# facebookresearch/PartDistillation

Measured on AMD Instinct MI355X. Metric: images/sec training step, R50 Mask2Former 1024² bs=2/GPU, 1/2/4/8 MI355X, higher is better.
Workload: dtype bf16

## Files before the change

### include/pd_rowwise.h

```cpp
#ifndef PD_ROWWISE_H
#define PD_ROWWISE_H

#include <stdint.h>

#ifdef __cplusplus
extern "C" {
#endif

int pd_add_layernorm_fwd(const void *x, int x_dtype, const float *res, const float *gamma, const float *beta, float eps,
                         float *z, float *y, void *y_c, const float *pos, int pos_div, void *ypos_c, int c_dtype,
                         float *mean, float *rstd, int rows, int C, void *stream);

int pd_add_layernorm_bwd(const float *dy, const float *dy2, const void *dy_c, const void *dypos_c, int c_dtype,
                         const float *z, const float *mean, const float *rstd, const float *gamma, float *dz, void *dz_c,
                         int dzc_dtype, float *dgamma, float *dbeta, float *dbias, float *dpos_acc, int pos_div,
                         int rows, int C, void *stream);

int pd_add_layernorm_fwd_amax(const void *x, int x_dtype, const float *res, const float *gamma, const float *beta, float eps,
                              float *z, float *y, void *y_c, const float *pos, int pos_div, void *ypos_c, int c_dtype,
                              float *mean, float *rstd, float *y_amax, float *ypos_amax, int rows, int C, void *stream);
int pd_add_layernorm_bwd_amax(const float *dy, const float *dy2, const void *dy_c, const void *dypos_c, int c_dtype,
                              const float *z, const float *mean, const float *rstd, const float *gamma, float *dz, void *dz_c,
                              int dzc_dtype, float *dgamma, float *dbeta, float *dbias, float *dpos_acc, int pos_div,
                              float *dz_amax, int rows, int C, void *stream);

int pd_colsum_acc(const void *x, int dtype, int rows, int N, float *acc, void *stream);

int pd_relu_bwd_colsum(void *dh, const void *h, int dtype, int rows, int N, float *acc, void *stream);

int pd_mem_prep_fwd(const float *tok, int64_t tok_batch_stride, const float *level_embed, const float *pos, void *mem_c,
                    void *mempos_c, int c_dtype, int B, int HW, int C, void *stream);

int pd_mem_prep_bwd(const void *dmem_c, const void *dmempos_c, int c_dtype, float *dtok, int64_t dtok_batch_stride, int B,
                    int HW, int C, void *stream);

int pd_attn_mask_u8(const void *logits, int dtype, int rows, int n, uint8_t *mask, void *stream);

int pd_matcher_point_terms(const void *x, int dtype, int rows, int n, float *x_f32, float *sigmoid_x, float *softplus_sum,
                           float *sigmoid_sum, void *stream);

int pd_msda_prep_fwd(const float *offs, const float *logits, const float *ref, const int64_t *spatial_shapes, float *loc,
                     float *attn, int64_t tokens, int M, int L, int P, int ld_offs, int ld_logits, void *stream);

int pd_msda_prep_bwd(const float *gloc, const float *gattn, const float *attn, const int64_t *spatial_shapes, float *d_offs,
                     float *d_logits, int64_t tokens, int M, int L, int P, int ld_offs, int ld_logits, void *stream);
int pd_msda_prep_bwd_amax(const float *gloc, const float *gattn, const float *attn, const int64_t *spatial_shapes, float *d_offs, float *d_logits,
                          float *row_amax, int64_t tokens, int M, int L, int P, int ld_offs, int ld_logits, void *stream);

int pd_point_sample_nhwc_f32(const float *in, const float *coords, float *out, int B, int H, int W, int C, int P, void *stream);
int pd_point_sample_nhwc_f32_bf16(const float *in, const float *coords, void *out, int B, int H, int W, int C, int P, void *stream);

int pd_point_sample_planar_f32(const float *in, const float *coords, float *out, int N, int C, int H, int W, int P, void *stream);
int pd_point_sample_planar_bwd_f32(const float *grad_out, const float *coords, float *grad_in, int N, int C, int H, int W, int P, void *stream);
int pd_point_sample_planar_bwd_needs_zero(int C, int H, int W);
int pd_point_sample_planar_bwd_needs_zero_n(int N, int C, int H, int W);

int pd_upsample_add_nhwc_f32(const float *lo, int64_t lo_batch_stride, const float *cur, float *y, int B, int h, int w, int H, int W, int C, void *stream);
int pd_upsample_add_amax_nhwc_f32(const float *lo, int64_t lo_batch_stride, const float *cur, float *y, float *amax, int B, int h, int w, int H, int W, int C,
                                  void *stream);
int pd_upsample2x_bwd_nhwc_f32(const float *dy, float *dlo, int B, int h, int w, int C, void *stream);

#define PD_RESIZE_MAX 4
int pd_resize_bilinear_nhwc_f32(const float *x, int B, int H, int W, int C, const int *heights, const int *widths, void *const *outs, int count,
                                int out_dtype, void *stream);


int pd_add_rows_amax_f32(const float *a, const float *b, float *q, float *a_copy, float *a_amax, float *q_amax, int rows, int cols, void *stream);

int pd_sum3_sum2_f32(const float *a, const float *b, const float *c, const float *d, float *out1, float *out2, int64_t n, void *stream);

int pd_skinny_linear_fwd(const void *x_bf16, const void *w, const void *b, int wb_dtype, float *y, int R, int C, int K, void *stream);
int64_t pd_skinny_linear_partial_floats(int R, int C, int K);
int pd_skinny_linear_bwd(const void *x_bf16, const void *w, int w_dtype, const float *dy, const void *dx_in_bf16, void *dx_out, int dx_dtype,
                         float *partial, void *dw, void *db, int b_dtype, int R, int C, int K, void *stream);

#define PD_TRANSPOSE_MAX 8
typedef struct {
  const void *src;
  void *dst;
  int64_t src_batch_stride, src_row_stride;
  int32_t batch, rows, cols, reserved;
} PdTransposeProblem;
int pd_transpose_batched_f32(const PdTransposeProblem *problems, int count, void *stream);

#define PD_COPY_MAX_SEGS 48
typedef struct PdCopySeg {
  const void *src;
  void *dst;
  int64_t bytes;
} PdCopySeg;
int pd_copy_segments(const PdCopySeg *segs, int count, void *stream);

#ifdef __cplusplus
}
#endif
#endif
```

### partdistillation_amd/csrc/cmdbuf.hip

```cpp
#include <hip/hip_runtime.h>
#include <stdint.h>
#include <string.h>

#include <type_traits>
#include <utility>

#include "pd_common.h"
#include "pd_cmdbuf.h"
#include "pd_attention.h"
#include "pd_conv.h"
#include "pd_declayer.h"
#include "pd_criterion.h"
#include "pd_fused.h"
#include "pd_gemm.h"
#include "pd_grouping.h"
#include "pd_igemm.h"
#include "pd_input.h"
#include "pd_kmeans.h"
#include "pd_msda.h"
#include "pd_mx8.h"
#include "pd_optim.h"
#include "pd_poly.h"
#include "pd_rowwise.h"
#include "pd_smallgemm.h"
#include "pd_stem.h"
#include "pd_swin.h"
#include "pd_window_attention.h"

namespace {

template <class T>
inline T word_to(uint64_t w)
{
  if constexpr (std::is_pointer_v<T>) {
    return reinterpret_cast<T>(static_cast<uintptr_t>(w));
  } else if constexpr (std::is_same_v<T, float>) {
    float f; uint32_t u = (uint32_t)w; memcpy(&f, &u, 4); return f;
  } else if constexpr (std::is_same_v<T, double>) {
    double d; memcpy(&d, &w, 8); return d;
  } else {
    return static_cast<T>(static_cast<int64_t>(w));
  }
}

template <auto F> struct Thunk;
template <class... A, int (*F)(A...)>
struct Thunk<F> {
  static constexpr int nargs = (int)sizeof...(A);
  template <size_t... I>
  static int invoke(const uint64_t *w, std::index_sequence<I...>) { return F(word_to<A>(w[I])...); }
  static int call(const uint64_t *w) { return invoke(w, std::index_sequence_for<A...>{}); }
};

struct Entry { const char *name; int (*call)(const uint64_t *); int nargs; };
#define PD_E(f) {#f, &Thunk<&f>::call, Thunk<&f>::nargs}
const Entry kTable[] = {
  PD_E(pd_adamw_clipped),
  PD_E(pd_adamw_clipped_shadow),
  PD_E(pd_add_layernorm_bwd),
  PD_E(pd_add_layernorm_bwd_amax),
  PD_E(pd_add_layernorm_fwd),
  PD_E(pd_add_layernorm_fwd_amax),
  PD_E(pd_add_rows_amax_f32),
  PD_E(pd_affine_act_bwd2_bf16),
  PD_E(pd_affine_act_bwd_bf16),
  PD_E(pd_affine_act_fwd_bf16),
  PD_E(pd_attn_bwd_d32),
  PD_E(pd_attn_fwd_d32),
  PD_E(pd_attn_mask_u8),
  PD_E(pd_cast_bf16_f32_amax),
  PD_E(pd_colsum_acc),
  PD_E(pd_conv3x3_nhwc_f16x2),
  PD_E(pd_conv3x3_nhwc_f32x3),
  PD_E(pd_conv3x3_wgrad_nhwc_f16x2),
  PD_E(pd_conv3x3_wgrad_nhwc_f32x3),
  PD_E(pd_conv_bf16_dgrad),
  PD_E(pd_conv_bf16_fwd),
  PD_E(pd_conv_bf16_wgrad),
  PD_E(pd_conv_bf16_wgrad_grouped),
  PD_E(pd_dec_bwd_a),
  PD_E(pd_dec_bwd_b),
  PD_E(pd_dec_fwd_a),
  PD_E(pd_dec_fwd_b),
  PD_E(pd_dec_pack_grouped),
  PD_E(pd_decoder_head_bf16),
  PD_E(pd_filter_transpose_grouped),
  PD_E(pd_gemm_tn_f16x2),
  PD_E(pd_gemm_tn_f16x2_bf16out),
  PD_E(pd_gemm_tn_f32),
  PD_E(pd_gemm_tn_f32x3),
  PD_E(pd_gemm_tn_f32x3_pre),
  PD_E(pd_gemm_tn_f32x3_relu_bits),
  PD_E(pd_gemm_tn_f32x3_relumask),
  PD_E(pd_gemm_wgrad_acc_f16x2_ws),
  PD_E(pd_gemm_wgrad_acc_f32),
  PD_E(pd_gemm_wgrad_acc_f32x3),
  PD_E(pd_gemm_wgrad_acc_f32x3_ws),
  PD_E(pd_gemm_wgrad_f16x2_grouped),
  PD_E(pd_gemm_wgrad_f32),
  PD_E(pd_gemm_wgrad_f32x3_grouped),
  PD_E(pd_gn_coeffs_bwd),
  PD_E(pd_gn_coeffs_fwd),
  PD_E(pd_igemm_bf16),
  PD_E(pd_igemm_bf16_seq),
  PD_E(pd_kmeans_assign),
  PD_E(pd_kmeans_assign_bounded),
  PD_E(pd_kmeans_assign_partial),
  PD_E(pd_kmeans_reduce),
  PD_E(pd_kmeans_reduce_update),
  PD_E(pd_kmeans_reduce_update_shift),
  PD_E(pd_kmeans_update),
  PD_E(pd_layernorm_rows_f32_bwd),
  PD_E(pd_layernorm_rows_f32_fwd),
  PD_E(pd_loss_vectors_bwd),
  PD_E(pd_loss_vectors_fwd),
  PD_E(pd_lsa_batched),
  PD_E(pd_mask_assign),
  PD_E(pd_mask_point_losses_bwd),
  PD_E(pd_mask_point_losses_fwd),
  PD_E(pd_matcher_costs),
  PD_E(pd_copy_segments),
  PD_E(pd_attn_fwd_d32_ld),
  PD_E(pd_attn_bwd_d32_ld),
  PD_E(pd_match_point_logits),
  PD_E(pd_swin_merge_ln_fwd),
  PD_E(pd_swin_tail_ln_fwd),
  PD_E(pd_swin_tail_ln_bwd),
  PD_E(pd_swin_merge_ln_bwd),
  PD_E(pd_matcher_point_terms),
  PD_E(pd_maxpool3s2_bwd_bf16),
  PD_E(pd_maxpool3s2_fwd_bf16),
  PD_E(pd_mem_prep_bwd),
  PD_E(pd_mem_prep_fwd),
  PD_E(pd_memcpy_d2d_async),
  PD_E(pd_memset_async),
  PD_E(pd_msda_backward),
  PD_E(pd_msda_forward),
  PD_E(pd_msda_forward_amax),
  PD_E(pd_msda_fused_backward),
  PD_E(pd_msda_fused_forward),
  PD_E(pd_msda_prep_bwd),
  PD_E(pd_msda_prep_bwd_amax),
  PD_E(pd_msda_prep_fwd),
  PD_E(pd_multi_gather_sumsq),
  PD_E(pd_mx8_gemm),
  PD_E(pd_mx8_quantize_bf16),
  PD_E(pd_mx8_quantize_grouped),
  PD_E(pd_nc_affine2_amax_f32),
  PD_E(pd_nc_affine2_f32),
  PD_E(pd_nc_affine_amax_f32),
  PD_E(pd_nc_affine_f32),
  PD_E(pd_nc_sums_f32),
  PD_E(pd_normalize_u8_nhwc),
  PD_E(pd_pair_logits_bwd_rows),
  PD_E(pd_pair_logits_bwd_tok),
  PD_E(pd_pair_logits_fwd),
  PD_E(pd_point_sample_nhwc_f32),
  PD_E(pd_point_sample_nhwc_f32_bf16),
  PD_E(pd_point_sample_planar_bwd_f32),
  PD_E(pd_point_sample_planar_f32),
  PD_E(pd_point_sample_u8),
  PD_E(pd_poly_crossings_i32),
  PD_E(pd_relu_bwd_colsum),
  PD_E(pd_resample_cols_canvas_u8),
  PD_E(pd_resample_cols_u8),
  PD_E(pd_resample_rows_u8),
  PD_E(pd_resize_bilinear_nhwc_f32),
  PD_E(pd_rle_sample_groups_canvas_u8),
  PD_E(pd_rle_sample_groups_u8),
  PD_E(pd_rle_sample_u8),
  PD_E(pd_row_amax_f32),
  PD_E(pd_scores_argmax_u8),
  PD_E(pd_sgemm_nn_bf16),
  PD_E(pd_sgemm_nn_splitn_bf16),
  PD_E(pd_sgemm_tn_batched_bf16),
  PD_E(pd_sgemm_tn_bf16),
  PD_E(pd_sgemm_tn_multi_bf16),
  PD_E(pd_sgemm_tn_splitk_bf16),
  PD_E(pd_sgemm_wgrad_bf16),
  PD_E(pd_sgemm_wgrad_grouped_bf16),
  PD_E(pd_sgemm_wgrad_split_bf16),
  PD_E(pd_skinny_linear_bwd),
  PD_E(pd_skinny_linear_fwd),
  PD_E(pd_split3_bf16),
  PD_E(pd_stem7x7_fwd),
  PD_E(pd_stem7x7_wgrad),
  PD_E(pd_sum3_sum2_f32),
  PD_E(pd_sumsq_accumulate),
  PD_E(pd_swin_ln_bwd),
  PD_E(pd_swin_ln_fwd),
  PD_E(pd_transpose_batched_f32),
  PD_E(pd_uncertain_points),
  PD_E(pd_upsample2x_bwd_nhwc_f32),
  PD_E(pd_upsample_add_amax_nhwc_f32),
  PD_E(pd_upsample_add_nhwc_f32),
  PD_E(pd_wgrad_bf16),
  PD_E(pd_wgrad_bf16_seq),
  PD_E(pd_window_attn_bwd_w12),
  PD_E(pd_window_attn_bwd_w7),
  PD_E(pd_window_attn_fwd_w12),
  PD_E(pd_window_attn_fwd_w7),
};
constexpr int kCount = (int)(sizeof(kTable) / sizeof(kTable[0]));
}

extern "C" int pd_memset_async(void *dst, int value, int64_t bytes, void *stream)
{
  if (bytes <= 0) return PD_OK;
  return hipMemsetAsync(dst, value, (size_t)bytes, (hipStream_t)stream) == hipSuccess ? PD_OK : pd_set_error(PD_ERR_LAUNCH, "pd_memset_async failed");
}

extern "C" int pd_memcpy_d2d_async(void *dst, const void *src, int64_t bytes, void *stream)
{
  if (bytes <= 0) return PD_OK;
  return hipMemcpyAsync(dst, src, (size_t)bytes, hipMemcpyDeviceToDevice, (hipStream_t)stream) == hipSuccess ? PD_OK
                                                                                                         : pd_set_error(PD_ERR_LAUNCH, "pd_memcpy_d2d_async failed");
}

extern "C" int pd_cmd_fn_index(const char *name)
{
  if (!name) return -1;
  for (int i = 0; i < kCount; ++i)
    if (!strcmp(kTable[i].name, name)) return i;
  return -1;
}

extern "C" int pd_cmd_fn_nargs(int fn) { return fn >= 0 && fn < kCount ? kTable[fn].nargs : -1; }

extern "C" int pd_cmd_replay(const PdCmd *cmds, int count, const uint64_t *slot_bases, int nslots, void *stream)
{
  uint64_t w[PD_CMD_MAX_ARGS];
  for (int c = 0; c < count; ++c) {
    const PdCmd &k = cmds[c];
    if (k.fn < 0 || k.fn >= kCount || k.nargs != kTable[k.fn].nargs || k.nargs > PD_CMD_MAX_ARGS)
      return pd_set_error(PD_ERR_INVALID_ARG, "pd_cmd_replay: command %d is malformed", c);
    for (int i = 0; i < k.nargs; ++i) {
      const int s = k.kind[i];
      if (s == PD_CMD_LITERAL) w[i] = k.a[i];
      else if (s == PD_CMD_STREAM) w[i] = (uint64_t)(uintptr_t)stream;
      else if (s >= 0 && s < nslots) w[i] = slot_bases[s] + k.a[i];
      else return pd_set_error(PD_ERR_INVALID_ARG, "pd_cmd_replay: command %d argument %d names slot %d of %d", c, i, s, nslots);
    }
    const int rc = kTable[k.fn].call(w);
    if (rc != PD_OK) return rc;
  }
  return PD_OK;
}
```

### partdistillation_amd/csrc/common.hip

```cpp
#include <hip/hip_runtime.h>
#include <stdarg.h>
#include <stdio.h>
#include <string.h>

#include "pd_common.h"
#include "pd_msda.h"

namespace {
thread_local char g_err[512] = {0};
}

int pd_set_error(int code, const char *fmt, ...)
{
  va_list ap;
  va_start(ap, fmt);
  vsnprintf(g_err, sizeof(g_err), fmt, ap);
  va_end(ap);
  return code;
}

int pd_check_launch(const char *what)
{
  hipError_t e = hipGetLastError();
  if (e == hipSuccess) return PD_OK;
  return pd_set_error(PD_ERR_LAUNCH, "%s: %s", what, hipGetErrorString(e));
}

extern "C" const char *pd_last_error(void) { return g_err; }
extern "C" int pd_abi_version(void) { return 49; }

extern int g_pd_dbg_atomic_scope;
extern int g_pd_dbg_force_generic;
extern int g_pd_dbg_ablate;
extern int g_pd_dbg_x3_narrow;
extern int g_pd_dbg_f16x2;
extern int g_pd_dbg_wgrad_wide;
extern "C" void pd_dbg_set_wgrad_xcd(int v);
extern "C" void pd_dbg_set_wgrad_fast(int v);
extern int g_pd_dbg_bwd_variant;
extern int g_pd_dbg_msda_gate_pct;
extern int g_pd_dbg_wgrad_wgs;
extern int g_pd_dbg_bwd_threads;
extern int g_pd_dbg_attn_scalar;
extern int g_pd_dbg_wattn;
extern int g_pd_dbg_wattn_chunk;
extern int g_pd_dbg_x3;
extern int g_pd_dbg_kmeans;
extern int g_pd_dbg_conv_group_rows;
extern int g_pd_dbg_conv_xcd_major;
extern int g_pd_dbg_sgemm_deep;
extern int g_ig_bn, g_ig_nst, g_ig_splits, g_ig_patch, g_ig_pcls;
extern int g_mx_bn, g_mx_nst;
extern int g_swin_ln_abl;
extern int g_ln_bwd_cap;
extern int g_crit_abl;
extern int g_attn_bwd_kc;
extern int g_wg_nst, g_wg_splits, g_wg_mode;
extern "C" int pd_debug_set(const char *key, int value)
{
  if (!key) return PD_ERR_INVALID_ARG;
  if (!strcmp(key, "msda_bwd_atomic_scope")) { g_pd_dbg_atomic_scope = value; return PD_OK; }
  if (!strcmp(key, "msda_ablate")) { g_pd_dbg_ablate = value; return PD_OK; }
  if (!strcmp(key, "msda_bwd_variant")) { g_pd_dbg_bwd_variant = value; return PD_OK; }
  if (!strcmp(key, "msda_gate_pct")) { g_pd_dbg_msda_gate_pct = value; return PD_OK; }
  if (!strcmp(key, "attn_scalar")) { g_pd_dbg_attn_scalar = value; return PD_OK; }
  if (!strcmp(key, "msda_bwd_threads")) { g_pd_dbg_bwd_threads = value; return PD_OK; }
  if (!strcmp(key, "wgrad_wgs")) { g_pd_dbg_wgrad_wgs = value; return PD_OK; }
  if (!strcmp(key, "kmeans_ablate")) { g_pd_dbg_kmeans = value; return PD_OK; }
  if (!strcmp(key, "wg_nst")) { g_wg_nst = value; return PD_OK; }
  if (!strcmp(key, "wg_splits")) { g_wg_splits = value; return PD_OK; }
  if (!strcmp(key, "wg_mode")) { g_wg_mode = value; return PD_OK; }
  if (!strcmp(key, "ig_bn")) { g_ig_bn = value; return PD_OK; }
  if (!strcmp(key, "ig_patch")) { g_ig_patch = value; return PD_OK; }
  if (!strcmp(key, "ig_pcls")) { g_ig_pcls = value; return PD_OK; }
  if (!strcmp(key, "ig_nst")) { g_ig_nst = value; return PD_OK; }
  if (!strcmp(key, "mx_bn")) { g_mx_bn = value; return PD_OK; }
  if (!strcmp(key, "attn_bwd_kc")) { g_attn_bwd_kc = value; return PD_OK; }
  if (!strcmp(key, "crit_abl")) { g_crit_abl = value; return PD_OK; }
  if (!strcmp(key, "ln_bwd_cap")) { g_ln_bwd_cap = value; return PD_OK; }
  if (!strcmp(key, "swin_ln_abl")) { g_swin_ln_abl = value; return PD_OK; }
  if (!strcmp(key, "mx_nst")) { g_mx_nst = value; return PD_OK; }
  if (!strcmp(key, "ig_splits")) { g_ig_splits = value; return PD_OK; }
  if (!strcmp(key, "sgemm_deep")) { g_pd_dbg_sgemm_deep = value; return PD_OK; }
  if (!strcmp(key, "conv_group_rows")) { g_pd_dbg_conv_group_rows = value; return PD_OK; }
  if (!strcmp(key, "conv_xcd_major")) { g_pd_dbg_conv_xcd_major = value; return PD_OK; }
  if (!strcmp(key, "x3_ablate")) { g_pd_dbg_x3 = value; return PD_OK; }
  if (!strcmp(key, "f16x2_tile")) { g_pd_dbg_f16x2 = value; return PD_OK; }
  if (!strcmp(key, "wgrad_wide")) { g_pd_dbg_wgrad_wide = value; return PD_OK; }
  if (!strcmp(key, "wgrad_xcd")) { pd_dbg_set_wgrad_xcd(value); return PD_OK; }
  if (!strcmp(key, "wgrad_fast")) { pd_dbg_set_wgrad_fast(value); return PD_OK; }
  if (!strcmp(key, "x3_narrow")) { g_pd_dbg_x3_narrow = value; return PD_OK; }
  if (!strcmp(key, "wattn_ablate")) { g_pd_dbg_wattn = value; return PD_OK; }
  if (!strcmp(key, "wattn_chunk")) {
    if (value < 0 || value > 8) return pd_set_error(PD_ERR_INVALID_ARG, "pd_debug_set: wattn_chunk is 0 (automatic) or 1..8, got %d", value);
    g_pd_dbg_wattn_chunk = value;
    return PD_OK;
  }
  if (!strcmp(key, "msda_force_generic")) { g_pd_dbg_force_generic = value; return PD_OK; }
  return pd_set_error(PD_ERR_INVALID_ARG, "pd_debug_set: unknown key %s", key);
}

extern "C" int pd_debug_get(const char *key, int *value)
{
  if (!key || !value) return PD_ERR_INVALID_ARG;
  if (!strcmp(key, "msda_bwd_variant")) { *value = g_pd_dbg_bwd_variant; return PD_OK; }
  if (!strcmp(key, "msda_gate_pct")) { *value = g_pd_dbg_msda_gate_pct; return PD_OK; }
  return pd_set_error(PD_ERR_INVALID_ARG, "pd_debug_get: unknown key %s", key);
}
```

### partdistillation_amd/csrc/rowwise.hip

```cpp
#include <hip/hip_runtime.h>
#include <stdint.h>
#include <string.h>

#include "pd_common.h"
#include "pd_msda.h"
#include "pd_rowwise.h"

int g_ln_bwd_cap = 0;
namespace {

typedef unsigned short bf16_t;

__device__ __forceinline__ float bf2f(bf16_t h) { return __uint_as_float((unsigned)h << 16); }
__device__ __forceinline__ bf16_t f2bf(float f)
{
  unsigned u = __float_as_uint(f);
  if ((u & 0x7fffffffu) > 0x7f800000u) return (bf16_t)((u >> 16) | 0x40);
  u += 0x7fffu + ((u >> 16) & 1u);
  return (bf16_t)(u >> 16);
}

__device__ __forceinline__ float4 ld4(const float *p) { return *reinterpret_cast<const float4 *>(p); }
__device__ __forceinline__ float4 ld4(const bf16_t *p)
{
  const ushort4 v = *reinterpret_cast<const ushort4 *>(p);
  return make_float4(bf2f(v.x), bf2f(v.y), bf2f(v.z), bf2f(v.w));
}
__device__ __forceinline__ void st4(float *p, float4 v) { *reinterpret_cast<float4 *>(p) = v; }
__device__ __forceinline__ void st4(bf16_t *p, float4 v)
{
  ushort4 o;
  o.x = f2bf(v.x); o.y = f2bf(v.y); o.z = f2bf(v.z); o.w = f2bf(v.w);
  *reinterpret_cast<ushort4 *>(p) = o;
}
__device__ __forceinline__ float4 add4(float4 a, float4 b) { return make_float4(a.x + b.x, a.y + b.y, a.z + b.z, a.w + b.w); }

template <int CTRL>
__device__ __forceinline__ float dpp_mov(float v)
{
  return __int_as_float(__builtin_amdgcn_update_dpp(0, __float_as_int(v), CTRL, 0xF, 0xF, true));
}

__device__ __forceinline__ float wave_sum(float v)
{
  v += dpp_mov<0xB1>(v);
  v += dpp_mov<0x4E>(v);
  v += dpp_mov<0x141>(v);
  v += dpp_mov<0x140>(v);
  v += __shfl_xor(v, 16, 64);
  v += __shfl_xor(v, 32, 64);
  return v;
}

__device__ __forceinline__ float wave_max(float v)
{
  v = fmaxf(v, dpp_mov<0xB1>(v));
  v = fmaxf(v, dpp_mov<0x4E>(v));
  v = fmaxf(v, dpp_mov<0x141>(v));
  v = fmaxf(v, dpp_mov<0x140>(v));
  v = fmaxf(v, __shfl_xor(v, 16, 64));
  v = fmaxf(v, __shfl_xor(v, 32, 64));
  return v;
}
__device__ __forceinline__ float amax4(float4 v) { return fmaxf(fmaxf(fabsf(v.x), fabsf(v.y)), fmaxf(fabsf(v.z), fabsf(v.w))); }

template <int NV4, typename XT, typename CT>
__global__ __launch_bounds__(256) void add_ln_fwd(const XT *__restrict__ x, const float *__restrict__ res,
                                                  const float *__restrict__ gamma, const float *__restrict__ beta, float eps,
                                                  float *__restrict__ z, float *__restrict__ y, CT *__restrict__ y_c,
                                                  const float *__restrict__ pos, int pos_div, CT *__restrict__ ypos_c,
                                                  float *__restrict__ mean, float *__restrict__ rstd, int rows,
                                                  float *__restrict__ y_amax, float *__restrict__ ypos_amax)
{
  constexpr int C = NV4 * 256;
  const int wave = threadIdx.x >> 6, lane = threadIdx.x & 63;
  float4 gm[NV4], bt[NV4];
#pragma unroll
  for (int j = 0; j < NV4; ++j) {
    gm[j] = ld4(gamma + j * 256 + lane * 4);
    bt[j] = ld4(beta + j * 256 + lane * 4);
  }
  for (int r = blockIdx.x * 4 + wave; r < rows; r += gridDim.x * 4) {
    const int64_t base = (int64_t)r * C + lane * 4;
    float4 v[NV4];
    float s = 0.f;
#pragma unroll
    for (int j = 0; j < NV4; ++j) {
      v[j] = x ? ld4(x + base + j * 256) : make_float4(0.f, 0.f, 0.f, 0.f);
      if (res) v[j] = add4(v[j], ld4(res + base + j * 256));
      if (z) st4(z + base + j * 256, v[j]);
      s += (v[j].x + v[j].y) + (v[j].z + v[j].w);
    }
    const float mu = wave_sum(s) * (1.f / C);
    float q = 0.f;
#pragma unroll
    for (int j = 0; j < NV4; ++j) {
      v[j].x -= mu; v[j].y -= mu; v[j].z -= mu; v[j].w -= mu;
      q += (v[j].x * v[j].x + v[j].y * v[j].y) + (v[j].z * v[j].z + v[j].w * v[j].w);
    }
    const float rs = rsqrtf(wave_sum(q) * (1.f / C) + eps);
    if (lane == 0) { mean[r] = mu; rstd[r] = rs; }
    const float *prow = pos ? pos + (int64_t)(r / pos_div) * C + lane * 4 : nullptr;
    float my = 0.f, mp = 0.f;
#pragma unroll
    for (int j = 0; j < NV4; ++j) {
      float4 o;
      o.x = v[j].x * rs * gm[j].x + bt[j].x;
      o.y = v[j].y * rs * gm[j].y + bt[j].y;
      o.z = v[j].z * rs * gm[j].z + bt[j].z;
      o.w = v[j].w * rs * gm[j].w + bt[j].w;
      if (y) st4(y + base + j * 256, o);
      if (y_c) st4(y_c + base + j * 256, o);
      my = fmaxf(my, amax4(o));
      if (ypos_c) {
        const float4 op = add4(o, ld4(prow + j * 256));
        st4(ypos_c + base + j * 256, op);
        mp = fmaxf(mp, amax4(op));
      }
    }
    if (y_amax) { my = wave_max(my); if (lane == 0) y_amax[r] = my; }
    if (ypos_amax) { mp = wave_max(mp); if (lane == 0) ypos_amax[r] = mp; }
  }
}

template <int NV4, typename CT, typename DT, int WAVES>
__global__ __launch_bounds__(64 * WAVES) void add_ln_bwd(const float *dy, const float *__restrict__ dy2,
                                                  const CT *__restrict__ dy_c, const CT *__restrict__ dypos_c,
                                                  const float *__restrict__ z, const float *__restrict__ mean,
                                                  const float *__restrict__ rstd, const float *__restrict__ gamma,
                                                  float *dz, DT *__restrict__ dz_c, float *__restrict__ dgamma,
                                                  float *__restrict__ dbeta, float *__restrict__ dbias,
                                                  float *__restrict__ dpos_acc, int pos_div, int rows, float *__restrict__ dz_amax)
{
  constexpr int C = NV4 * 256;
  __shared__ float red[WAVES][3][C];
  const int wave = threadIdx.x >> 6, lane = threadIdx.x & 63;
  float4 gm[NV4], ag[NV4], ab[NV4], ad[NV4];
#pragma unroll
  for (int j = 0; j < NV4; ++j) {
    gm[j] = ld4(gamma + j * 256 + lane * 4);
    ag[j] = ab[j] = ad[j] = make_float4(0.f, 0.f, 0.f, 0.f);
  }
  for (int r = blockIdx.x * WAVES + wave; r < rows; r += gridDim.x * WAVES) {
    const int64_t base = (int64_t)r * C + lane * 4;
    const float mu = mean[r], rs = rstd[r];
    float4 g[NV4], xh[NV4];
    float s1 = 0.f, s2 = 0.f;
#pragma unroll
    for (int j = 0; j < NV4; ++j) {
      float4 t = make_float4(0.f, 0.f, 0.f, 0.f);
      if (dy) t = ld4(dy + base + j * 256);
      if (dy2) t = add4(t, ld4(dy2 + base + j * 256));
      if (dy_c) t = add4(t, ld4(dy_c + base + j * 256));
      if (dypos_c) {
        const float4 p = ld4(dypos_c + base + j * 256);
        t = add4(t, p);
        if (dpos_acc) {
          float *a = dpos_acc + (int64_t)(r / pos_div) * C + j * 256 + lane * 4;
          if (pos_div == 1) st4(a, add4(ld4(a), p));
          else { atomicAdd(a, p.x); atomicAdd(a + 1, p.y); atomicAdd(a + 2, p.z); atomicAdd(a + 3, p.w); }
        }
      }
      float4 h = ld4(z + base + j * 256);
      h.x = (h.x - mu) * rs; h.y = (h.y - mu) * rs; h.z = (h.z - mu) * rs; h.w = (h.w - mu) * rs;
      ag[j].x += t.x * h.x; ag[j].y += t.y * h.y; ag[j].z += t.z * h.z; ag[j].w += t.w * h.w;
      ab[j] = add4(ab[j], t);
      t.x *= gm[j].x; t.y *= gm[j].y; t.z *= gm[j].z; t.w *= gm[j].w;
      s1 += (t.x + t.y) + (t.z + t.w);
      s2 += (t.x * h.x + t.y * h.y) + (t.z * h.z + t.w * h.w);
      g[j] = t; xh[j] = h;
    }
    const float m1 = wave_sum(s1) * (1.f / C), m2 = wave_sum(s2) * (1.f / C);
    float mz = 0.f;
#pragma unroll
    for (int j = 0; j < NV4; ++j) {
      float4 o;
      o.x = rs * (g[j].x - m1 - xh[j].x * m2);
      o.y = rs * (g[j].y - m1 - xh[j].y * m2);
      o.z = rs * (g[j].z - m1 - xh[j].z * m2);
      o.w = rs * (g[j].w - m1 - xh[j].w * m2);
      ad[j] = add4(ad[j], o);
      st4(dz + base + j * 256, o);
      if (dz_c) st4(dz_c + base + j * 256, o);
      mz = fmaxf(mz, amax4(o));
    }
    if (dz_amax) { mz = wave_max(mz); if (lane == 0) dz_amax[r] = mz; }
  }
  if (!dgamma && !dbeta && !dbias) return;
#pragma unroll
  for (int j = 0; j < NV4; ++j) {
    st4(&red[wave][0][j * 256 + lane * 4], ag[j]);
    st4(&red[wave][1][j * 256 + lane * 4], ab[j]);
    st4(&red[wave][2][j * 256 + lane * 4], ad[j]);
  }
  __syncthreads();
  float *const outs[3] = {dgamma, dbeta, dbias};
  for (int i = threadIdx.x; i < 3 * C; i += 64 * WAVES) {
    const int k = i / C, c = i - k * C;
    if (!outs[k]) continue;
    float sum = 0.f;
#pragma unroll
    for (int w = 0; w < WAVES; ++w) sum += red[w][k][c];
    atomicAdd(outs[k] + c, sum);
  }
}

template <typename T, bool RELU>
__global__ __launch_bounds__(256) void colsum_acc(T *__restrict__ x, const T *__restrict__ h, int rows, int N, int rows_per_blk,
                                                  float *__restrict__ acc)
{
  __shared__ float red[4][128];
  const int wave = threadIdx.x >> 6, lane = threadIdx.x & 63;
  const int c0 = blockIdx.x * 128 + lane * 2;
  const int r_begin = blockIdx.y * rows_per_blk, r_end = min(rows, r_begin + rows_per_blk);
  float a0 = 0.f, a1 = 0.f;
  int r = r_begin + wave;
  if (!RELU && sizeof(T) == 4) {
    for (; r + 12 < r_end; r += 16) {
      const float *p = reinterpret_cast<const float *>(x) + (int64_t)r * N + c0;
      const float2 u0 = *reinterpret_cast<const float2 *>(p), u1 = *reinterpret_cast<const float2 *>(p + (int64_t)4 * N);
      const float2 u2 = *reinterpret_cast<const float2 *>(p + (int64_t)8 * N), u3 = *reinterpret_cast<const float2 *>(p + (int64_t)12 * N);
      a0 += (u0.x + u1.x) + (u2.x + u3.x);
      a1 += (u0.y + u1.y) + (u2.y + u3.y);
    }
  }
  for (; r < r_end; r += 4) {
    T *p = x + (int64_t)r * N + c0;
    float v0, v1;
    if constexpr (sizeof(T) == 2) {
      const unsigned u = *reinterpret_cast<const unsigned *>(p);
      v0 = bf2f((bf16_t)(u & 0xffffu)); v1 = bf2f((bf16_t)(u >> 16));
    } else {
      const float2 u = *reinterpret_cast<const float2 *>(p);
      v0 = u.x; v1 = u.y;
    }
    if (RELU) {
      float h0, h1;
      if constexpr (sizeof(T) == 2) {
        const unsigned u = *reinterpret_cast<const unsigned *>(h + (int64_t)r * N + c0);
        h0 = bf2f((bf16_t)(u & 0xffffu)); h1 = bf2f((bf16_t)(u >> 16));
      } else {
        const float2 u = *reinterpret_cast<const float2 *>(h + (int64_t)r * N + c0);
        h0 = u.x; h1 = u.y;
      }
      if (!(h0 > 0.f)) v0 = 0.f;
      if (!(h1 > 0.f)) v1 = 0.f;
      if constexpr (sizeof(T) == 2) *reinterpret_cast<unsigned *>(p) = (unsigned)f2bf(v0) | ((unsigned)f2bf(v1) << 16);
      else *reinterpret_cast<float2 *>(p) = make_float2(v0, v1);
    }
    a0 += v0; a1 += v1;
  }
  if (!acc) return;
  red[wave][lane * 2] = a0; red[wave][lane * 2 + 1] = a1;
  __syncthreads();
  if (threadIdx.x < 128) {
    const int c = threadIdx.x;
    atomicAdd(acc + blockIdx.x * 128 + c, (red[0][c] + red[1][c]) + (red[2][c] + red[3][c]));
  }
}

template <typename CT>
__global__ __launch_bounds__(256) void mem_prep_fwd(const float *__restrict__ tok, int64_t bstride, const float *__restrict__ lvl,
                                                    const float *__restrict__ pos, CT *__restrict__ mem, CT *__restrict__ mempos,
                                                    int B, int HW, int C)
{
  const int wave = threadIdx.x >> 6, lane = threadIdx.x & 63;
  const int rows = B * HW;
  for (int r = blockIdx.x * 4 + wave; r < rows; r += gridDim.x * 4) {
    const int p = r / B, b = r - p * B;
    const float *src = tok + (int64_t)b * bstride + (int64_t)p * C;
    for (int c = lane * 4; c < C; c += 256) {
      float4 v = ld4(src + c);
      if (lvl) v = add4(v, ld4(lvl + c));
      if (mem) st4(mem + (int64_t)r * C + c, v);
      if (mempos) st4(mempos + (int64_t)r * C + c, add4(v, ld4(pos + (int64_t)p * C + c)));
    }
  }
}

template <typename CT>
__global__ __launch_bounds__(256) void mem_prep_bwd(const CT *__restrict__ dmem, const CT *__restrict__ dmempos,
                                                    float *__restrict__ dtok, int64_t bstride, int B, int HW, int C)
{
  const int wave = threadIdx.x >> 6, lane = threadIdx.x & 63;
  const int rows = B * HW;
  for (int r = blockIdx.x * 4 + wave; r < rows; r += gridDim.x * 4) {
    const int b = r / HW, p = r - b * HW;
    const int64_t srow = ((int64_t)p * B + b) * C;
    float *dst = dtok + (int64_t)b * bstride + (int64_t)p * C;
    for (int c = lane * 4; c < C; c += 256) {
      float4 v = make_float4(0.f, 0.f, 0.f, 0.f);
      if (dmem) v = ld4(dmem + srow + c);
      if (dmempos) v = add4(v, ld4(dmempos + srow + c));
      st4(dst + c, v);
    }
  }
}

template <typename T>
__global__ __launch_bounds__(256) void attn_mask_u8(const T *__restrict__ logits, int n, uint8_t *__restrict__ mask)
{
  __shared__ int any_open;
  const T *row = logits + (int64_t)blockIdx.x * n;
  uint8_t *out = mask + (int64_t)blockIdx.x * n;
  if (threadIdx.x == 0) any_open = 0;
  __syncthreads();
  int open = 0;
  for (int i = threadIdx.x; i < n; i += 256) {
    float v;
    if constexpr (sizeof(T) == 2) v = bf2f(row[i]); else v = row[i];
    open |= !(v < 0.f);
  }
  if (__ballot(open) != 0ull && (threadIdx.x & 63) == 0) atomicOr(&any_open, 1);
  __syncthreads();
  const bool keep = any_open != 0;
  for (int i = threadIdx.x; i < n; i += 256) {
    float v;
    if constexpr (sizeof(T) == 2) v = bf2f(row[i]); else v = row[i];
    out[i] = (keep && v < 0.f) ? 1 : 0;
  }
}

__device__ __forceinline__ unsigned neg2(unsigned w)
{
  const unsigned lo = w & 0xffffu, hi = w >> 16;
  const unsigned bl = (lo & 0x8000u) && (lo & 0x7fffu) != 0u && (lo & 0x7fffu) <= 0x7f80u;
  const unsigned bh = (hi & 0x8000u) && (hi & 0x7fffu) != 0u && (hi & 0x7fffu) <= 0x7f80u;
  return bl | (bh << 8);
}
constexpr int AMV = 8;
__global__ __launch_bounds__(256) void attn_mask_u8_bf16x8(const bf16_t *__restrict__ logits, int n, uint8_t *__restrict__ mask)
{
  __shared__ int any_open;
  const uint4 *row = reinterpret_cast<const uint4 *>(logits + (int64_t)blockIdx.x * n);
  uint2 *out = reinterpret_cast<uint2 *>(mask + (int64_t)blockIdx.x * n);
  const int nv = n >> 3;
  if (threadIdx.x == 0) any_open = 0;
  uint2 b[AMV];
  unsigned all = 0x01010101u;
// ... 371 lines not shown
      for (int of = 32; of; of >>= 1) m = fmaxf(m, __shfl_xor(m, of, 64));
      if ((threadIdx.x & 63) == 0) amax[i >> 6] = m;
    }
  }
}

struct ResizeLevels { void *out[PD_RESIZE_MAX]; int h[PD_RESIZE_MAX], w[PD_RESIZE_MAX]; int64_t first[PD_RESIZE_MAX + 1]; int count; };

template <bool BF16>
__global__ __launch_bounds__(256) void resize_bilinear_nhwc_multi(const float *__restrict__ x, int B, int H, int W, int C4, ResizeLevels lv)
{
  for (int64_t i = (int64_t)blockIdx.x * 256 + threadIdx.x; i < lv.first[lv.count]; i += (int64_t)gridDim.x * 256) {
    int l = 0;
#pragma unroll
    for (int k = 1; k < PD_RESIZE_MAX; ++k) l += (k < lv.count && i >= lv.first[k]) ? 1 : 0;
    const int h = lv.h[l], w = lv.w[l];
    int64_t t = i - lv.first[l];
    const int c = (int)(t % C4); t /= C4;
    const int ox = (int)(t % w); t /= w;
    const int oy = (int)(t % h);
    const int b = (int)(t / h);
    int y0, yp, x0, xp; float hy0, hy1, wx0, wx1;
    up_src(oy, (float)H / (float)h, H, y0, yp, hy0, hy1);
    up_src(ox, (float)W / (float)w, W, x0, xp, wx0, wx1);
    const float4 *L = reinterpret_cast<const float4 *>(x) + (int64_t)b * H * W * C4;
    const float4 a = L[((int64_t)y0 * W + x0) * C4 + c], bq = L[((int64_t)y0 * W + x0 + xp) * C4 + c];
    const float4 cq = L[((int64_t)(y0 + yp) * W + x0) * C4 + c], d = L[((int64_t)(y0 + yp) * W + x0 + xp) * C4 + c];
    float4 o;
    o.x = hy0 * (wx0 * a.x + wx1 * bq.x) + hy1 * (wx0 * cq.x + wx1 * d.x);
    o.y = hy0 * (wx0 * a.y + wx1 * bq.y) + hy1 * (wx0 * cq.y + wx1 * d.y);
    o.z = hy0 * (wx0 * a.z + wx1 * bq.z) + hy1 * (wx0 * cq.z + wx1 * d.z);
    o.w = hy0 * (wx0 * a.w + wx1 * bq.w) + hy1 * (wx0 * cq.w + wx1 * d.w);
    const int64_t oi = (((int64_t)b * h + oy) * w + ox) * C4 + c;
    if (BF16) st4(reinterpret_cast<bf16_t *>(lv.out[l]) + oi * 4, o);
    else st4(reinterpret_cast<float *>(lv.out[l]) + oi * 4, o);
  }
}

__global__ __launch_bounds__(256) void upsample2x_bwd_nhwc(const float *__restrict__ dy, float *__restrict__ dlo, int B, int h,
                                                           int w, int C4)
{
  const int H = 2 * h, W = 2 * w;
  const int64_t total = (int64_t)B * h * w * C4;
  for (int64_t i = (int64_t)blockIdx.x * blockDim.x + threadIdx.x; i < total; i += (int64_t)gridDim.x * blockDim.x) {
    const int c = (int)(i % C4);
    int64_t t = i / C4;
    const int ix = (int)(t % w); t /= w;
    const int iy = (int)(t % h);
    const int b = (int)(t / h);
    float wy[4], wx[4];
#pragma unroll
    for (int k = 0; k < 4; ++k) {
      const int oy = 2 * iy - 1 + k, ox = 2 * ix - 1 + k;
      wy[k] = 0.f; wx[k] = 0.f;
      if (oy >= 0 && oy < H) {
        int i0, ip; float l0, l1;
        up_src(oy, 0.5f, h, i0, ip, l0, l1);
        if (i0 == iy) wy[k] += l0;
        if (i0 + ip == iy) wy[k] += l1;
      }
      if (ox >= 0 && ox < W) {
        int i0, ip; float l0, l1;
        up_src(ox, 0.5f, w, i0, ip, l0, l1);
        if (i0 == ix) wx[k] += l0;
        if (i0 + ip == ix) wx[k] += l1;
      }
    }
    const float4 *G = reinterpret_cast<const float4 *>(dy) + (int64_t)b * H * W * C4;
    float4 acc = make_float4(0.f, 0.f, 0.f, 0.f);
    float4 gt[4][4];
#pragma unroll
    for (int ky = 0; ky < 4; ++ky) {
      const int oy = min(max(2 * iy - 1 + ky, 0), H - 1);
#pragma unroll
      for (int kx = 0; kx < 4; ++kx) gt[ky][kx] = G[((int64_t)oy * W + min(max(2 * ix - 1 + kx, 0), W - 1)) * C4 + c];
    }
#pragma unroll
    for (int ky = 0; ky < 4; ++ky) {
#pragma unroll
      for (int kx = 0; kx < 4; ++kx) {
        const float wgt = wy[ky] * wx[kx];
        const bool on = wy[ky] != 0.f && wx[kx] != 0.f;
        const float4 g = gt[ky][kx];
        acc.x = on ? fmaf(wgt, g.x, acc.x) : acc.x; acc.y = on ? fmaf(wgt, g.y, acc.y) : acc.y;
        acc.z = on ? fmaf(wgt, g.z, acc.z) : acc.z; acc.w = on ? fmaf(wgt, g.w, acc.w) : acc.w;
      }
    }
    reinterpret_cast<float4 *>(dlo)[i] = acc;
  }
}

int grid_rows(int rows, int cap) { return max(1, min(cap, (rows + 3) / 4)); }

struct TrBatch { PdTransposeProblem p[PD_TRANSPOSE_MAX]; int first_tile[PD_TRANSPOSE_MAX + 1]; int count; };

__global__ __launch_bounds__(256) void transpose_batched_f32(TrBatch tb)
{
  __shared__ float tile[32][33];
  int pi = 0;
#pragma unroll
  for (int i = 1; i < PD_TRANSPOSE_MAX; ++i) pi += (i < tb.count && (int)blockIdx.x >= tb.first_tile[i]) ? 1 : 0;
  const PdTransposeProblem &pr = tb.p[pi];
  const int tr = (pr.rows + 31) / 32, tc = (pr.cols + 31) / 32;
  int t = blockIdx.x - tb.first_tile[pi];
  const int b = t / (tr * tc); t -= b * tr * tc;
  const int r0 = (t / tc) * 32, c0 = (t % tc) * 32;
  const int tx = threadIdx.x & 31, ty = threadIdx.x >> 5;
  const float *src = (const float *)pr.src + (int64_t)b * pr.src_batch_stride;
  float *dst = (float *)pr.dst + (int64_t)b * pr.rows * pr.cols;
#pragma unroll
  for (int k = 0; k < 4; ++k) {
    const int r = r0 + ty + 8 * k, c = c0 + tx;
    if (r < pr.rows && c < pr.cols) tile[ty + 8 * k][tx] = src[(int64_t)r * pr.src_row_stride + c];
  }
  __syncthreads();
#pragma unroll
  for (int k = 0; k < 4; ++k) {
    const int c = c0 + ty + 8 * k, r = r0 + tx;
    if (r < pr.rows && c < pr.cols) dst[(int64_t)c * pr.rows + r] = tile[tx][ty + 8 * k];
  }
}


__global__ __launch_bounds__(256) void add_rows_amax_f32(const float *__restrict__ a, const float *__restrict__ b, float *__restrict__ q,
                                                         float *__restrict__ a_copy, float *__restrict__ a_amax, float *__restrict__ q_amax,
                                                         int rows, int cols)
{
  const int row = blockIdx.x * 4 + (threadIdx.x >> 6), lane = threadIdx.x & 63;
  if (row >= rows) return;
  const int64_t base = (int64_t)row * cols;
  float ma = 0.f, mq = 0.f;
  for (int c = lane * 4; c < cols; c += 256) {
    const float4 x = ld4(a + base + c), y = ld4(b + base + c);
    const float4 s = make_float4(x.x + y.x, x.y + y.y, x.z + y.z, x.w + y.w);
    st4(q + base + c, s);
    if (a_copy) st4(a_copy + base + c, x);
    ma = fmaxf(ma, amax4(x)); mq = fmaxf(mq, amax4(s));
  }
#pragma unroll
  for (int o = 32; o; o >>= 1) { ma = fmaxf(ma, __shfl_xor(ma, o, 64)); mq = fmaxf(mq, __shfl_xor(mq, o, 64)); }
  if (lane == 0) { a_amax[row] = ma; q_amax[row] = mq; }
}

__global__ __launch_bounds__(256) void sum3_sum2_f32(const float4 *__restrict__ a, const float4 *__restrict__ b, const float4 *__restrict__ c,
                                                     const float4 *__restrict__ d, float4 *__restrict__ o1, float4 *__restrict__ o2, int64_t n4)
{
  for (int64_t i = (int64_t)blockIdx.x * 256 + threadIdx.x; i < n4; i += (int64_t)gridDim.x * 256) {
    const float4 x = a[i], y = b[i], z = c[i], w = d[i];
    o1[i] = make_float4((x.x + y.x) + z.x, (x.y + y.y) + z.y, (x.z + y.z) + z.z, (x.w + y.w) + z.w);
    o2[i] = make_float4(w.x + z.x, w.y + z.y, w.z + z.z, w.w + z.w);
  }
}

bool dt_ok(int dt) { return dt == PD_F32 || dt == PD_BF16; }

}

#define NV4_SWITCH(C, BODY)                                                                                        \
  switch ((C) / 256) {                                                                                             \
    case 1: { constexpr int NV4 = 1; BODY; } break;                                                                \
    case 2: { constexpr int NV4 = 2; BODY; } break;                                                                \
    case 3: { constexpr int NV4 = 3; BODY; } break;                                                                \
    case 4: { constexpr int NV4 = 4; BODY; } break;                                                                \
    default: return pd_set_error(PD_ERR_INVALID_ARG, "C=%d: supported widths are 256, 512, 768, 1024", (C)); \
  }

static int add_layernorm_fwd(const void *x, int x_dtype, const float *res, const float *gamma, const float *beta, float eps,
                             float *z, float *y, void *y_c, const float *pos, int pos_div, void *ypos_c, int c_dtype,
                             float *mean, float *rstd, int rows, int C, void *stream_, float *y_amax, float *ypos_amax)
{
  if (rows < 0 || C <= 0 || (C % 256)) return pd_set_error(PD_ERR_INVALID_ARG, "pd_add_layernorm_fwd: rows=%d C=%d", rows, C);
  if (rows == 0) return PD_OK;
  if ((!x && !res) || !gamma || !beta || !mean || !rstd) return pd_set_error(PD_ERR_INVALID_ARG, "pd_add_layernorm_fwd: null pointer");
  if ((x && !dt_ok(x_dtype)) || ((y_c || ypos_c) && !dt_ok(c_dtype))) return pd_set_error(PD_ERR_INVALID_ARG, "pd_add_layernorm_fwd: dtype");
  if (ypos_c && (!pos || pos_div <= 0)) return pd_set_error(PD_ERR_INVALID_ARG, "pd_add_layernorm_fwd: ypos_c needs pos and pos_div > 0");
  hipStream_t s = (hipStream_t)stream_;
  dim3 g(grid_rows(rows, 2048)), b(256);
  const bool xb = x && x_dtype == PD_BF16, cb = c_dtype == PD_BF16;
#define LAUNCH(XT, CT) hipLaunchKernelGGL((add_ln_fwd<NV4, XT, CT>), g, b, 0, s, (const XT *)x, res, gamma, beta, eps, z, y, (CT *)y_c, pos, pos_div, (CT *)ypos_c, mean, rstd, rows, y_amax, ypos_amax)
  NV4_SWITCH(C, {
    if (xb) { if (cb) LAUNCH(bf16_t, bf16_t); else LAUNCH(bf16_t, float); }
    else { if (cb) LAUNCH(float, bf16_t); else LAUNCH(float, float); }
  })
#undef LAUNCH
  return pd_check_launch("pd_add_layernorm_fwd");
}

extern "C" int pd_add_layernorm_fwd(const void *x, int x_dtype, const float *res, const float *gamma, const float *beta, float eps,
                                    float *z, float *y, void *y_c, const float *pos, int pos_div, void *ypos_c, int c_dtype,
                                    float *mean, float *rstd, int rows, int C, void *stream_)
{
  return add_layernorm_fwd(x, x_dtype, res, gamma, beta, eps, z, y, y_c, pos, pos_div, ypos_c, c_dtype, mean, rstd, rows, C, stream_, nullptr, nullptr);
}

extern "C" int pd_add_layernorm_fwd_amax(const void *x, int x_dtype, const float *res, const float *gamma, const float *beta, float eps,
                                         float *z, float *y, void *y_c, const float *pos, int pos_div, void *ypos_c, int c_dtype,
                                         float *mean, float *rstd, float *y_amax, float *ypos_amax, int rows, int C, void *stream_)
{
  if (ypos_amax && !ypos_c) return pd_set_error(PD_ERR_INVALID_ARG, "pd_add_layernorm_fwd_amax: ypos_amax needs ypos_c");
  return add_layernorm_fwd(x, x_dtype, res, gamma, beta, eps, z, y, y_c, pos, pos_div, ypos_c, c_dtype, mean, rstd, rows, C, stream_, y_amax, ypos_amax);
}

static int add_layernorm_bwd(const float *dy, const float *dy2, const void *dy_c, const void *dypos_c, int c_dtype,
                             const float *z, const float *mean, const float *rstd, const float *gamma, float *dz,
                             void *dz_c, int dzc_dtype, float *dgamma, float *dbeta, float *dbias, float *dpos_acc,
                             int pos_div, int rows, int C, void *stream_, float *dz_amax)
{
  if (rows < 0 || C <= 0 || (C % 256)) return pd_set_error(PD_ERR_INVALID_ARG, "pd_add_layernorm_bwd: rows=%d C=%d", rows, C);
  if (rows == 0) return PD_OK;
  if ((!dy && !dy2 && !dy_c && !dypos_c) || !z || !mean || !rstd || !gamma || !dz)
    return pd_set_error(PD_ERR_INVALID_ARG, "pd_add_layernorm_bwd: null pointer");
  if (((dy_c || dypos_c) && !dt_ok(c_dtype)) || (dz_c && !dt_ok(dzc_dtype))) return pd_set_error(PD_ERR_INVALID_ARG, "pd_add_layernorm_bwd: dtype");
  if (dpos_acc && pos_div <= 0) return pd_set_error(PD_ERR_INVALID_ARG, "pd_add_layernorm_bwd: pos_div");
  hipStream_t s = (hipStream_t)stream_;
  const bool cb = c_dtype == PD_BF16, db = dzc_dtype == PD_BF16;
#define LAUNCH(CT, DT, WV) hipLaunchKernelGGL((add_ln_bwd<NV4, CT, DT, WV>), g, b, 0, s, dy, dy2, (const CT *)dy_c, (const CT *)dypos_c, z, mean, rstd, gamma, dz, (DT *)dz_c, dgamma, dbeta, dbias, dpos_acc, pos_div, rows, dz_amax)
#define LAUNCH_W(WV)                                                                    \
  if (cb) { if (db) LAUNCH(bf16_t, bf16_t, WV); else LAUNCH(bf16_t, float, WV); }      \
  else { if (db) LAUNCH(float, bf16_t, WV); else LAUNCH(float, float, WV); }
  NV4_SWITCH(C, {
    constexpr int FAT = NV4 == 1 ? 16 : NV4 == 2 ? 8 : 4;
    if (rows >= 8192 && FAT > 4 && g_ln_bwd_cap >= 0) {
      const int cap = g_ln_bwd_cap > 0 ? g_ln_bwd_cap : 256;
      const dim3 g(max(1, min(cap, (rows + 4 * FAT - 1) / (4 * FAT))));
      const dim3 b(64 * FAT);
      LAUNCH_W(FAT)
    } else {
      const dim3 g(grid_rows(rows, 1024));
      const dim3 b(256);
      LAUNCH_W(4)
    }
  })
#undef LAUNCH_W
#undef LAUNCH
  return pd_check_launch("pd_add_layernorm_bwd");
}

extern "C" int pd_add_layernorm_bwd(const float *dy, const float *dy2, const void *dy_c, const void *dypos_c, int c_dtype,
                                    const float *z, const float *mean, const float *rstd, const float *gamma, float *dz,
                                    void *dz_c, int dzc_dtype, float *dgamma, float *dbeta, float *dbias, float *dpos_acc,
                                    int pos_div, int rows, int C, void *stream_)
{
  return add_layernorm_bwd(dy, dy2, dy_c, dypos_c, c_dtype, z, mean, rstd, gamma, dz, dz_c, dzc_dtype, dgamma, dbeta, dbias, dpos_acc, pos_div, rows, C,
                           stream_, nullptr);
}

extern "C" int pd_add_layernorm_bwd_amax(const float *dy, const float *dy2, const void *dy_c, const void *dypos_c, int c_dtype,
                                         const float *z, const float *mean, const float *rstd, const float *gamma, float *dz,
                                         void *dz_c, int dzc_dtype, float *dgamma, float *dbeta, float *dbias, float *dpos_acc,
                                         int pos_div, float *dz_amax, int rows, int C, void *stream_)
{
  return add_layernorm_bwd(dy, dy2, dy_c, dypos_c, c_dtype, z, mean, rstd, gamma, dz, dz_c, dzc_dtype, dgamma, dbeta, dbias, dpos_acc, pos_div, rows, C,
                           stream_, dz_amax);
}

static int colsum_launch(void *x, const void *h, int dtype, int rows, int N, float *acc, bool relu, hipStream_t s, const char *who)
{
  if (rows < 0 || N <= 0 || (N % 128) || !dt_ok(dtype)) return pd_set_error(PD_ERR_INVALID_ARG, "%s: rows=%d N=%d dtype=%d", who, rows, N, dtype);
  if (rows == 0) return PD_OK;
  if (!x || (relu && !h) || (!relu && !acc)) return pd_set_error(PD_ERR_INVALID_ARG, "%s: null pointer", who);
  const int rpb = rows <= 4096 ? 64 : 256;
  dim3 g(N / 128, (rows + rpb - 1) / rpb), b(256);
  if (dtype == PD_BF16) {
    if (relu) hipLaunchKernelGGL((colsum_acc<bf16_t, true>), g, b, 0, s, (bf16_t *)x, (const bf16_t *)h, rows, N, rpb, acc);
    else hipLaunchKernelGGL((colsum_acc<bf16_t, false>), g, b, 0, s, (bf16_t *)x, (const bf16_t *)h, rows, N, rpb, acc);
  } else {
    if (relu) hipLaunchKernelGGL((colsum_acc<float, true>), g, b, 0, s, (float *)x, (const float *)h, rows, N, rpb, acc);
    else hipLaunchKernelGGL((colsum_acc<float, false>), g, b, 0, s, (float *)x, (const float *)h, rows, N, rpb, acc);
  }
  return pd_check_launch(who);
}

extern "C" int pd_colsum_acc(const void *x, int dtype, int rows, int N, float *acc, void *stream_)
{
  return colsum_launch(const_cast<void *>(x), nullptr, dtype, rows, N, acc, false, (hipStream_t)stream_, "pd_colsum_acc");
}

extern "C" int pd_relu_bwd_colsum(void *dh, const void *h, int dtype, int rows, int N, float *acc, void *stream_)
{
  return colsum_launch(dh, h, dtype, rows, N, acc, true, (hipStream_t)stream_, "pd_relu_bwd_colsum");
}

extern "C" int pd_mem_prep_fwd(const float *tok, int64_t tok_batch_stride, const float *level_embed, const float *pos, void *mem_c,
                               void *mempos_c, int c_dtype, int B, int HW, int C, void *stream_)
{
  if (B < 0 || HW < 0 || C <= 0 || (C % 256) || !dt_ok(c_dtype)) return pd_set_error(PD_ERR_INVALID_ARG, "pd_mem_prep_fwd: B=%d HW=%d C=%d", B, HW, C);
  if (B == 0 || HW == 0) return PD_OK;
  if (!tok || (!mem_c && !mempos_c) || (mempos_c && !pos)) return pd_set_error(PD_ERR_INVALID_ARG, "pd_mem_prep_fwd: null pointer");
  dim3 g(grid_rows(B * HW, 4096)), b(256);
  if (c_dtype == PD_BF16) hipLaunchKernelGGL((mem_prep_fwd<bf16_t>), g, b, 0, (hipStream_t)stream_, tok, tok_batch_stride, level_embed, pos, (bf16_t *)mem_c, (bf16_t *)mempos_c, B, HW, C);
  else hipLaunchKernelGGL((mem_prep_fwd<float>), g, b, 0, (hipStream_t)stream_, tok, tok_batch_stride, level_embed, pos, (float *)mem_c, (float *)mempos_c, B, HW, C);
  return pd_check_launch("pd_mem_prep_fwd");
}

extern "C" int pd_mem_prep_bwd(const void *dmem_c, const void *dmempos_c, int c_dtype, float *dtok, int64_t dtok_batch_stride, int B,
                               int HW, int C, void *stream_)
{
  if (B < 0 || HW < 0 || C <= 0 || (C % 256) || !dt_ok(c_dtype)) return pd_set_error(PD_ERR_INVALID_ARG, "pd_mem_prep_bwd: B=%d HW=%d C=%d", B, HW, C);
  if (B == 0 || HW == 0) return PD_OK;
  if (!dtok || (!dmem_c && !dmempos_c)) return pd_set_error(PD_ERR_INVALID_ARG, "pd_mem_prep_bwd: null pointer");
  dim3 g(grid_rows(B * HW, 4096)), b(256);
  if (c_dtype == PD_BF16) hipLaunchKernelGGL((mem_prep_bwd<bf16_t>), g, b, 0, (hipStream_t)stream_, (const bf16_t *)dmem_c, (const bf16_t *)dmempos_c, dtok, dtok_batch_stride, B, HW, C);
  else hipLaunchKernelGGL((mem_prep_bwd<float>), g, b, 0, (hipStream_t)stream_, (const float *)dmem_c, (const float *)dmempos_c, dtok, dtok_batch_stride, B, HW, C);
  return pd_check_launch("pd_mem_prep_bwd");
}

struct CopySegs {
  const unsigned char *src[PD_COPY_MAX_SEGS];
  unsigned char *dst[PD_COPY_MAX_SEGS];
  int64_t bytes[PD_COPY_MAX_SEGS];
};
__global__ __launch_bounds__(256) void copy_segments(const CopySegs sg)
{
  const int seg = blockIdx.y;
  const unsigned char *src = sg.src[seg];
  unsigned char *dst = sg.dst[seg];
  const int64_t n = sg.bytes[seg];
  const int64_t tid = (int64_t)blockIdx.x * 256 + threadIdx.x, nth = (int64_t)gridDim.x * 256;
  if ((((uintptr_t)src | (uintptr_t)dst) & 15) == 0) {
    const int64_t n16 = n >> 4;
    for (int64_t i = tid; i < n16; i += nth) reinterpret_cast<uint4 *>(dst)[i] = reinterpret_cast<const uint4 *>(src)[i];
    for (int64_t i = (n16 << 4) + tid; i < n; i += nth) dst[i] = src[i];
  } else {
    for (int64_t i = tid; i < n; i += nth) dst[i] = src[i];
  }
}

extern "C" int pd_copy_segments(const PdCopySeg *segs, int count, void *stream_)
{
  if (count < 0 || count > PD_COPY_MAX_SEGS || (count > 0 && !segs)) return pd_set_error(PD_ERR_INVALID_ARG, "pd_copy_segments: count=%d (<= %d)", count, PD_COPY_MAX_SEGS);
  if (count == 0) return PD_OK;
  CopySegs sg;
  int64_t longest = 0;
  for (int i = 0; i < count; ++i) {
    if (segs[i].bytes < 0 || (segs[i].bytes > 0 && (!segs[i].src || !segs[i].dst))) return pd_set_error(PD_ERR_INVALID_ARG, "pd_copy_segments: segment %d", i);
    sg.src[i] = (const unsigned char *)segs[i].src; sg.dst[i] = (unsigned char *)segs[i].dst; sg.bytes[i] = segs[i].bytes;
    if (segs[i].bytes > longest) longest = segs[i].bytes;
  }
  for (int i = count; i < PD_COPY_MAX_SEGS; ++i) { sg.src[i] = nullptr; sg.dst[i] = nullptr; sg.bytes[i] = 0; }
  int bx = (int)((longest + 256 * 16 * 4 - 1) / (256 * 16 * 4));
  bx = bx < 1 ? 1 : bx > 64 ? 64 : bx;
  hipLaunchKernelGGL(copy_segments, dim3((unsigned)bx, (unsigned)count), dim3(256), 0, (hipStream_t)stream_, sg);
  return pd_check_launch("pd_copy_segments");
}

extern "C" int pd_attn_mask_u8(const void *logits, int dtype, int rows, int n, uint8_t *mask, void *stream_)
{
  if (rows < 0 || n < 0 || !dt_ok(dtype)) return pd_set_error(PD_ERR_INVALID_ARG, "pd_attn_mask_u8: rows=%d n=%d dtype=%d", rows, n, dtype);
  if (rows == 0 || n == 0) return PD_OK;
  if (!logits || !mask) return pd_set_error(PD_ERR_INVALID_ARG, "pd_attn_mask_u8: null pointer");
  if (dtype == PD_BF16 && !(n & 7) && n <= 256 * 8 * AMV && !((uintptr_t)logits & 15) && !((uintptr_t)mask & 7))
    hipLaunchKernelGGL(attn_mask_u8_bf16x8, dim3(rows), dim3(256), 0, (hipStream_t)stream_, (const bf16_t *)logits, n, mask);
  else if (dtype == PD_BF16) hipLaunchKernelGGL((attn_mask_u8<bf16_t>), dim3(rows), dim3(256), 0, (hipStream_t)stream_, (const bf16_t *)logits, n, mask);
  else hipLaunchKernelGGL((attn_mask_u8<float>), dim3(rows), dim3(256), 0, (hipStream_t)stream_, (const float *)logits, n, mask);
  return pd_check_launch("pd_attn_mask_u8");
}

extern "C" int pd_matcher_point_terms(const void *x, int dtype, int rows, int n, float *x_f32, float *sigmoid_x, float *softplus_sum,
                                      float *sigmoid_sum, void *stream_)
{
  if (rows < 0 || n < 0 || !dt_ok(dtype)) return pd_set_error(PD_ERR_INVALID_ARG, "pd_matcher_point_terms: rows=%d n=%d dtype=%d", rows, n, dtype);
  if (rows == 0) return PD_OK;
  if (!x || !sigmoid_x || !softplus_sum || !sigmoid_sum) return pd_set_error(PD_ERR_INVALID_ARG, "pd_matcher_point_terms: null pointer");
  if (dtype == PD_BF16) hipLaunchKernelGGL((matcher_point_terms<bf16_t>), dim3(rows), dim3(256), 0, (hipStream_t)stream_, (const bf16_t *)x, n, x_f32, sigmoid_x, softplus_sum, sigmoid_sum);
  else hipLaunchKernelGGL((matcher_point_terms<float>), dim3(rows), dim3(256), 0, (hipStream_t)stream_, (const float *)x, n, x_f32, sigmoid_x, softplus_sum, sigmoid_sum);
  return pd_check_launch("pd_matcher_point_terms");
}

extern "C" int pd_msda_prep_fwd(const float *offs, const float *logits, const float *ref, const int64_t *spatial_shapes, float *loc,
                                float *attn, int64_t tokens, int M, int L, int P, int ld_offs, int ld_logits, void *stream_)
{
  if (ld_offs < M * L * P * 2 || ld_logits < M * L * P || (ld_offs & 3) || (ld_logits & 3))
    return pd_set_error(PD_ERR_INVALID_ARG, "pd_msda_prep_fwd: row strides %d / %d (>= row length, multiples of 4)", ld_offs, ld_logits);
  if (tokens < 0 || M <= 0 || L <= 0 || P <= 0) return pd_set_error(PD_ERR_INVALID_ARG, "pd_msda_prep_fwd: tokens=%lld M=%d L=%d P=%d", (long long)tokens, M, L, P);
  if (tokens == 0) return PD_OK;
  if (!offs || !logits || !ref || !spatial_shapes || !loc || !attn) return pd_set_error(PD_ERR_INVALID_ARG, "pd_msda_prep_fwd: null pointer");
  const int64_t total = tokens * M;
  const dim3 g((unsigned)((total + 255) / 256)), b(256);
  hipStream_t s = (hipStream_t)stream_;
  const int LP = L * P;
#define LAUNCH(KER) hipLaunchKernelGGL(KER, g, b, 0, s, offs, logits, ref, spatial_shapes, loc, attn, total, M, L, P, ld_offs, ld_logits)
  if ((P & 1) == 0 && LP == 12) LAUNCH(msda_prep_fwd_v<3>);
  else if ((P & 1) == 0 && LP == 16) LAUNCH(msda_prep_fwd_v<4>);
  else if ((P & 1) == 0 && LP == 8) LAUNCH(msda_prep_fwd_v<2>);
  else LAUNCH(msda_prep_fwd);
#undef LAUNCH
  return pd_check_launch("pd_msda_prep_fwd");
}

static int msda_prep_bwd_launch(const float *gloc, const float *gattn, const float *attn, const int64_t *spatial_shapes, float *d_offs,
                                float *d_logits, int64_t tokens, int M, int L, int P, int ld_offs, int ld_logits, void *stream_, float *row_amax)
{
  if (row_amax && (M != 8 || (P & 1) || (L * P != 12 && L * P != 16 && L * P != 8)))
    return pd_set_error(PD_ERR_INVALID_ARG, "pd_msda_prep_bwd_amax: row maxima need 8 heads and L P in {8, 12, 16} (the vector kernels)");
  if (ld_offs < M * L * P * 2 || ld_logits < M * L * P || (ld_offs & 3) || (ld_logits & 3))
    return pd_set_error(PD_ERR_INVALID_ARG, "pd_msda_prep_bwd: row strides %d / %d (>= row length, multiples of 4)", ld_offs, ld_logits);
  if (tokens < 0 || M <= 0 || L <= 0 || P <= 0) return pd_set_error(PD_ERR_INVALID_ARG, "pd_msda_prep_bwd: tokens=%lld M=%d L=%d P=%d", (long long)tokens, M, L, P);
  if (tokens == 0) return PD_OK;
  if (!gloc || !gattn || !attn || !spatial_shapes || !d_offs || !d_logits) return pd_set_error(PD_ERR_INVALID_ARG, "pd_msda_prep_bwd: null pointer");
  const int64_t total = tokens * M;
  const dim3 g((unsigned)((total + 255) / 256)), b(256);
  hipStream_t s = (hipStream_t)stream_;
  const int LP = L * P;
#define LAUNCH(KER) hipLaunchKernelGGL(KER, g, b, 0, s, gloc, gattn, attn, spatial_shapes, d_offs, d_logits, total, M, L, P, ld_offs, ld_logits, row_amax)
  if ((P & 1) == 0 && LP == 12) LAUNCH(msda_prep_bwd_v<3>);
  else if ((P & 1) == 0 && LP == 16) LAUNCH(msda_prep_bwd_v<4>);
// ... 318 lines not shown
```

### partdistillation_amd/functions/encoder_core.py

```python
import os

import torch
from torch.autograd import Function

from .. import MultiScaleDeformableAttention as MSDA
from .. import lib as _lib
from . import rowwise as rw
from .. import cmdbuf
from . import gemm as _gemm
from .gemm import (WgradQueue, gemm_tn_h2, gemm_tn_x3, gemm_tn_x3_pre, gemm_tn_x3_relu_bits, gemm_tn_x3_relumask, gemm_wgrad_acc,
                   h2_bits_supported, pre_supported, relu_bits_supported, row_amax, split3)

def _timed(kind, fn, *args):
    from ..modeling.pixel_decoder.ops.functions.ms_deform_attn_func import _timed as t
    return t(kind, fn, *args)


def _drop_backward_of(key, rec, cache):
    for k in [k for k in cache if k[0] == "bwd" and k[1] == id(rec)]:
        cache.pop(k)


_RECS = cmdbuf.LRU(int(__import__("os").environ.get("PD_ENCODER_REC_CAP", "6")), _drop_backward_of)


def _msda_timing():
    from ..modeling.pixel_decoder.ops.functions.ms_deform_attn_func import _TIMING as t
    return t


N_LAYER = 16


def msda_prep_fwd(offs, logits, ref, shapes, M, L, P):
    tokens = offs.shape[0]
    assert offs.stride(1) == 1 and logits.stride(1) == 1 and offs.dtype == torch.float32 and logits.dtype == torch.float32
    loc = torch.empty((tokens, M, L, P, 2), dtype=torch.float32, device=offs.device)
    attn = torch.empty((tokens, M, L, P), dtype=torch.float32, device=offs.device)
    _lib.check(_lib.load().pd_msda_prep_fwd(offs.data_ptr(), logits.data_ptr(), ref.data_ptr(), shapes.data_ptr(), loc.data_ptr(),
                                            attn.data_ptr(), tokens, M, L, P, offs.stride(0), logits.stride(0), rw._stream()))
    return loc, attn


def msda_prep_bwd(gloc, gattn, attn, shapes, tokens, M, L, P, out=None, amax=None):
    n = M * L * P
    if out is None:
        out = torch.empty((tokens, 3 * n), dtype=torch.float32, device=attn.device)
    d_offs, d_logits = out[:, :2 * n], out[:, 2 * n:]
    if amax is not None:
        _lib.check(_lib.load().pd_msda_prep_bwd_amax(gloc.data_ptr(), gattn.data_ptr(), attn.data_ptr(), shapes.data_ptr(), d_offs.data_ptr(),
                                                     d_logits.data_ptr(), amax.data_ptr(), tokens, M, L, P, out.stride(0), out.stride(0), rw._stream()))
        return d_offs, d_logits
    _lib.check(_lib.load().pd_msda_prep_bwd(gloc.data_ptr(), gattn.data_ptr(), attn.data_ptr(), shapes.data_ptr(), d_offs.data_ptr(),
                                            d_logits.data_ptr(), tokens, M, L, P, out.stride(0), out.stride(0), rw._stream()))
    return d_offs, d_logits


def prep_amax_supported(M, L, P):
    return M == 8 and P % 2 == 0 and L * P in (8, 12, 16)


def msda_forward_amax(value, shapes, lsi, loc, attn, im2col_step, row_amax):
    B, S, M, D = value.shape
    Lq, L, P = loc.shape[1], loc.shape[3], loc.shape[4]
    out = torch.empty((B, Lq, M * D), dtype=value.dtype, device=value.device)
    _lib.check(_lib.load().pd_msda_forward_amax(value.data_ptr(), shapes.data_ptr(), lsi.data_ptr(), loc.data_ptr(), attn.data_ptr(), out.data_ptr(),
                                                row_amax.data_ptr(), B, S, M, D, L, Lq, P, int(im2col_step), _lib.PD_F32, rw._stream()))
    return out


FUSED_MSDA = os.environ.get("PD_MSDA_FUSED", "1") != "0"


def msda_fused_supported(B, S, M, D, L, Lq, P):
    return FUSED_MSDA and bool(_lib.load().pd_msda_fused_supported(B, S, M, D, L, Lq, P))


def msda_fused_forward(value, shapes, lsi, oa, ref, row_amax):
    B, S, M, D = value.shape
    L = int(shapes.shape[0])
    P = oa.shape[1] // (3 * M * L)
    assert oa.stride(1) == 1 and oa.dtype == torch.float32 and ref.is_contiguous() and ref.numel() == B * S * L * 2
    out = torch.empty((B * S, M * D), dtype=torch.float32, device=value.device)
    stats = torch.empty((B * S * M, 2), dtype=torch.float32, device=value.device)
    _lib.check(_lib.load().pd_msda_fused_forward(value.data_ptr(), shapes.data_ptr(), lsi.data_ptr(), oa.data_ptr(), oa.stride(0), ref.data_ptr(),
                                                 out.data_ptr(), stats.data_ptr(), row_amax.data_ptr() if row_amax is not None else None,
                                                 B, S, M, D, L, S, P, rw._stream()))
    return out, stats


def msda_fused_backward(value, shapes, lsi, oa, ref, stats, out, grad_out):
    B, S, M, D = value.shape
    L = int(shapes.shape[0])
    n_oa = oa.shape[1]
    P = n_oa // (3 * M * L)
    both = torch.empty(value.numel() + B * S, dtype=torch.float32, device=value.device)
    gv, d_oa_am = both[:value.numel()].view(value.shape), both[value.numel():]
    d_oa = torch.empty((B * S, n_oa), dtype=torch.float32, device=value.device)
    scratch = torch.empty(B * S * M * L, dtype=torch.float32, device=value.device)
    grad_out = grad_out if grad_out.is_contiguous() else grad_out.contiguous()
    _lib.check(_lib.load().pd_msda_fused_backward(value.data_ptr(), shapes.data_ptr(), lsi.data_ptr(), oa.data_ptr(), oa.stride(0), ref.data_ptr(),
                                                  stats.data_ptr(), out.data_ptr(), grad_out.data_ptr(), gv.data_ptr(), d_oa.data_ptr(), d_oa.stride(0),
                                                  d_oa_am.data_ptr(), scratch.data_ptr(), B, S, M, D, L, S, P, rw._stream()))
    return gv, d_oa, d_oa_am


class EncoderSpec:
    def __init__(self, n_heads, n_levels, n_points, eps, im2col_step, reference_points, spatial_shapes, level_start_index):
        self.M, self.L, self.P, self.eps, self.im2col_step = n_heads, n_levels, n_points, eps, im2col_step
        self.ref, self.shapes, self.lsi = reference_points, spatial_shapes, level_start_index


USE_X3 = True
GROUP_WGRADS = os.environ.get("PD_GROUP_WGRADS", "1") != "0"
X3_PROJ = os.environ.get("PD_X3_PROJ", "1") != "0"
H2_WGRAD = os.environ.get("PD_H2_WGRAD", "1") != "0"
H2 = os.environ.get("PD_H2", "1") != "0"
PRESPLIT = False


def _proj(x, w, b=None):
    if X3_PROJ and USE_X3 and x.is_cuda and x.dtype == torch.float32 and w.dtype == torch.float32 and x.shape[1] % 4 == 0 and x.stride(1) == 1 \
            and x.stride(0) % 4 == 0:
        return gemm_tn_x3(x, w, b)
    return torch.addmm(b, x, w.t()) if b is not None else torch.mm(x, w.t())


def _ffn_gemm(x, w, b=None, relu=False):
    if USE_X3 and x.is_cuda and x.dtype == torch.float32 and w.dtype == torch.float32 and x.shape[1] % 4 == 0:
        return gemm_tn_x3(x, w, b, relu)
    if relu:
        return torch._addmm_activation(b, x, w.t(), use_gelu=False)
    return torch.addmm(b, x, w.t()) if b is not None else torch.mm(x, w.t())


import ctypes as _ct


class _TrProblem(_ct.Structure):
    _fields_ = [("src", _ct.c_void_p), ("dst", _ct.c_void_p), ("src_batch_stride", _ct.c_int64), ("src_row_stride", _ct.c_int64),
                ("batch", _ct.c_int32), ("rows", _ct.c_int32), ("cols", _ct.c_int32), ("reserved", _ct.c_int32)]


class _Stack:

    def __init__(self, t, rev):
        self.t, self.rev = t, rev

    def __getitem__(self, i):
        return self.t[self.t.shape[0] - 1 - i if self.rev else i]


class EncoderCore(Function):
    @staticmethod
    def forward(ctx, spec: EncoderSpec, src, pos, *params):
        ctx.set_materialize_grads(False)
        B, S, C = src.shape
        M, L, P = spec.M, spec.L, spec.P
        nl = len(params) // N_LAYER
        T = B * S
        src2 = src.reshape(T, C)
        src2 = src2 if src2.is_contiguous() else src2.contiguous()
        pos2 = pos.reshape(T, C)
        pos2 = pos2 if pos2.is_contiguous() else pos2.contiguous()
        ref = spec.ref.reshape(T, L, 2)
        ref = ref if ref.is_contiguous() else ref.contiguous()
        saved = []
        x = src2
        h2 = H2 and USE_X3 and X3_PROJ and src2.is_cuda and C % 4 == 0 and src2.dtype == torch.float32 and pos2.dtype == torch.float32
        ctx.h2 = h2
        if h2:
            return EncoderCore._forward_h2(ctx, spec, src2, pos2, None, ref, params, (B, S, C, nl))
        q = src2 + pos2
        for i in range(nl):
            (so_w, so_b, aw_w, aw_b, vp_w, vp_b, op_w, op_b, n1_w, n1_b, l1_w, l1_b, l2_w, l2_b, n2_w, n2_b) = params[i * N_LAYER:(i + 1) * N_LAYER]
            value = _proj(x, vp_w, vp_b)
            w_oa, b_oa = torch.cat([so_w, aw_w]), torch.cat([so_b, aw_b])
            oa = _proj(q, w_oa, b_oa)
            n_off = so_w.shape[0]
            loc, attn = msda_prep_fwd(oa[:, :n_off], oa[:, n_off:], ref, spec.shapes, M, L, P)
            v4, loc6, attn5 = value.view(B, S, M, C // M), loc.view(B, S, M, L, P, 2), attn.view(B, S, M, L, P)
            a = _timed("fwd", MSDA.ms_deform_attn_forward, v4, spec.shapes, spec.lsi, loc6, attn5, spec.im2col_step).view(T, C)
            z1, y1, _, _, m1, r1 = rw.add_ln_fwd(_proj(a, op_w, op_b), x, n1_w, n1_b, spec.eps)
            hbits = None
            pre = USE_X3 and PRESPLIT and pre_supported(T, l1_w.shape[0], l1_w.shape[1]) and pre_supported(T, l2_w.shape[0], l2_w.shape[1])
            if pre:
                h, hbits = gemm_tn_x3_pre(y1, split3(l1_w), l1_b, mode=1, want_bits=True)
            elif USE_X3 and relu_bits_supported(T, l1_w.shape[0]):
                h, hbits = gemm_tn_x3_relu_bits(y1, l1_w, l1_b)
            else:
                h = _ffn_gemm(y1, l1_w, l1_b, relu=True)
            ffn2 = gemm_tn_x3_pre(h, split3(l2_w), l2_b) if pre else _ffn_gemm(h, l2_w, l2_b)
            last = i == nl - 1
            z2, y2, _, ypos, m2, r2 = rw.add_ln_fwd(ffn2, y1, n2_w, n2_b, spec.eps, c_dtype=torch.float32,
                                                    pos=pos2, pos_div=1, want_ypos=not last)
            saved.append((x, q, v4, loc6, attn5, a, z1, m1, r1, y1, h, z2, m2, r2, w_oa, hbits))
            x, q = y2, ypos
        ctx.spec, ctx.saved, ctx.params, ctx.dims = spec, saved, params, (B, S, C, nl)
        return x.view(B, S, C)

    @staticmethod
    def _forward_h2(ctx, spec, src2, pos2, q, ref, params, dims):
        B, S, C, nl = dims
        P_ = lambda i, j: params[i * N_LAYER + j]
        n_off, n_aw = P_(0, 0).shape[0], P_(0, 2).shape[0]
        wk = torch.cat([P_(i, j) for i in range(nl) for j in (0, 2, 4, 6, 10)])
        b_oa_all = torch.cat([P_(i, j) for i in range(nl) for j in (1, 3)]).view(nl, n_off + n_aw)
        l2_all = torch.cat([P_(i, 12) for i in range(nl)])
        ctx.wk = wk
        use_rec = (cmdbuf.usable() and src2.is_cuda and any(ctx.needs_input_grad) and not _gemm._TIMING["on"]
                   and not _msda_timing()["on"])
        if not use_rec:
            ctx.rec = None
            x, saved, saved_am = EncoderCore._layers_h2(spec, src2, pos2, q, ref, wk, b_oa_all, l2_all, params, dims)
        else:
            slots = [src2, pos2, ref, wk, b_oa_all, l2_all, spec.shapes, spec.lsi] + list(params)
            key = ("fwd", B, S, C, nl, spec.M, spec.L, spec.P, str(src2.device), _lib.current_stream())
            rec = _RECS.get(key)
            if rec is None or not rec.matches(slots):
                rec = cmdbuf.Recording(slots, "encoder forward")
                with rec:
                    outs = EncoderCore._layers_h2(spec, src2, pos2, q, ref, wk, b_oa_all, l2_all, params, dims)
                x, saved, saved_am = rec.finish(outs)
                _RECS.put(key, rec)
            else:
                x, saved, saved_am = rec.replay(slots)
            ctx.rec, ctx.rec_gen = rec, rec.generation
        ctx.saved_am = saved_am
        ctx.spec, ctx.saved, ctx.params, ctx.dims = spec, saved, params, (B, S, C, nl)
        return x.view(B, S, C)

    @staticmethod
    def _layers_h2(spec, src2, pos2, q, ref, wk, b_oa_all, l2_all, params, dims):
        B, S, C, nl = dims
        M, L, P = spec.M, spec.L, spec.P
        T = B * S
        P_ = lambda i, j: params[i * N_LAYER + j]
        n_off, n_aw, n_l1 = P_(0, 0).shape[0], P_(0, 2).shape[0], P_(0, 10).shape[0]
        per = n_off + n_aw + 2 * C + n_l1
        x_am = q_am = None
        if q is None and src2.dtype == torch.float32 and pos2.dtype == torch.float32 and C % 4 == 0:
            q, src_c, x_am, q_am = rw.add_rows_amax(src2, pos2, copy_a=cmdbuf.active() is not None)
            src2 = src_c if src_c is not None else src2
        else:
            if q is None:
                assert cmdbuf.active() is None
                q = src2 + pos2
            if cmdbuf.active() is not None:
                src2, q = rw.copy_d2d(torch.empty_like(src2), src2), rw.copy_d2d(torch.empty_like(q), q)
        wk_am = row_amax(wk)
        l2_am = row_amax(l2_all)
        fwd_amax = C // M == 32 and L == 3 and P == 4 and src2.dtype == torch.float32
        zam = torch.zeros((2 * nl if fwd_amax else nl, T), dtype=torch.float32, device=src2.device)
        h_am_all, a_am_all = zam[:nl], (zam[nl:] if fwd_amax else None)
        x = src2
        if x_am is None:
            x_am, q_am = row_amax(src2), row_amax(q)
        saved, saved_am = [], []
        for i in range(nl):
            (so_w, so_b, aw_w, aw_b, vp_w, vp_b, op_w, op_b, n1_w, n1_b, l1_w, l1_b, l2_w, l2_b, n2_w, n2_b) = params[i * N_LAYER:(i + 1) * N_LAYER]
            o = i * per
            w_oa, oa_wam = wk[o:o + n_off + n_aw], wk_am[o:o + n_off + n_aw]
            o += n_off + n_aw
            vp_c, vp_wam = wk[o:o + C], wk_am[o:o + C]
            op_c, op_wam = wk[o + C:o + 2 * C], wk_am[o + C:o + 2 * C]
            l1_c, l1_wam = wk[o + 2 * C:o + 2 * C + n_l1], wk_am[o + 2 * C:o + 2 * C + n_l1]
            value = gemm_tn_h2(x, vp_c, vp_b, a_amax=x_am, b_amax=vp_wam)
            oa = gemm_tn_h2(q, w_oa, b_oa_all[i], a_amax=q_am, b_amax=oa_wam)
            v4 = value.view(B, S, M, C // M)
            fused = fwd_amax and n_off == 2 * n_aw and msda_fused_supported(B, S, M, C // M, L, S, P)
            if fused:
                a_am = a_am_all[i]
                a, stats = _timed("fwd", msda_fused_forward, v4, spec.shapes, spec.lsi, oa, ref, a_am)
                loc6, attn5 = oa, stats
            else:
                loc, attn = msda_prep_fwd(oa[:, :n_off], oa[:, n_off:], ref, spec.shapes, M, L, P)
                loc6, attn5 = loc.view(B, S, M, L, P, 2), attn.view(B, S, M, L, P)
            if fused:
                pass
            elif fwd_amax:
                a_am = a_am_all[i]
                a = _timed("fwd", msda_forward_amax, v4, spec.shapes, spec.lsi, loc6, attn5, spec.im2col_step, a_am).view(T, C)
            else:
                a = _timed("fwd", MSDA.ms_deform_attn_forward, v4, spec.shapes, spec.lsi, loc6, attn5, spec.im2col_step).view(T, C)
                a_am = row_amax(a)
            z1, y1, _, _, m1, r1, y1_am, _ = rw.add_ln_fwd(gemm_tn_h2(a, op_c, op_b, a_amax=a_am, b_amax=op_wam), x, n1_w, n1_b, spec.eps, amax=True)
            h_am = h_am_all[i]
            if h2_bits_supported(T, n_l1):
                h, hbits = gemm_tn_h2(y1, l1_c, l1_b, mode=1, want_bits=True, a_amax=y1_am, b_amax=l1_wam, c_amax=h_am)
            else:
                h, hbits = gemm_tn_h2(y1, l1_c, l1_b, mode=1, a_amax=y1_am, b_amax=l1_wam, c_amax=h_am), None
            ffn2 = gemm_tn_h2(h, l2_all[i * C:(i + 1) * C], l2_b, a_amax=h_am, b_amax=l2_am[i * C:(i + 1) * C])
            last = i == nl - 1
            z2, y2, _, ypos, m2, r2, y2_am, ypos_am = rw.add_ln_fwd(ffn2, y1, n2_w, n2_b, spec.eps, c_dtype=torch.float32,
                                                                     pos=pos2, pos_div=1, want_ypos=not last, amax=True)
            saved.append((x, q, v4, loc6, attn5, a, z1, m1, r1, y1, h, z2, m2, r2, ref if fused else None, hbits))
            saved_am.append((x_am, q_am, a_am, y1_am, h_am))
            x, q, x_am, q_am = y2, ypos, y2_am, ypos_am
        return x, saved, saved_am

    @staticmethod
    def _stack_t(params, nl, j):
        ws = [params[i * N_LAYER + j] for i in range(nl)]
        d = (ws[1].data_ptr() - ws[0].data_ptr()) if nl > 1 else 0
        es = ws[0].element_size()
        if nl > 1 and d != 0 and d % es == 0 and all(w.is_contiguous() and w.shape == ws[0].shape for w in ws) \
                and all(ws[i].data_ptr() - ws[0].data_ptr() == i * d for i in range(nl)) \
                and all(w.untyped_storage().data_ptr() == ws[0].untyped_storage().data_ptr() for w in ws):
            N_, K_ = ws[0].shape
            base = ws[0] if d > 0 else ws[-1]
            return _Stack(torch.as_strided(base, (nl, N_, K_), (abs(d) // es, K_, 1)).transpose(1, 2).contiguous(), d < 0)
        return _Stack(torch.stack(ws).transpose(1, 2).contiguous(), False)

    @staticmethod
    def _stacks_t_one_launch(params, nl, wk, n_oa, per, C):
        import ctypes
        from .. import lib as _lib
        probs, views, total = [], [], 0
        for j in (10, 12, 6, 4):
            ws = [params[i * N_LAYER + j] for i in range(nl)]
            d = (ws[1].data_ptr() - ws[0].data_ptr()) if nl > 1 else 0
            es = ws[0].element_size()
            ok = (ws[0].is_cuda and ws[0].dtype == torch.float32 and all(w.is_contiguous() and w.shape == ws[0].shape for w in ws)
                  and (nl == 1 or (d != 0 and d % es == 0 and all(ws[i].data_ptr() - ws[0].data_ptr() == i * d for i in range(nl)))))
            if not ok:
                return None
            N_, K_ = ws[0].shape
            base = ws[0] if d >= 0 else ws[-1]
            probs.append((base.data_ptr(), abs(d) // es if nl > 1 else N_ * K_, K_, nl, N_, K_, d < 0))
        if not (wk.is_cuda and wk.dtype == torch.float32 and wk.is_contiguous()):
            return None
        probs.append((wk.data_ptr(), per * C, C, nl, n_oa, C, False))
        for p_ in probs:
            total += p_[3] * p_[4] * p_[5]
        buf = torch.empty(total, dtype=torch.float32, device=wk.device)
        descs = (_TrProblem * len(probs))()
        off = 0
        for d_, (src, bs, rs, batch, rows, cols, rev) in zip(descs, probs):
            d_.src, d_.dst, d_.src_batch_stride, d_.src_row_stride = src, buf.data_ptr() + 4 * off, bs, rs
            d_.batch, d_.rows, d_.cols, d_.reserved = batch, rows, cols, 0
            views.append(_Stack(buf[off:off + batch * rows * cols].view(batch, cols, rows), rev))
            off += batch * rows * cols
        _lib.check(_lib.load().pd_transpose_batched_f32(ctypes.byref(descs), len(probs), _lib.current_stream()))
        return views

    @staticmethod
    def _backward_h2(ctx, d_out):
        spec, params = ctx.spec, ctx.params
        B, S, C, nl = ctx.dims
        T = B * S
        need_w = any(ctx.needs_input_grad[3:])
        n_off, n_aw, n_l1 = params[0].shape[0], params[2].shape[0], params[10].shape[0]
        per = n_off + n_aw + 2 * C + n_l1
        wk = ctx.wk
        stacks5 = EncoderCore._stacks_t_one_launch(params, nl, wk, n_off + n_aw, per, C)
        if stacks5 is not None:
            l1_t, l2_t, op_t, vp_t, oa_t = stacks5
        else:
            st = EncoderCore._stack_t
            l1_t, l2_t, op_t, vp_t = st(params, nl, 10), st(params, nl, 12), st(params, nl, 6), st(params, nl, 4)
            oa_t = _Stack(torch.as_strided(wk, (nl, n_off + n_aw, C), (per * C, C, 1)).transpose(1, 2).contiguous(), False)
        dy = d_out.reshape(T, C)
        dy = dy if dy.is_contiguous() else dy.contiguous()
        stacks = (l1_t, l2_t, op_t, vp_t, oa_t)
        ref = spec.ref.reshape(T, spec.L, 2)
        ref = ref if ref.is_contiguous() else ref.contiguous()
        rec_f = getattr(ctx, "rec", None)
        if rec_f is None:
            dy, dy2, dyq, d_pos, grads = EncoderCore._bwd_layers_h2(spec, params, ctx.dims, ctx.saved, ctx.saved_am, dy, stacks, need_w, ref)
        else:
            if rec_f.generation != ctx.rec_gen:
                raise RuntimeError("the fused encoder ran another forward before this backward: the recorded region's activation arena was "
                                   "overwritten (set PD_CMDBUF=0 for graphs that keep several forward passes alive)")
            slots = [dy] + [k.t for k in stacks] + [spec.shapes, spec.lsi, ref] + list(params)
            key = ("bwd", id(rec_f), need_w, tuple(k.rev for k in stacks))
            rec = _RECS.get(key)
            if rec is None or not rec.matches(slots):
                rec = cmdbuf.Recording(slots, "encoder backward", stable=[rec_f])
                with rec:
                    outs = EncoderCore._bwd_layers_h2(spec, params, ctx.dims, ctx.saved, ctx.saved_am, dy, stacks, need_w, ref)
                    outs = outs[:4] + (cmdbuf.Fresh(outs[4]),)
                dy, dy2, dyq, d_pos, grads = rec.finish(outs)
                _RECS.put(key, rec)
            else:
                cmdbuf.unalias_grads(params, rec.owns)
                dy, dy2, dyq, d_pos, grads = rec.replay(slots)
        if all(t_.is_cuda and t_.dtype == torch.float32 and t_.is_contiguous() and t_.numel() == dy.numel() for t_ in (dy, dy2, dyq, d_pos)) \
                and dy.numel() % 4 == 0:
            d_src, d_pos_out = torch.empty_like(dy), torch.empty_like(d_pos)
            _lib.check(_lib.load().pd_sum3_sum2_f32(dy.data_ptr(), dy2.data_ptr(), dyq.data_ptr(), d_pos.data_ptr(), d_src.data_ptr(),
                                                    d_pos_out.data_ptr(), dy.numel(), _lib.current_stream()))
            d_pos = d_pos_out
        else:
            d_pos = d_pos + dyq if rec_f is not None else d_pos.add_(dyq)
            d_src = dy + dy2
            d_src += dyq
        if not need_w:
            grads = [None] * len(grads)
        return (None, d_src.view(B, S, C), d_pos.view(B, S, C), *grads)

    @staticmethod
    def _bwd_layers_h2(spec, params, dims, saved, saved_am, dy, stacks, need_w, ref):
        B, S, C, nl = dims
        M, L, P = spec.M, spec.L, spec.P
        T = B * S
        dev = dy.device
        l1_t, l2_t, op_t, vp_t, oa_t = stacks
        wh2 = H2_WGRAD
        queue = WgradQueue(h2=wh2) if (need_w and GROUP_WGRADS and _gemm.WGRAD_X3) else None
        if not need_w:
            wgrad = lambda *a, **k: None
        elif queue is not None:
            wgrad = (lambda dy_, x_, dw_, db_=None, ya=None, xa=None: queue.add(dy_, x_, dw_, db_, ya if wh2 else None, xa if wh2 else None))
        else:
            wgrad = (lambda dy_, x_, dw_, db_=None, ya=None, xa=None: gemm_wgrad_acc(dy_, x_, dw_, db_, h2=wh2, y_amax=ya if wh2 else None,
                                                                                     x_amax=xa if wh2 else None))
        offs, total = [], 0
        for p in params:
            offs.append(total)
            total += (p.numel() + 3) // 4 * 4
        n_off = params[0].shape[0]
        n_oa = n_off + params[2].shape[0]
        oa_base, oa_per = total, n_oa * C + (n_oa + 3) // 4 * 4
        total += nl * oa_per
        buf = torch.zeros(total, dtype=torch.float32, device=dev)

        def OA(i):
            o = oa_base + i * oa_per
            return buf[o:o + n_oa * C].view(n_oa, C), buf[o + n_oa * C:o + n_oa * C + n_oa]

        def G(i, j):
            p = params[i * N_LAYER + j]
            o = offs[i * N_LAYER + j]
            return buf[o:o + p.numel()].view(p.shape)
        d_pos = torch.zeros((T, C), dtype=torch.float32, device=dev)
        grads = [None] * (nl * N_LAYER)
        t_am = lambda w: _Stack(row_amax(w.t.view(-1, w.t.shape[2])).view(nl, w.t.shape[1]), w.rev)
        l1_tam, l2_tam, op_tam, vp_tam, oa_tam = t_am(l1_t), t_am(l2_t), t_am(op_t), t_am(vp_t), t_am(oa_t)
        dh_am_all = torch.zeros((nl, T), dtype=torch.float32, device=dev)
        dy2 = dyq = None
        for i in reversed(range(nl)):
            n1_w, l1_w, n2_w = params[i * N_LAYER + 8], params[i * N_LAYER + 10], params[i * N_LAYER + 14]
            x, q, v4, loc6, attn5, a, z1, m1, r1, y1, h, z2, m2, r2, fused_ref, hbits = saved[i]
            (g_sow, g_sob, g_aww, g_awb, g_vpw, g_vpb, g_opw, g_opb, g_n1w, g_n1b, g_l1w, g_l1b, g_l2w, g_l2b, g_n2w,
             g_n2b) = [G(i, j) for j in range(N_LAYER)]
            dz2, _, dz2_am = rw.add_ln_bwd(z2, m2, r2, n2_w, dy=dy, dy2=dy2, dypos_c=dyq, dgamma=g_n2w, dbeta=g_n2b, dbias=g_l2b,
                                           dpos_acc=d_pos if dyq is not None else None, pos_div=1, amax=True)
            x_am, q_am, a_am, y1_am, h_am = saved_am[i]
            wgrad(dz2, h, g_l2w, None, dz2_am, h_am)
            if hbits is not None:
                dh = gemm_tn_h2(dz2, l2_t[i], None, mode=2, bits=hbits, colsum=g_l1b, a_amax=dz2_am, b_amax=l2_tam[i], c_amax=dh_am_all[i])
                dh_am = dh_am_all[i]
            else:
                dh = rw.relu_bwd_colsum(gemm_tn_h2(dz2, l2_t[i], a_amax=dz2_am, b_amax=l2_tam[i]), h, g_l1b)
                dh_am = row_amax(dh)
            wgrad(dh, y1, g_l1w, None, dh_am, y1_am)
            dy1 = gemm_tn_h2(dh, l1_t[i], a_amax=dh_am, b_amax=l1_tam[i])
            dz1, _, dz1_am = rw.add_ln_bwd(z1, m1, r1, n1_w, dy=dz2, dy2=dy1, dgamma=g_n1w, dbeta=g_n1b, dbias=g_opb,
                                           out=None if queue is not None else dz2, amax=True)
            wgrad(dz1, a, g_opw, None, dz1_am, a_am)
            da = gemm_tn_h2(dz1, op_t[i], a_amax=dz1_am, b_amax=op_tam[i]).view(B, S, C)
            if fused_ref is not None:
                gv, d_oa, d_oa_am = _timed("bwd", msda_fused_backward, v4, spec.shapes, spec.lsi, loc6, ref, attn5, a, da)
            else:
                gv, gloc, gattn = _timed("bwd", MSDA.ms_deform_attn_backward, v4, spec.shapes, spec.lsi, loc6, attn5, da, spec.im2col_step)
                d_oa = torch.empty((T, n_oa), dtype=torch.float32, device=dev)
            if fused_ref is not None:
                pass
            elif prep_amax_supported(M, L, P):
                d_oa_am = torch.empty(T, dtype=torch.float32, device=dev)
                msda_prep_bwd(gloc, gattn, attn5, spec.shapes, T, M, L, P, out=d_oa, amax=d_oa_am)
            else:
                msda_prep_bwd(gloc, gattn, attn5, spec.shapes, T, M, L, P, out=d_oa)
                d_oa_am = row_amax(d_oa)
            g_oaw, g_oab = OA(i)
            wgrad(d_oa, q, g_oaw, g_oab, d_oa_am, q_am)
            g_sow, g_aww, g_sob, g_awb = g_oaw[:n_off], g_oaw[n_off:], g_oab[:n_off], g_oab[n_off:]
            dq = gemm_tn_h2(d_oa, oa_t[i], a_amax=d_oa_am, b_amax=oa_tam[i])
            gv2 = gv.view(T, C)
            gv_am = row_amax(gv2)
            wgrad(gv2, x, g_vpw, g_vpb, gv_am, x_am)
            dxv = gemm_tn_h2(gv2, vp_t[i], a_amax=gv_am, b_amax=vp_tam[i])
            grads[i * N_LAYER:(i + 1) * N_LAYER] = [g_sow, g_sob, g_aww, g_awb, g_vpw, g_vpb, g_opw, g_opb, g_n1w, g_n1b,
                                                     g_l1w, g_l1b, g_l2w, g_l2b, g_n2w, g_n2b]
            dy, dy2, dyq = dz1, dxv, dq
        if queue is not None:
            queue.flush()
        return dy, dy2, dyq, d_pos, grads

    @staticmethod
    def backward(ctx, d_out):
        if getattr(ctx, "h2", False) and X3_PROJ and USE_X3:
            return EncoderCore._backward_h2(ctx, d_out)
        spec, params = ctx.spec, ctx.params
        B, S, C, nl = ctx.dims
        M, L, P = spec.M, spec.L, spec.P
        T = B * S
        dev = d_out.device
        need_w = any(ctx.needs_input_grad[3:])
        from . import gemm as _gemm
        h2 = getattr(ctx, "h2", False)
        wh2 = h2 and H2_WGRAD
        queue = WgradQueue(h2=wh2) if (need_w and GROUP_WGRADS and _gemm.WGRAD_X3 and d_out.is_cuda) else None
        if not need_w:
            wgrad = lambda *a, **k: None
        elif queue is not None:
            wgrad = (lambda dy_, x_, dw_, db_=None, ya=None, xa=None: queue.add(dy_, x_, dw_, db_, ya if wh2 else None, xa if wh2 else None))
        else:
            wgrad = (lambda dy_, x_, dw_, db_=None, ya=None, xa=None: gemm_wgrad_acc(dy_, x_, dw_, db_, h2=wh2, y_amax=ya if wh2 else None,
                                                                                     x_amax=xa if wh2 else None))
        offs, total = [], 0
        for p in params:
            offs.append(total)
            total += (p.numel() + 3) // 4 * 4
        n_oa = params[0].shape[0] + params[2].shape[0]
        oa_base, oa_per = total, n_oa * C + (n_oa + 3) // 4 * 4
        total += nl * oa_per
        buf = torch.zeros(total, dtype=torch.float32, device=dev)

        def OA(i):
            o = oa_base + i * oa_per
            return buf[o:o + n_oa * C].view(n_oa, C), buf[o + n_oa * C:o + n_oa * C + n_oa]

        def G(i, j):
            p = params[i * N_LAYER + j]
            o = offs[i * N_LAYER + j]
            return buf[o:o + p.numel()].view(p.shape)
        d_pos = torch.zeros((T, C), dtype=torch.float32, device=dev)
        grads = [None] * (nl * N_LAYER)
        def T_all(j):
            ws = [params[i * N_LAYER + j] for i in range(nl)]
            d = (ws[1].data_ptr() - ws[0].data_ptr()) if nl > 1 else 0
            es = ws[0].element_size()
            if nl > 1 and d != 0 and d % es == 0 and all(w.is_contiguous() and w.shape == ws[0].shape for w in ws) \
                    and all(ws[i].data_ptr() - ws[0].data_ptr() == i * d for i in range(nl)) \
                    and all(w.untyped_storage().data_ptr() == ws[0].untyped_storage().data_ptr() for w in ws):
                N_, K_ = ws[0].shape
                base = ws[0] if d > 0 else ws[-1]
                return _Stack(torch.as_strided(base, (nl, N_, K_), (abs(d) // es, K_, 1)).transpose(1, 2).contiguous(), d < 0)
            return _Stack(torch.stack(ws).transpose(1, 2).contiguous(), False)
        l1_t, l2_t = T_all(10), T_all(12)
        op_t, vp_t = (T_all(6), T_all(4)) if X3_PROJ and USE_X3 else (None, None)
        oa_t = _Stack(torch.stack([sv[14] for sv in ctx.saved]).transpose(1, 2).contiguous(), False) if op_t is not None else None
        if h2:
            t_am = lambda w: _Stack(row_amax(w.t.view(-1, w.t.shape[2])).view(nl, w.t.shape[1]), w.rev)
            l1_tam, l2_tam, op_tam, vp_tam, oa_tam = t_am(l1_t), t_am(l2_t), t_am(op_t), t_am(vp_t), t_am(oa_t)
            dh_am_all = torch.zeros((nl, T), dtype=torch.float32, device=dev)
        dy = d_out.reshape(T, C)
        dy = dy if dy.is_contiguous() else dy.contiguous()
        dy2 = dyq = None
        for i in reversed(range(nl)):
            (so_w, so_b, aw_w, aw_b, vp_w, vp_b, op_w, op_b, n1_w, n1_b, l1_w, l1_b, l2_w, l2_b, n2_w, n2_b) = params[i * N_LAYER:(i + 1) * N_LAYER]
            x, q, v4, loc6, attn5, a, z1, m1, r1, y1, h, z2, m2, r2, w_oa, hbits = ctx.saved[i]
            (g_sow, g_sob, g_aww, g_awb, g_vpw, g_vpb, g_opw, g_opb, g_n1w, g_n1b, g_l1w, g_l1b, g_l2w, g_l2b, g_n2w,
             g_n2b) = [G(i, j) for j in range(N_LAYER)]
            dz2, _, dz2_am = rw.add_ln_bwd(z2, m2, r2, n2_w, dy=dy, dy2=dy2, dypos_c=dyq, dgamma=g_n2w, dbeta=g_n2b, dbias=g_l2b,
                                           dpos_acc=d_pos if dyq is not None else None, pos_div=1, amax=True)
            if h2:
                x_am, q_am, a_am, y1_am, h_am = ctx.saved_am[i]
                wgrad(dz2, h, g_l2w, None, dz2_am, h_am)
                if hbits is not None:
                    dh = gemm_tn_h2(dz2, l2_t[i], None, mode=2, bits=hbits, colsum=g_l1b, a_amax=dz2_am, b_amax=l2_tam[i], c_amax=dh_am_all[i])
                    dh_am = dh_am_all[i]
                else:
                    dh = rw.relu_bwd_colsum(gemm_tn_h2(dz2, l2_t[i], a_amax=dz2_am, b_amax=l2_tam[i]), h, g_l1b)
                    dh_am = row_amax(dh)
                wgrad(dh, y1, g_l1w, None, dh_am, y1_am)
                dy1 = gemm_tn_h2(dh, l1_t[i], a_amax=dh_am, b_amax=l1_tam[i])
                del dh
                dz1, _, dz1_am = rw.add_ln_bwd(z1, m1, r1, n1_w, dy=dz2, dy2=dy1, dgamma=g_n1w, dbeta=g_n1b, dbias=g_opb,
                                               out=None if queue is not None else dz2, amax=True)
                wgrad(dz1, a, g_opw, None, dz1_am, a_am)
                da = gemm_tn_h2(dz1, op_t[i], a_amax=dz1_am, b_amax=op_tam[i]).view(B, S, C)
                gv, gloc, gattn = _timed("bwd", MSDA.ms_deform_attn_backward, v4, spec.shapes, spec.lsi, loc6, attn5, da, spec.im2col_step)
                d_oa = torch.empty((T, w_oa.shape[0]), dtype=torch.float32, device=dev)
                if prep_amax_supported(M, L, P):
                    d_oa_am = torch.empty(T, dtype=torch.float32, device=dev)
                    msda_prep_bwd(gloc, gattn, attn5, spec.shapes, T, M, L, P, out=d_oa, amax=d_oa_am)
                else:
                    msda_prep_bwd(gloc, gattn, attn5, spec.shapes, T, M, L, P, out=d_oa)
                    d_oa_am = row_amax(d_oa)
                g_oaw, g_oab = OA(i)
                wgrad(d_oa, q, g_oaw, g_oab, d_oa_am, q_am)
                n_off = so_w.shape[0]
                g_sow, g_aww, g_sob, g_awb = g_oaw[:n_off], g_oaw[n_off:], g_oab[:n_off], g_oab[n_off:]
                dq = gemm_tn_h2(d_oa, oa_t[i], a_amax=d_oa_am, b_amax=oa_tam[i])
                gv2 = gv.view(T, C)
                gv_am = row_amax(gv2)
                wgrad(gv2, x, g_vpw, g_vpb, gv_am, x_am)
                dxv = gemm_tn_h2(gv2, vp_t[i], a_amax=gv_am, b_amax=vp_tam[i])
                grads[i * N_LAYER:(i + 1) * N_LAYER] = [g_sow, g_sob, g_aww, g_awb, g_vpw, g_vpb, g_opw, g_opb, g_n1w, g_n1b,
                                                         g_l1w, g_l1b, g_l2w, g_l2b, g_n2w, g_n2b]
                dy, dy2, dyq = dz1, dxv, dq
                continue
            wgrad(dz2, h, g_l2w)
            pre = hbits is not None and USE_X3 and PRESPLIT and pre_supported(T, l2_w.shape[1], l2_w.shape[0]) and pre_supported(T, l1_w.shape[1], l1_w.shape[0])
            if pre:
                dh = gemm_tn_x3_pre(dz2, split3(l2_w, transpose=True), mode=2, bits=hbits, colsum=g_l1b)
            elif hbits is not None:
                dh = gemm_tn_x3_relumask(dz2, l2_t[i], hbits, g_l1b)
            else:
                dh = rw.relu_bwd_colsum(_ffn_gemm(dz2, l2_t[i]), h, g_l1b)
            wgrad(dh, y1, g_l1w)
            dy1 = gemm_tn_x3_pre(dh, split3(l1_w, transpose=True)) if pre else _ffn_gemm(dh, l1_t[i])
            del dh
            dz1, _ = rw.add_ln_bwd(z1, m1, r1, n1_w, dy=dz2, dy2=dy1, dgamma=g_n1w, dbeta=g_n1b, dbias=g_opb, out=None if queue is not None else dz2)
            wgrad(dz1, a, g_opw)
            da = (_proj(dz1, op_t[i]) if op_t is not None else torch.mm(dz1, op_w)).view(B, S, C)
            gv, gloc, gattn = _timed("bwd", MSDA.ms_deform_attn_backward, v4, spec.shapes, spec.lsi, loc6, attn5, da, spec.im2col_step)
            d_oa = torch.empty((T, w_oa.shape[0]), dtype=torch.float32, device=dev)
            msda_prep_bwd(gloc, gattn, attn5, spec.shapes, T, M, L, P, out=d_oa)
            g_oaw, g_oab = OA(i)
            wgrad(d_oa, q, g_oaw, g_oab)
            n_off = so_w.shape[0]
            g_sow, g_aww, g_sob, g_awb = g_oaw[:n_off], g_oaw[n_off:], g_oab[:n_off], g_oab[n_off:]
            dq = _proj(d_oa, oa_t[i]) if op_t is not None else torch.mm(d_oa, w_oa)
            gv2 = gv.view(T, C)
            wgrad(gv2, x, g_vpw, g_vpb)
            dxv = _proj(gv2, vp_t[i]) if vp_t is not None else torch.mm(gv2, vp_w)
            grads[i * N_LAYER:(i + 1) * N_LAYER] = [g_sow, g_sob, g_aww, g_awb, g_vpw, g_vpb, g_opw, g_opb, g_n1w, g_n1b,
                                                     g_l1w, g_l1b, g_l2w, g_l2b, g_n2w, g_n2b]
            dy, dy2, dyq = dz1, dxv, dq
        if queue is not None:
            queue.flush()
        d_pos += dyq
        d_src = dy + dy2
        d_src += dyq
        if not need_w:
            grads = [None] * len(grads)
        return (None, d_src.view(B, S, C), d_pos.view(B, S, C), *grads)
```

### partdistillation_amd/functions/rowwise.py

```python
import ctypes

import torch
from torch.autograd import Function

from .. import lib as _lib

_DT = {torch.float32: _lib.PD_F32, torch.bfloat16: _lib.PD_BF16}


def _stream():
    return _lib.current_stream()


def _p(t):
    return None if t is None else t.data_ptr()


def _need_cuda(t, who):
    if not t.is_cuda:
        raise RuntimeError(f"{who} runs on the GPU only (no CPU fallback in partdistillation_amd)")


def add_ln_fwd(x, res, gamma, beta, eps, *, want_z=True, want_y=True, c_dtype=None, want_yc=False, pos=None, pos_div=1,
               want_ypos=False, amax=False):
    ref = x if x is not None else res
    _need_cuda(ref, "pd_add_layernorm_fwd")
    rows, C = ref.shape
    dev = ref.device
    assert (x is None or x.is_contiguous()) and (res is None or (res.is_contiguous() and res.dtype == torch.float32))
    assert gamma.dtype == torch.float32 and beta.dtype == torch.float32 and gamma.numel() == C and beta.numel() == C
    z = torch.empty((rows, C), dtype=torch.float32, device=dev) if want_z else None
    y = torch.empty((rows, C), dtype=torch.float32, device=dev) if want_y else None
    y_c = torch.empty((rows, C), dtype=c_dtype, device=dev) if want_yc else None
    ypos_c = torch.empty((rows, C), dtype=c_dtype, device=dev) if want_ypos else None
    stats = torch.empty((2, rows), dtype=torch.float32, device=dev)
    if want_ypos:
        assert pos is not None and pos.dtype == torch.float32 and pos.is_contiguous() and pos.shape[-1] == C
    if amax:
        am = torch.empty((2, rows), dtype=torch.float32, device=dev)
        _lib.check(_lib.load().pd_add_layernorm_fwd_amax(
            _p(x), _DT[x.dtype] if x is not None else 0, _p(res), gamma.data_ptr(), beta.data_ptr(), float(eps), _p(z), _p(y), _p(y_c),
            _p(pos) if want_ypos else None, int(pos_div), _p(ypos_c), _DT[c_dtype] if c_dtype is not None else 0,
            stats[0].data_ptr(), stats[1].data_ptr(), am[0].data_ptr(), am[1].data_ptr() if want_ypos else None, rows, C, _stream()))
        return z, y, y_c, ypos_c, stats[0], stats[1], am[0], (am[1] if want_ypos else None)
    _lib.check(_lib.load().pd_add_layernorm_fwd(
        _p(x), _DT[x.dtype] if x is not None else 0, _p(res), gamma.data_ptr(), beta.data_ptr(), float(eps), _p(z), _p(y), _p(y_c),
        _p(pos) if want_ypos else None, int(pos_div), _p(ypos_c), _DT[c_dtype] if c_dtype is not None else 0,
        stats[0].data_ptr(), stats[1].data_ptr(), rows, C, _stream()))
    return z, y, y_c, ypos_c, stats[0], stats[1]


def add_ln_bwd(z, mean, rstd, gamma, *, dy=None, dy2=None, dy_c=None, dypos_c=None, dz_c_dtype=None, dgamma=None, dbeta=None,
               dbias=None, dpos_acc=None, pos_div=1, out=None, amax=False):
    rows, C = z.shape
    assert z.dtype == torch.float32 and gamma.dtype == torch.float32 and mean.dtype == torch.float32
    cd = None
    for t in (dy_c, dypos_c):
        if t is not None:
            assert t.is_contiguous() and (cd is None or cd == t.dtype)
            cd = t.dtype
    for t in (dy, dy2):
        assert t is None or (t.is_contiguous() and t.dtype == torch.float32)
    dz = out if out is not None else torch.empty((rows, C), dtype=torch.float32, device=z.device)
    dz_c = torch.empty((rows, C), dtype=dz_c_dtype, device=z.device) if dz_c_dtype is not None else None
    if amax:
        am = torch.empty(rows, dtype=torch.float32, device=z.device)
        _lib.check(_lib.load().pd_add_layernorm_bwd_amax(
            _p(dy), _p(dy2), _p(dy_c), _p(dypos_c), _DT[cd] if cd is not None else 0, z.data_ptr(), mean.data_ptr(), rstd.data_ptr(),
            gamma.data_ptr(), dz.data_ptr(), _p(dz_c), _DT[dz_c_dtype] if dz_c_dtype is not None else 0, _p(dgamma), _p(dbeta),
            _p(dbias), _p(dpos_acc), int(pos_div), am.data_ptr(), rows, C, _stream()))
        return dz, dz_c, am
    _lib.check(_lib.load().pd_add_layernorm_bwd(
        _p(dy), _p(dy2), _p(dy_c), _p(dypos_c), _DT[cd] if cd is not None else 0, z.data_ptr(), mean.data_ptr(), rstd.data_ptr(),
        gamma.data_ptr(), dz.data_ptr(), _p(dz_c), _DT[dz_c_dtype] if dz_c_dtype is not None else 0, _p(dgamma), _p(dbeta),
        _p(dbias), _p(dpos_acc), int(pos_div), rows, C, _stream()))
    return dz, dz_c


def copy_d2d(dst, src):
    n = src.numel() * src.element_size()
    assert dst.numel() * dst.element_size() == n and dst.is_contiguous() and src.is_contiguous()
    _lib.check(_lib.load().pd_memcpy_d2d_async(dst.data_ptr(), src.data_ptr(), n, _stream()))
    return dst


class _CopySeg(ctypes.Structure):
    _fields_ = [("src", ctypes.c_void_p), ("dst", ctypes.c_void_p), ("bytes", ctypes.c_int64)]


MAX_COPY_SEGS = 48


def copy_segments(pairs):
    from .. import cmdbuf
    assert 0 < len(pairs) <= MAX_COPY_SEGS
    segs = (_CopySeg * len(pairs))()
    for sgm, (dst, src) in zip(segs, pairs):
        n = src.numel() * src.element_size()
        assert dst.numel() * dst.element_size() == n and dst.is_contiguous() and src.is_contiguous()
        if cmdbuf.active() is not None:
            cmdbuf.require_stable(src.data_ptr(), "source of a grouped copy")
        sgm.src, sgm.dst, sgm.bytes = src.data_ptr(), dst.data_ptr(), n
    _lib.check(_lib.load().pd_copy_segments(segs, len(pairs), _stream()))


def add_rows_amax(a, b, copy_a=False):
    assert a.is_contiguous() and b.is_contiguous() and a.shape == b.shape and a.dtype == torch.float32 and b.dtype == torch.float32 and a.dim() == 2
    q = torch.empty_like(a)
    ac = torch.empty_like(a) if copy_a else None
    am = torch.empty(a.shape[0], dtype=torch.float32, device=a.device)
    qm = torch.empty(a.shape[0], dtype=torch.float32, device=a.device)
    _lib.check(_lib.load().pd_add_rows_amax_f32(a.data_ptr(), b.data_ptr(), q.data_ptr(), ac.data_ptr() if ac is not None else None, am.data_ptr(),
                                                qm.data_ptr(), a.shape[0], a.shape[1], _stream()))
    return q, ac, am, qm


def colsum_acc(x, acc):
    assert x.is_contiguous() and acc.dtype == torch.float32 and acc.numel() == x.shape[1]
    _lib.check(_lib.load().pd_colsum_acc(x.data_ptr(), _DT[x.dtype], x.shape[0], x.shape[1], acc.data_ptr(), _stream()))


def relu_bwd_colsum(dh, h, acc=None):
    assert dh.is_contiguous() and h.is_contiguous() and dh.dtype == h.dtype and dh.shape == h.shape
    _lib.check(_lib.load().pd_relu_bwd_colsum(dh.data_ptr(), h.data_ptr(), _DT[dh.dtype], dh.shape[0], dh.shape[1], _p(acc), _stream()))
    return dh


def _token_view(x):
    B, C, H, W = x.shape
    t = x.permute(0, 2, 3, 1)
    if t.dtype != torch.float32 or t.stride(3) != 1 or t.stride(2) != C or t.stride(1) != W * C:
        t = t.float().contiguous()
    return t, t.stride(0)


def mem_prep_fwd(x, level_embed, pos, c_dtype):
    _need_cuda(x, "pd_mem_prep_fwd")
    B, C, H, W = x.shape
    t, bstride = _token_view(x)
    assert pos.dtype == torch.float32 and pos.is_contiguous() and (level_embed is None or level_embed.dtype == torch.float32)
    mem = torch.empty((H * W * B, C), dtype=c_dtype, device=x.device)
    mempos = torch.empty((H * W * B, C), dtype=c_dtype, device=x.device)
    _lib.check(_lib.load().pd_mem_prep_fwd(t.data_ptr(), bstride, _p(level_embed), pos.data_ptr(), mem.data_ptr(), mempos.data_ptr(),
                                           _DT[c_dtype], B, H * W, C, _stream()))
    return mem, mempos


def mem_prep_bwd(dmem, dmempos, B, H, W, C):
    ref = dmem if dmem is not None else dmempos
    dtok = torch.empty((B, H * W, C), dtype=torch.float32, device=ref.device)
    _lib.check(_lib.load().pd_mem_prep_bwd(_p(dmem), _p(dmempos), _DT[ref.dtype], dtok.data_ptr(), H * W * C, B, H * W, C, _stream()))
    return dtok


def attn_mask_u8(logits):
    _need_cuda(logits, "pd_attn_mask_u8")
    assert logits.is_contiguous()
    n = logits.shape[-1]
    mask = torch.empty(logits.shape, dtype=torch.uint8, device=logits.device)
    _lib.check(_lib.load().pd_attn_mask_u8(logits.data_ptr(), _DT[logits.dtype], logits.numel() // max(n, 1), n, mask.data_ptr(), _stream()))
    return mask


def matcher_point_terms(x, want_f32=True):
    _need_cuda(x, "pd_matcher_point_terms")
    assert x.is_contiguous() and x.dtype in _DT
    n = x.shape[-1]
    rows = x.numel() // max(n, 1)
    xf = torch.empty(x.shape, dtype=torch.float32, device=x.device) if want_f32 else None
    sg = torch.empty(x.shape, dtype=torch.float32, device=x.device)
    if x.numel() == 0:
        z = torch.zeros(x.shape[:-1], dtype=torch.float32, device=x.device)
        return xf, sg, z, z.clone()
    sums = torch.empty((2,) + tuple(x.shape[:-1]), dtype=torch.float32, device=x.device)
    _lib.check(_lib.load().pd_matcher_point_terms(x.data_ptr(), _DT[x.dtype], rows, n, xf.data_ptr() if xf is not None else None, sg.data_ptr(),
                                                  sums[0].data_ptr(), sums[1].data_ptr(), _stream()))
    return xf, sg, sums[0], sums[1]


def point_sample_nhwc(x, coords, out_dtype=torch.float32):
    _need_cuda(x, "pd_point_sample_nhwc_f32")
    B, C, H, W = x.shape
    t = x.permute(0, 2, 3, 1)
    if t.dtype != torch.float32 or not t.is_contiguous():
        t = t.float().contiguous()
    coords = coords.float().contiguous()
    P = coords.shape[1]
    out = torch.empty((B, P, C), dtype=out_dtype, device=x.device)
    fn = _lib.load().pd_point_sample_nhwc_f32_bf16 if out_dtype == torch.bfloat16 else _lib.load().pd_point_sample_nhwc_f32
    assert out_dtype in (torch.float32, torch.bfloat16)
    _lib.check(fn(t.data_ptr(), coords.data_ptr(), out.data_ptr(), B, H, W, C, P, _stream()))
    return out


class PointSamplePlanar(Function):

    @staticmethod
    def forward(ctx, x, coords):
        N, C, H, W = x.shape
        P = coords.shape[1]
        out = torch.empty((N, C, P), dtype=torch.float32, device=x.device)
        _lib.check(_lib.load().pd_point_sample_planar_f32(x.data_ptr(), coords.data_ptr(), out.data_ptr(), N, C, H, W, P, _stream()))
        ctx.save_for_backward(coords)
        ctx.shape = (N, C, H, W)
        return out

    @staticmethod
    def backward(ctx, g):
        (coords,) = ctx.saved_tensors
        N, C, H, W = ctx.shape
        L = _lib.load()
        alloc = torch.zeros if L.pd_point_sample_planar_bwd_needs_zero_n(N, C, H, W) else torch.empty
        gx = alloc((N, C, H, W), dtype=torch.float32, device=g.device)
        g = g.contiguous()
        _lib.check(_lib.load().pd_point_sample_planar_bwd_f32(g.data_ptr(), coords.data_ptr(), gx.data_ptr(), N, C, H, W, coords.shape[1], _stream()))
        return gx, None


def point_sample_planar_supported(x, coords):
    return (x.is_cuda and x.dtype == torch.float32 and x.dim() == 4 and x.is_contiguous() and coords.dtype == torch.float32
            and coords.dim() == 3 and coords.shape[0] == x.shape[0] and coords.shape[2] == 2 and not coords.requires_grad)


def point_sample_planar(x, coords):
    return PointSamplePlanar.apply(x, coords.contiguous())


def resize_bilinear_rows(x, sizes, out_dtype=torch.float32):
    import ctypes
    _need_cuda(x, "pd_resize_bilinear_nhwc_f32")
    B, C, H, W = x.shape
    assert x.dtype == torch.float32 and x.is_contiguous(memory_format=torch.channels_last) and C % 4 == 0 and 0 < len(sizes) <= 4
    outs = [torch.empty((B, h * w, C), dtype=out_dtype, device=x.device) for h, w in sizes]
    hs = (ctypes.c_int * len(sizes))(*[int(h) for h, _ in sizes])
    ws = (ctypes.c_int * len(sizes))(*[int(w) for _, w in sizes])
    ptrs = (ctypes.c_void_p * len(sizes))(*[o.data_ptr() for o in outs])
    _lib.check(_lib.load().pd_resize_bilinear_nhwc_f32(x.data_ptr(), B, H, W, C, hs, ws, ptrs, len(sizes), _DT[out_dtype], _stream()))
    return outs


def resize_bilinear_rows_supported(x, sizes):
    return (x.is_cuda and x.dtype == torch.float32 and x.dim() == 4 and x.shape[1] % 4 == 0 and 0 < len(sizes) <= 4
            and x.is_contiguous(memory_format=torch.channels_last))


def supports_width(C):
    return C % 256 == 0 and C <= 1024


class AddLayerNorm(Function):

    @staticmethod
    def forward(ctx, x, res, gamma, beta, eps, pos):
        ctx.set_materialize_grads(False)
        shape = x.shape
        C = shape[-1]
        x2 = x.reshape(-1, C)
        x2 = x2 if x2.is_contiguous() else x2.contiguous()
        r2 = None
        if res is not None:
            r2 = res.reshape(-1, C)
            r2 = r2 if r2.is_contiguous() else r2.contiguous()
        p2 = None
        if pos is not None:
            p2 = pos.reshape(-1, C)
            p2 = p2 if p2.is_contiguous() else p2.contiguous()
            assert p2.shape[0] == x2.shape[0]
# ... 71 lines not shown
```

### partdistillation_amd/lib.py

```python
import ctypes
import os
import subprocess

_HERE = os.path.dirname(os.path.abspath(__file__))
LIB_PATH = os.environ.get("PD_LIB_PATH") or os.path.join(_HERE, "libpd_hip.so")
CSRC = os.path.join(_HERE, "csrc")

PD_F32, PD_F64, PD_BF16 = 0, 1, 2
ABI_VERSION = 49

_c_int, _c_vp = ctypes.c_int, ctypes.c_void_p

SIGNATURES = {
    "pd_msda_forward": (_c_int, [_c_vp] * 6 + [_c_int] * 9 + [_c_vp]),
    "pd_msda_backward": (_c_int, [_c_vp] * 9 + [_c_int] * 9 + [_c_vp]),
    "pd_msda_backward_last_gate": (_c_int, [_c_vp]),
    "pd_stem7x7_fwd": (_c_int, [_c_vp, _c_int] + [_c_vp] * 4 + [_c_int] * 4 + [_c_vp]),
    "pd_stem_wgrad_workspace_floats": (ctypes.c_int64, []),
    "pd_stem7x7_wgrad": (_c_int, [_c_vp, _c_int] + [_c_vp] * 4 + [_c_int, _c_vp] + [_c_int] * 4 + [_c_vp]),
    "pd_msda_fused_supported": (_c_int, [_c_int] * 7),
    "pd_msda_fused_forward": (_c_int, [_c_vp] * 4 + [_c_int] + [_c_vp] * 4 + [_c_int] * 7 + [_c_vp]),
    "pd_msda_fused_backward": (_c_int, [_c_vp] * 4 + [_c_int] + [_c_vp] * 6 + [_c_int, _c_vp, _c_vp] + [_c_int] * 7 + [_c_vp]),
    "pd_lsa_batched": (_c_int, [_c_vp] * 4 + [_c_int] * 3 + [_c_vp]),
    "pd_sumsq_accumulate": (_c_int, [_c_vp, ctypes.c_int64, _c_int, _c_vp, _c_vp]),
    "pd_adamw_clipped": (_c_int, [_c_vp] * 4 + [ctypes.c_int64, _c_int] + [ctypes.c_double] * 5 + [_c_int, _c_vp, ctypes.c_double, _c_vp, _c_vp]),
    "pd_gemm_tn_f32": (_c_int, [_c_vp] * 4 + [_c_int] * 7 + [_c_vp]),
    "pd_gemm_tn_f32x3": (_c_int, [_c_vp] * 4 + [_c_int] * 7 + [_c_vp]),
    "pd_gemm_wgrad_f16x2_takes_wide_tiles": (_c_int, [_c_int] * 2),
    "pd_gemm_wgrad_f16x2_ws_floats": (ctypes.c_int64, [_c_int] * 2),
    "pd_gemm_wgrad_f16x2_grouped_ws_floats": (ctypes.c_int64, [_c_vp, _c_int]),
    "pd_gemm_wgrad_acc_f16x2_ws": (_c_int, [_c_vp] * 7 + [ctypes.c_int64] + [_c_int] * 6 + [_c_vp]),
    "pd_gemm_wgrad_f16x2_grouped": (_c_int, [_c_vp, _c_int, _c_vp, _c_vp, _c_vp, ctypes.c_int64, _c_vp]),
    "pd_conv3x3_wgrad_nhwc_f16x2": (_c_int, [_c_vp] * 7 + [ctypes.c_int64] + [_c_int] * 5 + [_c_vp]),
    "pd_conv3x3_nhwc_f16x2": (_c_int, [_c_vp] * 7 + [_c_int] * 5 + [_c_vp]),
    "pd_gemm_tn_f16x2_which": (_c_int, [_c_int] * 11),
    "pd_gemm_tn_f16x2_bits_words": (ctypes.c_int64, [_c_int] * 2),
    "pd_gemm_tn_f16x2": (_c_int, [_c_vp] * 9 + [_c_int] * 7 + [_c_vp]),
    "pd_gemm_tn_f16x2_bf16out": (_c_int, [_c_vp] * 6 + [_c_int] * 6 + [_c_vp]),
    "pd_cast_bf16_f32_amax": (_c_int, [_c_vp, _c_int, _c_int, _c_vp, _c_vp, _c_vp]),
    "pd_row_amax_f32": (_c_int, [_c_vp, _c_int, _c_int, _c_int, _c_vp, _c_vp]),
    "pd_gemm_tn_f32x3_relumask": (_c_int, [_c_vp] * 5 + [_c_int] * 6 + [_c_vp]),
    "pd_gemm_tn_f32x3_relu_bits": (_c_int, [_c_vp] * 5 + [_c_int] * 6 + [_c_vp]),
    "pd_gemm_tn_f32x3_relu_bits_words": (ctypes.c_int64, [_c_int] * 2),
    "pd_split3_bf16": (_c_int, [_c_vp, _c_int, _c_int, _c_int, _c_int, _c_vp, _c_vp]),
    "pd_gemm_tn_f32x3_pre": (_c_int, [_c_vp] * 6 + [_c_int] * 6 + [_c_vp]),
    "pd_gemm_wgrad_f32": (_c_int, [_c_vp] * 4 + [_c_int] * 6 + [_c_vp]),
    "pd_gemm_wgrad_acc_f32": (_c_int, [_c_vp] * 4 + [_c_int] * 6 + [_c_vp]),
    "pd_conv3x3_nhwc_f32x3": (_c_int, [_c_vp] * 4 + [_c_int] * 5 + [_c_vp]),
    "pd_gemm_wgrad_acc_f32x3": (_c_int, [_c_vp] * 4 + [_c_int] * 6 + [_c_vp]),
    "pd_conv3x3_wgrad_nhwc_f32x3": (_c_int, [_c_vp] * 5 + [ctypes.c_int64] + [_c_int] * 5 + [_c_vp]),
    "pd_gemm_wgrad_f32x3_ws_floats": (ctypes.c_int64, [_c_int] * 2),
    "pd_gemm_wgrad_f32x3_grouped_table_bytes": (ctypes.c_int64, [_c_int]),
    "pd_gemm_wgrad_f32x3_grouped_ws_floats": (ctypes.c_int64, [_c_vp, _c_int]),
    "pd_gemm_wgrad_f32x3_grouped": (_c_int, [_c_vp, _c_int, _c_vp, _c_vp, _c_vp, ctypes.c_int64, _c_vp]),
    "pd_gemm_wgrad_acc_f32x3_ws": (_c_int, [_c_vp] * 5 + [ctypes.c_int64] + [_c_int] * 6 + [_c_vp]),
    "pd_adamw_clipped_shadow": (_c_int, [_c_vp] * 5 + [ctypes.c_int64] + [ctypes.c_double] * 5 + [_c_int, _c_vp, ctypes.c_double, _c_vp, _c_vp]),
    "pd_conv_bf16_supported": (_c_int, [_c_int] * 5),
    "pd_conv_bf16_fwd": (_c_int, [_c_vp] * 6 + [_c_int] * 11 + [_c_vp]),
    "pd_conv_bf16_wgrad_workspace_floats": (ctypes.c_int64, [_c_int] * 6),
    "pd_conv_bf16_wgrad": (_c_int, [_c_vp] * 4 + [ctypes.c_int64] + [_c_int] * 10 + [_c_vp]),
    "pd_conv_bf16_wgrad_grouped_table_bytes": (ctypes.c_int64, [_c_int]),
    "pd_conv_bf16_wgrad_grouped_workspace_floats": (ctypes.c_int64, [_c_vp, _c_int]),
    "pd_conv_bf16_wgrad_grouped": (_c_int, [_c_vp, _c_int, _c_vp, _c_vp, _c_vp, ctypes.c_int64, _c_vp]),
    "pd_conv_bf16_dgrad": (_c_int, [_c_vp] * 4 + [_c_int] * 10 + [_c_vp]),
    "pd_maxpool3s2_fwd_bf16": (_c_int, [_c_vp] * 3 + [_c_int] * 4 + [_c_vp]),
    "pd_maxpool3s2_bwd_bf16": (_c_int, [_c_vp] * 3 + [_c_int] * 4 + [_c_vp]),
    "pd_affine_act_fwd_bf16": (_c_int, [_c_vp] * 5 + [ctypes.c_int64, _c_int, _c_int, _c_vp]),
    "pd_affine_act_bwd_bf16": (_c_int, [_c_vp] * 5 + [ctypes.c_int64, _c_int, _c_int, _c_vp]),
    "pd_affine_act_bwd2_bf16": (_c_int, [_c_vp] * 6 + [ctypes.c_int64, _c_int, _c_int, _c_vp]),
    "pd_multi_gather_sumsq": (_c_int, [_c_vp] * 8 + [_c_int, _c_int, _c_vp]),
    "pd_attn_workspace_floats": (ctypes.c_int64, [_c_int] * 4),
    "pd_attn_fwd_d32": (_c_int, [_c_vp] * 7 + [_c_int] * 4 + [ctypes.c_float, _c_int, _c_vp]),
    "pd_attn_bwd_d32": (_c_int, [_c_vp] * 11 + [_c_int] * 4 + [ctypes.c_float, _c_int, _c_vp]),
    "pd_attn_fwd_d32_ld": (_c_int, [_c_vp] * 7 + [_c_int] * 4 + [ctypes.c_float, _c_int, _c_int, _c_vp]),
    "pd_attn_bwd_d32_ld": (_c_int, [_c_vp] * 11 + [_c_int] * 4 + [ctypes.c_float, _c_int, _c_int, _c_vp]),
    "pd_nc_sums_f32": (_c_int, [_c_vp] * 6 + [_c_int] * 5 + [_c_vp]),
    "pd_nc_affine_f32": (_c_int, [_c_vp] * 4 + [_c_int] * 4 + [_c_vp]),
    "pd_nc_affine_amax_f32": (_c_int, [_c_vp] * 5 + [_c_int] * 4 + [_c_vp]),
    "pd_nc_affine2_amax_f32": (_c_int, [_c_vp] * 8 + [_c_int] * 4 + [_c_vp]),
    "pd_upsample_add_amax_nhwc_f32": (_c_int, [_c_vp, ctypes.c_int64] + [_c_vp] * 3 + [_c_int] * 6 + [_c_vp]),
    "pd_nc_affine2_f32": (_c_int, [_c_vp] * 7 + [_c_int] * 4 + [_c_vp]),
    "pd_add_layernorm_fwd": (_c_int, [_c_vp, _c_int, _c_vp, _c_vp, _c_vp, ctypes.c_float, _c_vp, _c_vp, _c_vp, _c_vp, _c_int, _c_vp,
                                      _c_int, _c_vp, _c_vp, _c_int, _c_int, _c_vp]),
    "pd_add_layernorm_bwd": (_c_int, [_c_vp] * 4 + [_c_int] + [_c_vp] * 6 + [_c_int] + [_c_vp] * 4 + [_c_int] * 3 + [_c_vp]),
    "pd_add_layernorm_fwd_amax": (_c_int, [_c_vp, _c_int, _c_vp, _c_vp, _c_vp, ctypes.c_float, _c_vp, _c_vp, _c_vp, _c_vp, _c_int, _c_vp,
                                           _c_int, _c_vp, _c_vp, _c_vp, _c_vp, _c_int, _c_int, _c_vp]),
    "pd_add_layernorm_bwd_amax": (_c_int, [_c_vp] * 4 + [_c_int] + [_c_vp] * 6 + [_c_int] + [_c_vp] * 4 + [_c_int] + [_c_vp] + [_c_int] * 2 + [_c_vp]),
    "pd_colsum_acc": (_c_int, [_c_vp, _c_int, _c_int, _c_int, _c_vp, _c_vp]),
    "pd_relu_bwd_colsum": (_c_int, [_c_vp, _c_vp, _c_int, _c_int, _c_int, _c_vp, _c_vp]),
    "pd_mem_prep_fwd": (_c_int, [_c_vp, ctypes.c_int64, _c_vp, _c_vp, _c_vp, _c_vp, _c_int, _c_int, _c_int, _c_int, _c_vp]),
    "pd_mem_prep_bwd": (_c_int, [_c_vp, _c_vp, _c_int, _c_vp, ctypes.c_int64, _c_int, _c_int, _c_int, _c_vp]),
    "pd_attn_mask_u8": (_c_int, [_c_vp, _c_int, _c_int, _c_int, _c_vp, _c_vp]),
    "pd_add_rows_amax_f32": (_c_int, [_c_vp] * 6 + [_c_int, _c_int, _c_vp]),
    "pd_sum3_sum2_f32": (_c_int, [_c_vp] * 6 + [ctypes.c_int64, _c_vp]),
    "pd_transpose_batched_f32": (_c_int, [_c_vp, _c_int, _c_vp]),
    "pd_normalize_u8_nhwc": (_c_int, [_c_vp, _c_int, _c_int, _c_int, _c_vp, _c_vp, _c_vp, _c_vp]),
    "pd_resize_bilinear_nhwc_f32": (_c_int, [_c_vp] + [_c_int] * 4 + [_c_vp] * 3 + [_c_int, _c_int, _c_vp]),
    "pd_matcher_point_terms": (_c_int, [_c_vp, _c_int, _c_int, _c_int, _c_vp, _c_vp, _c_vp, _c_vp, _c_vp]),
    "pd_match_point_logits": (_c_int, [_c_vp] * 4 + [_c_int] * 7 + [_c_vp]),
    "pd_matcher_costs": (_c_int, [_c_vp, _c_int, _c_vp] + [ctypes.c_int64] * 3 + [_c_vp] * 3 + [_c_int] * 6 + [ctypes.c_float] * 3 + [_c_vp]),
    "pd_mask_point_losses_fwd": (_c_int, [_c_vp] * 5 + [_c_int, _c_int, _c_vp]),
    "pd_mask_point_losses_bwd": (_c_int, [_c_vp] * 6 + [_c_int, _c_int, _c_vp]),
    "pd_uncertain_points": (_c_int, [_c_vp] * 4 + [_c_int] * 4 + [_c_vp]),
    "pd_point_sample_u8": (_c_int, [_c_vp] * 4 + [_c_int] * 5 + [_c_vp]),
    "pd_skinny_linear_fwd": (_c_int, [_c_vp] * 3 + [_c_int, _c_vp] + [_c_int] * 3 + [_c_vp]),
    "pd_skinny_linear_partial_floats": (ctypes.c_int64, [_c_int] * 3),
    "pd_skinny_linear_bwd": (_c_int, [_c_vp, _c_vp, _c_int, _c_vp, _c_vp, _c_vp, _c_int, _c_vp, _c_vp, _c_vp] + [_c_int] * 4 + [_c_vp]),
    "pd_loss_vectors_fwd": (_c_int, [_c_vp, ctypes.c_int64, ctypes.c_int64] + [_c_vp] * 9 + [_c_int] * 5 + [_c_vp]),
    "pd_loss_vectors_bwd": (_c_int, [_c_vp, ctypes.c_int64, ctypes.c_int64] + [_c_vp] * 10 + [_c_int] * 5 + [_c_vp]),
    "pd_pair_logits_fwd": (_c_int, [_c_vp] * 5 + [_c_int] * 4 + [_c_vp]),
    "pd_pair_logits_bwd_tok": (_c_int, [_c_vp] * 5 + [_c_int] * 4 + [_c_vp]),
    "pd_pair_logits_workspace_floats": (ctypes.c_int64, [_c_int] * 3),
    "pd_pair_logits_bwd_rows": (_c_int, [_c_vp] * 6 + [_c_int] * 4 + [_c_vp]),
    "pd_msda_prep_fwd": (_c_int, [_c_vp] * 6 + [ctypes.c_int64] + [_c_int] * 5 + [_c_vp]),
    "pd_msda_prep_bwd_amax": (_c_int, [_c_vp] * 7 + [ctypes.c_int64] + [_c_int] * 5 + [_c_vp]),
    "pd_msda_forward_amax": (_c_int, [_c_vp] * 7 + [_c_int] * 9 + [_c_vp]),
    "pd_msda_prep_bwd": (_c_int, [_c_vp] * 6 + [ctypes.c_int64] + [_c_int] * 5 + [_c_vp]),
    "pd_sgemm_tn_batched_bf16": (_c_int, [_c_vp] * 3 + [_c_int] * 7 + [ctypes.c_int64] * 3 + [_c_vp]),
    "pd_sgemm_tn_multi_bf16": (_c_int, [_c_vp, _c_int, _c_int, _c_vp]),
    "pd_decoder_head_bf16": (_c_int, [_c_vp] * 3 + [ctypes.c_float] + [_c_vp] * 10 + [_c_int] * 4 + [_c_vp]),
    "pd_dec_fwd_a": (_c_int, [_c_vp] * 3 + [_c_int] + [_c_vp] * 4 + [ctypes.c_float] + [_c_vp] * 10 + [_c_int] + [_c_vp]),
    "pd_dec_fwd_b": (_c_int, [_c_vp] * 3 + [_c_int] + [_c_vp] * 20 + [ctypes.c_float] + [_c_vp] * 13 + [_c_int] * 2 + [_c_vp]),
    "pd_dec_bwd_b": (_c_int, [_c_vp] * 14 + [_c_int] + [_c_vp] * 15 + [_c_int] + [_c_vp]),
    "pd_dec_split": (_c_int, []),
    "pd_dec_workspace_bytes": (ctypes.c_int64, [_c_int]),
    "pd_dec_pack_table_bytes": (ctypes.c_int64, [_c_int]),
    "pd_dec_pack_grouped": (_c_int, [_c_vp, _c_int, _c_vp, _c_vp, _c_vp]),
    "pd_dec_bwd_a": (_c_int, [_c_vp] * 11 + [_c_int] + [_c_vp] * 4 + [_c_int] + [_c_vp]),
    "pd_sgemm_split_workspace_floats": (ctypes.c_int64, [_c_int] * 3),
    "pd_sgemm_split_tickets": (ctypes.c_int64, [_c_int] * 2),
    "pd_sgemm_tn_splitk_bf16": (_c_int, [_c_vp] * 5 + [ctypes.c_int64, _c_vp] + [_c_int] * 7 + [_c_vp]),
    "pd_sgemm_nn_splitn_bf16": (_c_int, [_c_vp] * 5 + [ctypes.c_int64, _c_vp] + [_c_int] * 7 + [_c_vp]),
    "pd_sgemm_tn_bf16": (_c_int, [_c_vp] * 4 + [_c_int] * 7 + [_c_vp]),
    "pd_sgemm_nn_bf16": (_c_int, [_c_vp] * 4 + [_c_int] * 7 + [_c_vp]),
    "pd_sgemm_wgrad_bf16": (_c_int, [_c_vp] * 4 + [_c_int] * 6 + [_c_vp]),
    "pd_gn_coeffs_fwd": (_c_int, [_c_vp] * 3 + [_c_int] * 4 + [ctypes.c_float] + [_c_vp] * 6),
    "pd_gn_coeffs_bwd": (_c_int, [_c_vp] * 4 + [_c_int] * 4 + [_c_vp] * 6),
    "pd_point_sample_nhwc_f32": (_c_int, [_c_vp] * 3 + [_c_int] * 5 + [_c_vp]),
    "pd_point_sample_nhwc_f32_bf16": (_c_int, [_c_vp] * 3 + [_c_int] * 5 + [_c_vp]),
    "pd_point_sample_planar_f32": (_c_int, [_c_vp] * 3 + [_c_int] * 5 + [_c_vp]),
    "pd_point_sample_planar_bwd_needs_zero": (_c_int, [_c_int] * 3),
    "pd_point_sample_planar_bwd_needs_zero_n": (_c_int, [_c_int] * 4),
    "pd_point_sample_planar_bwd_f32": (_c_int, [_c_vp] * 3 + [_c_int] * 5 + [_c_vp]),
    "pd_upsample_add_nhwc_f32": (_c_int, [_c_vp, ctypes.c_int64] + [_c_vp] * 2 + [_c_int] * 6 + [_c_vp]),
    "pd_upsample2x_bwd_nhwc_f32": (_c_int, [_c_vp] * 2 + [_c_int] * 4 + [_c_vp]),
    "pd_scores_argmax_u8": (_c_int, [_c_vp] * 3 + [_c_int] * 7 + [_c_vp]),
    "pd_kmeans_assign": (_c_int, [_c_vp, _c_vp, _c_int] + [_c_vp] * 7 + [_c_int, _c_int, _c_vp]),
    "pd_kmeans_assign_partial": (_c_int, [_c_vp, _c_vp, _c_int] + [_c_vp] * 7 + [_c_int, _c_int, _c_vp]),
    "pd_kmeans_reduce": (_c_int, [_c_vp] * 6 + [_c_int] * 3 + [_c_vp]),
    "pd_kmeans_reduce_update_scratch_floats": (ctypes.c_int64, [_c_int] * 3),
    "pd_kmeans_reduce_update": (_c_int, [_c_vp] * 11 + [_c_int] * 3 + [_c_vp]),
    "pd_kmeans_assign_bounded": (_c_int, [_c_vp, _c_vp, _c_int] + [_c_vp] * 11 + [_c_int, _c_int, _c_vp]),
    "pd_kmeans_reduce_update_shift": (_c_int, [_c_vp] * 12 + [_c_int] * 3 + [_c_vp]),
    "pd_kmeans_update": (_c_int, [_c_vp] * 8 + [_c_int] * 3 + [_c_vp]),
    "pd_mask_assign": (_c_int, [_c_vp] * 6 + [_c_int] * 7 + [_c_vp]),
    "pd_window_attn_fwd_w12": (_c_int, [_c_vp] * 6 + [_c_int] * 3 + [ctypes.c_float, _c_vp, _c_vp, _c_int, _c_vp]),
    "pd_window_attn_bwd_w12": (_c_int, [_c_vp] * 9 + [_c_int] * 3 + [ctypes.c_float, _c_vp, _c_vp, _c_int, _c_vp]),
    "pd_window_attn_fwd_w7": (_c_int, [_c_vp] * 6 + [_c_int] * 3 + [ctypes.c_float, _c_vp]),
    "pd_window_attn_bwd_w7": (_c_int, [_c_vp] * 9 + [_c_int] * 3 + [ctypes.c_float, _c_vp]),
    "pd_layernorm_rows_f32_fwd": (_c_int, [_c_vp] * 3 + [ctypes.c_float] + [_c_vp] * 3 + [ctypes.c_int64, _c_int, _c_vp]),
    "pd_layernorm_rows_f32_bwd": (_c_int, [_c_vp] * 8 + [ctypes.c_int64, _c_int, _c_vp]),
    "pd_swin_tail_ln_fwd": (_c_int, [_c_vp] * 3 + [_c_int] + [_c_vp] * 2 + [ctypes.c_float] + [_c_vp] * 4 + [ctypes.c_int64, _c_int, _c_vp]),
    "pd_swin_tail_ln_bwd": (_c_int, [_c_vp] * 7 + [_c_int] + [_c_vp] * 4 + [ctypes.c_int64, _c_int, _c_vp]),
    "pd_swin_merge_ln_fwd": (_c_int, [_c_vp] * 3 + [ctypes.c_float] + [_c_vp] * 3 + [_c_int] * 4 + [_c_vp]),
    "pd_swin_merge_ln_bwd": (_c_int, [_c_vp] * 8 + [_c_int] * 4 + [_c_vp]),
    "pd_swin_ln_fwd": (_c_int, [_c_vp, _c_vp, _c_vp, _c_int, _c_vp, _c_vp, _c_vp, ctypes.c_float, _c_vp, _c_vp, _c_vp, _c_int, _c_vp,
                                _c_int, _c_vp, _c_vp, _c_int, _c_int, _c_int, _c_vp, _c_vp, _c_int, _c_vp]),
    "pd_swin_ln_bwd": (_c_int, [_c_vp, _c_vp, _c_int, _c_vp, _c_vp, _c_vp, _c_vp, _c_vp, _c_vp, _c_vp, _c_vp, _c_int, _c_vp, _c_vp,
                                _c_int, _c_vp, _c_vp, _c_int, _c_int, _c_int, _c_vp, _c_vp, _c_int, _c_int, ctypes.c_int64, _c_vp]),
    "pd_resample_rows_u8": (_c_int, [_c_vp] + [_c_int] * 6 + [_c_vp] * 3 + [_c_int, _c_int, _c_vp, _c_vp]),
    "pd_resample_cols_u8": (_c_int, [_c_vp] + [_c_int] * 3 + [_c_vp] * 3 + [_c_int] * 5 + [_c_vp, _c_vp]),
    "pd_resample_cols_canvas_u8": (_c_int, [_c_vp] + [_c_int] * 3 + [_c_vp] * 3 + [_c_int] * 7 + [_c_vp, _c_vp]),
    "pd_rle_sample_u8": (_c_int, [_c_vp, _c_vp] + [_c_int] * 4 + [_c_vp, _c_vp] + [_c_int] * 3 + [_c_vp, _c_vp, _c_vp]),
    "pd_rle_sample_groups_u8": (_c_int, [_c_vp, _c_vp] + [_c_int] * 3 + [_c_vp, _c_vp] + [_c_int] * 2 + [_c_vp, _c_vp, _c_int] + [_c_vp] * 4),
    "pd_rle_sample_groups_canvas_u8": (_c_int, [_c_vp, _c_vp] + [_c_int] * 3 + [_c_vp, _c_vp] + [_c_int] * 4 + [_c_vp, _c_vp, _c_int] + [_c_vp] * 4),
    "pd_poly_crossings_i32": (_c_int, [_c_vp, _c_vp] + [_c_int] * 3 + [_c_vp] * 3),
    "pd_sgemm_wgrad_grouped_table_bytes": (ctypes.c_int64, [_c_int]),
    "pd_sgemm_wgrad_grouped_bf16": (_c_int, [_c_vp, _c_int, _c_vp, _c_vp, _c_vp]),
    "pd_sgemm_wgrad_split_workspace": (ctypes.c_int64, [_c_int] * 3),
    "pd_sgemm_wgrad_split_bf16": (_c_int, [_c_vp] * 5 + [_c_int] * 6 + [_c_vp]),
    "pd_igemm_bf16_supported": (_c_int, [_c_int] * 5),
    "pd_igemm_bf16_workspace_bytes": (ctypes.c_int64, [_c_vp]),
    "pd_igemm_bf16": (_c_int, [_c_vp, _c_vp, ctypes.c_int64, _c_vp]),
    "pd_igemm_bf16_time": (_c_int, [_c_vp, _c_vp, ctypes.c_int64, _c_int, _c_vp, _c_vp]),
    "pd_igemm_bf16_seq_workspace_bytes": (ctypes.c_int64, [_c_vp, _c_int]),
    "pd_igemm_bf16_seq": (_c_int, [_c_vp, _c_int, _c_vp, ctypes.c_int64, _c_vp]),
    "pd_wgrad_bf16_workspace_bytes": (ctypes.c_int64, [_c_vp]),
    "pd_wgrad_bf16": (_c_int, [_c_vp, _c_vp, ctypes.c_int64, _c_vp]),
    "pd_wgrad_bf16_seq_workspace_bytes": (ctypes.c_int64, [_c_vp, _c_int]),
    "pd_wgrad_bf16_seq": (_c_int, [_c_vp, _c_int, _c_vp, ctypes.c_int64, _c_vp]),
    "pd_wgrad_bf16_time": (_c_int, [_c_vp, _c_vp, ctypes.c_int64, _c_int, _c_vp, _c_vp]),
    "pd_mx8_quantize_bf16": (_c_int, [_c_vp, ctypes.c_int64, _c_int, ctypes.c_int64, _c_int, _c_vp, _c_vp, _c_vp]),
    "pd_mx8_quantize_table_bytes": (ctypes.c_int64, [_c_int]),
    "pd_mx8_quantize_grouped": (_c_int, [_c_vp, _c_int, _c_int, _c_vp, _c_vp, _c_vp]),
    "pd_mx8_gemm": (_c_int, [_c_vp, _c_vp]),
    "pd_mx8_gemm_supported": (_c_int, [_c_int] * 3),
    "pd_filter_transpose_table_bytes": (ctypes.c_int64, [_c_int]),
    "pd_filter_transpose_grouped": (_c_int, [_c_vp, _c_int, _c_vp, _c_vp, _c_vp]),
    "pd_eval_table_bytes": (ctypes.c_int64, [_c_int]),
    "pd_eval_pack_grouped": (_c_int, [_c_vp, _c_int, _c_vp, _c_vp, _c_vp]),
    "pd_eval_intersect_grouped": (_c_int, [_c_vp, _c_int, _c_vp, _c_vp, _c_vp]),
    "pd_eval_confusion_grouped": (_c_int, [_c_vp, _c_int, _c_int, _c_vp, _c_int, _c_vp, _c_vp, _c_vp]),
    "pd_eval_recall_grouped": (_c_int, [_c_vp, _c_int] + [_c_vp] * 6),
    "pd_grouping_table_bytes": (ctypes.c_int64, [_c_int]),
    "pd_scores_argmax_resized_u8": (_c_int, [_c_vp, _c_int, _c_vp, _c_vp, _c_vp]),
    "pd_masks_resize_u8": (_c_int, [_c_vp, _c_int, _c_vp, _c_vp, _c_vp]),
    "pd_assign_table_bytes": (ctypes.c_int64, [_c_int]),
    "pd_mask_assign_resized": (_c_int, [_c_vp, _c_int, _c_vp, _c_vp, _c_vp]),
    "pd_assign_histogram": (_c_int, [_c_vp, _c_int, _c_vp, _c_vp, _c_vp]),
    "pd_dcrf_prepare": (_c_int, [_c_vp, _c_vp] + [_c_int] * 3 + [ctypes.c_double] * 4 + [_c_vp] * 5),
    "pd_dcrf_spatial_message": (_c_int, [_c_vp, _c_vp] + [_c_int] * 3 + [ctypes.c_double] * 2 + [_c_vp] * 3),
    "pd_dcrf_bilateral_update": (_c_int, [_c_vp] * 5 + [_c_int] * 3 + [ctypes.c_double] * 4 + [_c_vp, _c_vp]),
    "pd_dcrf_argmax": (_c_int, [_c_vp] + [_c_int] * 3 + [_c_vp, _c_vp]),
    "pd_rle_seg_rows": (_c_int, []),
    "pd_rle_runs_workspace_bytes": (ctypes.c_int64, [_c_int] * 3),
    "pd_rle_plane_runs": (_c_int, [_c_vp, ctypes.c_int64] + [_c_int] * 5 + [_c_vp] * 6),
    "pd_rle_decode": (_c_int, [_c_vp, _c_vp] + [_c_int] * 3 + [_c_vp, _c_vp, _c_vp]),
    "pd_cmd_fn_index": (_c_int, [ctypes.c_char_p]),
    "pd_cmd_fn_nargs": (_c_int, [_c_int]),
    "pd_cmd_replay": (_c_int, [_c_vp, _c_int, _c_vp, _c_int, _c_vp]),
    "pd_memset_async": (_c_int, [_c_vp, _c_int, ctypes.c_int64, _c_vp]),
    "pd_memcpy_d2d_async": (_c_int, [_c_vp, _c_vp, ctypes.c_int64, _c_vp]),
    "pd_copy_segments": (_c_int, [_c_vp, _c_int, _c_vp]),
    "pd_last_error": (ctypes.c_char_p, []),
    "pd_abi_version": (_c_int, []),
    "pd_debug_set": (_c_int, [ctypes.c_char_p, _c_int]),
    "pd_debug_get": (_c_int, [ctypes.c_char_p, _c_vp]),
}

_lib = None
_PROXY = None


class PdHipError(RuntimeError):
    pass


def build(force=False, verbose=False):
    args = ["make", "-C", CSRC, "-j4"] + (["-B"] if force else [])
    out = subprocess.run(args, stdout=subprocess.PIPE, stderr=subprocess.STDOUT, text=True)
# ... 49 lines not shown
```

### partdistillation_amd/modeling/pixel_decoder/msdeformattn.py

```python
from typing import Callable, Dict, List, Optional, Union

import numpy as np
import torch
import torch.nn.functional as F
from torch import nn
from torch.nn.init import normal_

from ...compat import SEM_SEG_HEADS_REGISTRY, ShapeSpec, configurable
from ...compat.layers import Conv2d, c2_xavier_fill, get_norm
from ..transformer_decoder.position_encoding import PositionEmbeddingSine
from ...functions import conv_x3
from ...functions.fused import group_norm_nhwc, group_norm_nhwc_supported
from ...functions.gemm import linear_f32
from .ops.modules import MSDeformAttn
from ...functions.encoder_core import EncoderCore, EncoderSpec
from ...functions.rowwise import supports_width, upsample_add, upsample_add_supported


class MSDeformAttnTransformerEncoderLayer(nn.Module):
    def __init__(self, d_model=256, d_ffn=1024, dropout=0.1, activation="relu", n_levels=4, n_heads=8, n_points=4):
        super().__init__()
        assert activation == "relu"
        self.self_attn = MSDeformAttn(d_model, n_levels, n_heads, n_points)
        self.dropout1 = nn.Dropout(dropout)
        self.norm1 = nn.LayerNorm(d_model)
        self.linear1 = nn.Linear(d_model, d_ffn)
        self.dropout2 = nn.Dropout(dropout)
        self.linear2 = nn.Linear(d_ffn, d_model)
        self.dropout3 = nn.Dropout(dropout)
        self.norm2 = nn.LayerNorm(d_model)

    def forward(self, src, pos, reference_points, spatial_shapes, level_start_index, padding_mask=None):
        q = src if pos is None else src + pos
        attn = self.self_attn(q, reference_points, src, spatial_shapes, level_start_index, padding_mask)
        src = self.norm1(src + self.dropout1(attn))
        lin = MSDeformAttn._linear
        if self.dropout2.p == 0.0 and src.dtype == torch.float32 and src.is_cuda and not torch.is_autocast_enabled():
            hidden = linear_f32(src, self.linear1.weight, self.linear1.bias, True)
        else:
            hidden = self.dropout2(F.relu(self.linear1(src)))
        ffn = lin(self.linear2, hidden)
        return self.norm2(src + self.dropout3(ffn))


class MSDeformAttnTransformerEncoder(nn.Module):
    def __init__(self, encoder_layer_factory, num_layers):
        super().__init__()
        self.layers = nn.ModuleList([encoder_layer_factory() for _ in range(num_layers)])
        self.num_layers = num_layers
        self._ref_cache = {}

    @staticmethod
    def get_reference_points(spatial_shapes, valid_ratios, device):
        refs = []
        for lvl, (H_, W_) in enumerate(spatial_shapes):
            H_, W_ = int(H_), int(W_)
            ry, rx = torch.meshgrid(torch.linspace(0.5, H_ - 0.5, H_, dtype=torch.float32, device=device),
                                    torch.linspace(0.5, W_ - 0.5, W_, dtype=torch.float32, device=device), indexing="ij")
            ry = ry.reshape(-1)[None] / (valid_ratios[:, None, lvl, 1] * H_)
            rx = rx.reshape(-1)[None] / (valid_ratios[:, None, lvl, 0] * W_)
            refs.append(torch.stack((rx, ry), -1))
        ref = torch.cat(refs, 1)
        return ref[:, :, None] * valid_ratios[:, None]

    def forward(self, src, spatial_shapes, level_start_index, valid_ratios, pos=None, padding_mask=None,
                shapes_host=None):
        key = (tuple(map(tuple, shapes_host)), src.shape[0], str(src.device)) if shapes_host is not None else None
        if key is not None and key in self._ref_cache:
            reference_points = self._ref_cache[key]
        else:
            reference_points = self.get_reference_points(shapes_host or spatial_shapes.tolist(), valid_ratios, src.device)
            if key is not None:
                self._ref_cache[key] = reference_points
        if self._fused_ok(src, pos, reference_points, padding_mask):
            l0 = self.layers[0]
            spec = EncoderSpec(l0.self_attn.n_heads, l0.self_attn.n_levels, l0.self_attn.n_points, l0.norm1.eps,
                               l0.self_attn.im2col_step, reference_points, spatial_shapes, level_start_index)
            return EncoderCore.apply(spec, src, pos, *self._core_params())
        out = src
        for layer in self.layers:
            out = layer(out, pos, reference_points, spatial_shapes, level_start_index, padding_mask)
        return out

    fused_core = True

    def _fused_ok(self, src, pos, reference_points, padding_mask):
        if not (self.fused_core and self.num_layers and src.is_cuda and src.dtype == torch.float32 and pos is not None
                and padding_mask is None and reference_points.shape[-1] == 2 and not torch.is_autocast_enabled("cuda")):
            return False
        l0 = self.layers[0]
        if self.training and any(d.p > 0 for l in self.layers for d in (l.dropout1, l.dropout2, l.dropout3)):
            return False
        return (supports_width(src.shape[-1]) and l0.linear1.out_features % 128 == 0
                and all(p.dtype == torch.float32 for p in l0.parameters()))

    def _core_params(self):
        p = []
        for l in self.layers:
            a = l.self_attn
            p += [a.sampling_offsets.weight, a.sampling_offsets.bias, a.attention_weights.weight, a.attention_weights.bias,
                  a.value_proj.weight, a.value_proj.bias, a.output_proj.weight, a.output_proj.bias, l.norm1.weight, l.norm1.bias,
                  l.linear1.weight, l.linear1.bias, l.linear2.weight, l.linear2.bias, l.norm2.weight, l.norm2.bias]
        return p


class LevelPos(torch.autograd.Function):

    @staticmethod
    def forward(ctx, level_embed, *pos_embeds):
        ctx.sizes = [int(p.shape[2] * p.shape[3]) for p in pos_embeds]
        B, C = pos_embeds[0].shape[:2]
        out = torch.empty((B, sum(ctx.sizes), C), dtype=pos_embeds[0].dtype, device=pos_embeds[0].device)
        flat = None
        if all(p.stride(0) == 0 for p in pos_embeds):
            key = tuple((p.data_ptr(), tuple(p.shape)) for p in pos_embeds)
            hit = LevelPos._flat.get(key)
            if hit is None:
                if len(LevelPos._flat) >= 8:
                    LevelPos._flat.clear()
                hit = LevelPos._flat[key] = (torch.cat([p[0].flatten(1).t() for p in pos_embeds]).contiguous(), pos_embeds)
            flat = hit[0]
        o = 0
        for i, (p, n) in enumerate(zip(pos_embeds, ctx.sizes)):
            a = flat[o:o + n].unsqueeze(0).expand(B, -1, -1) if flat is not None else p.flatten(2).transpose(1, 2)
            torch.add(a, level_embed[i].view(1, 1, -1), out=out[:, o:o + n])
            o += n
        return out

    _flat = {}

    @staticmethod
    def backward(ctx, d_pos):
        from ...functions.rowwise import colsum_acc
        d_pos = d_pos if d_pos.is_contiguous() else d_pos.contiguous()
        B, S, C = d_pos.shape
        d_le = torch.zeros((len(ctx.sizes), C), dtype=torch.float32, device=d_pos.device)
        start = 0
        for l, n in enumerate(ctx.sizes):
            for b in range(B):
                colsum_acc(d_pos[b, start:start + n], d_le[l])
            start += n
        return (d_le,) + (None,) * len(ctx.sizes)


class CatLevels(torch.autograd.Function):

    @staticmethod
    def forward(ctx, *srcs):
        ctx.shapes = [tuple(s.shape) for s in srcs]
        B, C = srcs[0].shape[:2]
        sizes = [s.shape[2] * s.shape[3] for s in srcs]
        out = torch.empty((B, sum(sizes), C), dtype=srcs[0].dtype, device=srcs[0].device)
        o = 0
        for s_, n in zip(srcs, sizes):
            out[:, o:o + n].copy_(s_.flatten(2).transpose(1, 2))
            o += n
        return out

    @staticmethod
    def backward(ctx, g):
        outs, o = [], 0
        for (B, C, h, w) in ctx.shapes:
            outs.append(g[:, o:o + h * w].transpose(1, 2).reshape(B, C, h, w))
            o += h * w
        return tuple(outs)


class MSDeformAttnTransformerEncoderOnly(nn.Module):
    def __init__(self, d_model=256, nhead=8, num_encoder_layers=6, dim_feedforward=1024, dropout=0.1,
                 activation="relu", num_feature_levels=4, enc_n_points=4):
        super().__init__()
        self.d_model, self.nhead = d_model, nhead
        self.encoder = MSDeformAttnTransformerEncoder(
            lambda: MSDeformAttnTransformerEncoderLayer(d_model, dim_feedforward, dropout, activation,
                                                        num_feature_levels, nhead, enc_n_points), num_encoder_layers)
        self.level_embed = nn.Parameter(torch.Tensor(num_feature_levels, d_model))
        self._shape_cache = {}
        self._reset_parameters()

    def _reset_parameters(self):
        for p in self.parameters():
            if p.dim() > 1:
                nn.init.xavier_uniform_(p)
        for m in self.modules():
            if isinstance(m, MSDeformAttn):
                m._reset_parameters()
        normal_(self.level_embed)

    def forward(self, srcs, pos_embeds):
        shapes_host = [(int(s.shape[2]), int(s.shape[3])) for s in srcs]
        key = (tuple(shapes_host), str(srcs[0].device))
        if key not in self._shape_cache:
            sh = torch.as_tensor(shapes_host, dtype=torch.long, device=srcs[0].device)
            self._shape_cache[key] = (sh, torch.cat((sh.new_zeros((1,)), sh.prod(1).cumsum(0)[:-1])))
        spatial_shapes, level_start_index = self._shape_cache[key]
        if srcs[0].is_cuda:
            src = CatLevels.apply(*srcs)
        else:
            src = torch.cat([s.flatten(2).transpose(1, 2) for s in srcs], 1)
        if src.is_cuda and src.dtype == torch.float32 and self.level_embed.dtype == torch.float32 and self.d_model % 128 == 0:
            pos = LevelPos.apply(self.level_embed, *pos_embeds)
        else:
            pos = torch.cat([p.flatten(2).transpose(1, 2) + self.level_embed[i].view(1, 1, -1)
                             for i, p in enumerate(pos_embeds)], 1)
        valid_ratios = src.new_ones((src.shape[0], len(srcs), 2))
        memory = self.encoder(src, spatial_shapes, level_start_index, valid_ratios, pos, None, shapes_host=shapes_host)
        return memory, spatial_shapes, level_start_index, shapes_host


CONV_X3 = bool(int(__import__("os").environ.get("PD_CONV_X3", "1")))


def _as_fp32_input(x, conv):
    if x.dtype == torch.bfloat16 and CONV_X3 and conv_x3.conv1x1_supported(x, conv) and x.requires_grad:
        return x
    return x.float()


def _conv_gn(conv, gn, x, relu=False):
    if CONV_X3 and conv_x3.supported(x, conv):
        y = conv_x3.conv3x3(x, conv.weight, conv.bias)
    elif CONV_X3 and conv_x3.conv1x1_supported(x, conv):
        y = conv_x3.conv1x1(x, conv.weight, conv.bias)
    else:
        y = F.conv2d(x, conv.weight, conv.bias, conv.stride, conv.padding, conv.dilation, conv.groups)
    if isinstance(gn, nn.GroupNorm) and group_norm_nhwc_supported(y, gn.num_groups):
        return group_norm_nhwc(y, gn.weight, gn.bias, gn.num_groups, gn.eps, relu)
    if gn is not None:
        y = gn(y)
    return F.relu(y) if relu else y


@SEM_SEG_HEADS_REGISTRY.register()
class MSDeformAttnPixelDecoder(nn.Module):
    @configurable
    def __init__(self, input_shape: Dict[str, ShapeSpec], *, transformer_dropout: float, transformer_nheads: int,
                 transformer_dim_feedforward: int, transformer_enc_layers: int, conv_dim: int, mask_dim: int,
                 norm: Optional[Union[str, Callable]] = None, transformer_in_features: List[str], common_stride: int):
        super().__init__()
        tf_shape = {k: v for k, v in input_shape.items() if k in transformer_in_features}
        by_stride = sorted(input_shape.items(), key=lambda kv: kv[1].stride)
        self.in_features = [k for k, _ in by_stride]
        self.feature_strides = [v.stride for _, v in by_stride]
        self.feature_channels = [v.channels for _, v in by_stride]
        tf_by_stride = sorted(tf_shape.items(), key=lambda kv: kv[1].stride)
        self.transformer_in_features = [k for k, _ in tf_by_stride]
        tf_channels = [v.channels for _, v in tf_by_stride]
        self.transformer_feature_strides = [v.stride for _, v in tf_by_stride]
        self.transformer_num_feature_levels = len(self.transformer_in_features)
        chans = tf_channels[::-1] if self.transformer_num_feature_levels > 1 else [tf_channels[-1]]
        self.input_proj = nn.ModuleList(
            [nn.Sequential(nn.Conv2d(c, conv_dim, kernel_size=1), nn.GroupNorm(32, conv_dim)) for c in chans])
        for proj in self.input_proj:
            nn.init.xavier_uniform_(proj[0].weight, gain=1)
            nn.init.constant_(proj[0].bias, 0)
        self.transformer = MSDeformAttnTransformerEncoderOnly(
            d_model=conv_dim, dropout=transformer_dropout, nhead=transformer_nheads,
            dim_feedforward=transformer_dim_feedforward, num_encoder_layers=transformer_enc_layers,
            num_feature_levels=self.transformer_num_feature_levels)
        self.pe_layer = PositionEmbeddingSine(conv_dim // 2, normalize=True)
        self.mask_dim = mask_dim
        self.mask_features = Conv2d(conv_dim, mask_dim, kernel_size=1, stride=1, padding=0)
        c2_xavier_fill(self.mask_features)
        self.maskformer_num_feature_levels = 3
        self.common_stride = common_stride
        self.num_fpn_levels = int(np.log2(min(self.transformer_feature_strides)) - np.log2(self.common_stride))
        lateral_convs, output_convs = [], []
        use_bias = norm == ""
        for idx, in_channels in enumerate(self.feature_channels[: self.num_fpn_levels]):
            lateral = Conv2d(in_channels, conv_dim, kernel_size=1, bias=use_bias, norm=get_norm(norm, conv_dim))
            output = Conv2d(conv_dim, conv_dim, kernel_size=3, stride=1, padding=1, bias=use_bias,
                            norm=get_norm(norm, conv_dim), activation=F.relu)
            c2_xavier_fill(lateral)
            c2_xavier_fill(output)
            self.add_module(f"adapter_{idx + 1}", lateral)
            self.add_module(f"layer_{idx + 1}", output)
            lateral_convs.append(lateral)
            output_convs.append(output)
        self.lateral_convs = lateral_convs[::-1]
        self.output_convs = output_convs[::-1]

    @classmethod
    def from_config(cls, cfg, input_shape: Dict[str, ShapeSpec]):
        head = cfg.MODEL.SEM_SEG_HEAD
        return dict(
            input_shape={k: v for k, v in input_shape.items() if k in head.IN_FEATURES},
            conv_dim=head.CONVS_DIM, mask_dim=head.MASK_DIM, norm=head.NORM,
            transformer_dropout=cfg.MODEL.MASK_FORMER.DROPOUT, transformer_nheads=cfg.MODEL.MASK_FORMER.NHEADS,
            transformer_dim_feedforward=1024,
            transformer_enc_layers=head.TRANSFORMER_ENC_LAYERS,
            transformer_in_features=head.DEFORMABLE_TRANSFORMER_ENCODER_IN_FEATURES,
            common_stride=head.COMMON_STRIDE)

    def forward_features(self, features):
        with torch.autocast(device_type=next(iter(features.values())).device.type, enabled=False):
            srcs, pos = [], []
            for idx, f in enumerate(self.transformer_in_features[::-1]):
                x = _as_fp32_input(features[f], self.input_proj[idx][0])
                srcs.append(_conv_gn(self.input_proj[idx][0], self.input_proj[idx][1], x))
                pos.append(self.pe_layer(x))
            y, spatial_shapes, level_start_index, shapes_host = self.transformer(srcs, pos)
            bs = y.shape[0]
            sizes = [h * w for h, w in shapes_host]
            out = [z.transpose(1, 2).reshape(bs, -1, h, w) for z, (h, w) in zip(torch.split(y, sizes, dim=1), shapes_host)]
            for idx, f in enumerate(self.in_features[: self.num_fpn_levels][::-1]):
                x = _as_fp32_input(features[f], self.lateral_convs[idx])
                lat, outc = self.lateral_convs[idx], self.output_convs[idx]
                cur = _conv_gn(lat, lat.norm, x, relu=lat.activation is not None)
                if upsample_add_supported(out[-1], cur):
                    y = upsample_add(out[-1], cur)
                else:
                    y = cur + F.interpolate(out[-1], size=cur.shape[-2:], mode="bilinear", align_corners=False)
                out.append(_conv_gn(outc, outc.norm, y, relu=outc.activation is not None))
            multi_scale = out[: self.maskformer_num_feature_levels]
            mf = self.mask_features
            if CONV_X3 and mf.norm is None and mf.activation is None and conv_x3.conv1x1_supported(out[-1], mf):
                return conv_x3.conv1x1(out[-1], mf.weight, mf.bias), out[0], multi_scale
            return mf(out[-1]), out[0], multi_scale
```

Measured before the change: 110.1.

## Fuse level-embed gradient reduction into encoder backward layernorm and sum kernels

Moves the level_embed gradient into the fused encoder autograd node. The per-level column sums of the positional gradient are accumulated inside the add-layernorm backward kernel and a new sum3 kernel, using shared-memory level buckets and atomics, instead of accumulating a full per-token dpos tensor and reducing it through LevelPos backward. This aims to remove the extra read and write of the positional-gradient tensor and the separate reduction launches. In exchange it adds shared-memory atomics and an ABI bump, and the generic path is limited to the fused encoder.

```diff
diff --git a/include/pd_rowwise.h b/include/pd_rowwise.h
--- a/include/pd_rowwise.h
+++ b/include/pd_rowwise.h
@@ -23,6 +23,16 @@
                               const float *z, const float *mean, const float *rstd, const float *gamma, float *dz, void *dz_c,
                               int dzc_dtype, float *dgamma, float *dbeta, float *dbias, float *dpos_acc, int pos_div,
                               float *dz_amax, int rows, int C, void *stream);
+
+#define PD_LEVEL_SUMS_MAX 4
+int pd_add_layernorm_bwd_levels_amax(const float *dy, const float *dy2, const void *dy_c, const void *dypos_c, int c_dtype,
+                                     const float *z, const float *mean, const float *rstd, const float *gamma, float *dz, void *dz_c,
+                                     int dzc_dtype, float *dgamma, float *dbeta, float *dbias, float *level_acc,
+                                     const int64_t *level_start, int levels, int tokens_per_image, float *dz_amax, int rows, int C,
+                                     void *stream);
+
+int pd_sum3_levels_f32(const float *a, const float *b, const float *c, float *out, float *level_acc, const int64_t *level_start, int levels,
+                       int tokens_per_image, int rows, int C, void *stream);
 
 int pd_colsum_acc(const void *x, int dtype, int rows, int N, float *acc, void *stream);
 
diff --git a/partdistillation_amd/csrc/cmdbuf.hip b/partdistillation_amd/csrc/cmdbuf.hip
--- a/partdistillation_amd/csrc/cmdbuf.hip
+++ b/partdistillation_amd/csrc/cmdbuf.hip
@@ -59,6 +59,7 @@
   PD_E(pd_adamw_clipped_shadow),
   PD_E(pd_add_layernorm_bwd),
   PD_E(pd_add_layernorm_bwd_amax),
+  PD_E(pd_add_layernorm_bwd_levels_amax),
   PD_E(pd_add_layernorm_fwd),
   PD_E(pd_add_layernorm_fwd_amax),
   PD_E(pd_add_rows_amax_f32),
@@ -185,6 +186,7 @@
   PD_E(pd_split3_bf16),
   PD_E(pd_stem7x7_fwd),
   PD_E(pd_stem7x7_wgrad),
+  PD_E(pd_sum3_levels_f32),
   PD_E(pd_sum3_sum2_f32),
   PD_E(pd_sumsq_accumulate),
   PD_E(pd_swin_ln_bwd),
diff --git a/partdistillation_amd/csrc/common.hip b/partdistillation_amd/csrc/common.hip
--- a/partdistillation_amd/csrc/common.hip
+++ b/partdistillation_amd/csrc/common.hip
@@ -27,7 +27,7 @@
 }
 
 extern "C" const char *pd_last_error(void) { return g_err; }
-extern "C" int pd_abi_version(void) { return 49; }
+extern "C" int pd_abi_version(void) { return 50; }
 
 extern int g_pd_dbg_atomic_scope;
 extern int g_pd_dbg_force_generic;
diff --git a/partdistillation_amd/csrc/rowwise.hip b/partdistillation_amd/csrc/rowwise.hip
--- a/partdistillation_amd/csrc/rowwise.hip
+++ b/partdistillation_amd/csrc/rowwise.hip
@@ -123,25 +123,67 @@
   }
 }
 
-template <int NV4, typename CT, typename DT, int WAVES>
+struct LevelMap {
+  const int64_t *start;
+  int levels, tokens;
+};
+
+__device__ __forceinline__ int level_of(int r, int tokens, int s1, int s2, int s3)
+{
+  const int t = r % tokens;
+  return (int)(t >= s1) + (int)(t >= s2) + (int)(t >= s3);
+}
+
+template <int NV4>
+__device__ __forceinline__ void level_flush(float *lv, int lane, float4 (&acc)[NV4])
+{
+#pragma unroll
+  for (int j = 0; j < NV4; ++j) {
+    float *p = lv + j * 256 + lane * 4;
+    atomicAdd(p, acc[j].x); atomicAdd(p + 1, acc[j].y); atomicAdd(p + 2, acc[j].z); atomicAdd(p + 3, acc[j].w);
+    acc[j] = make_float4(0.f, 0.f, 0.f, 0.f);
+  }
+}
+
+template <int NV4, typename CT, typename DT, int WAVES, bool LVL = false>
 __global__ __launch_bounds__(64 * WAVES) void add_ln_bwd(const float *dy, const float *__restrict__ dy2,
                                                   const CT *__restrict__ dy_c, const CT *__restrict__ dypos_c,
                                                   const float *__restrict__ z, const float *__restrict__ mean,
                                                   const float *__restrict__ rstd, const float *__restrict__ gamma,
                                                   float *dz, DT *__restrict__ dz_c, float *__restrict__ dgamma,
                                                   float *__restrict__ dbeta, float *__restrict__ dbias,
-                                                  float *__restrict__ dpos_acc, int pos_div, int rows, float *__restrict__ dz_amax)
+                                                  float *__restrict__ dpos_acc, int pos_div, int rows, float *__restrict__ dz_amax,
+                                                  LevelMap lm, float *__restrict__ lvl_acc)
 {
   constexpr int C = NV4 * 256;
   __shared__ float red[WAVES][3][C];
+  __shared__ float lv[LVL ? PD_LEVEL_SUMS_MAX : 1][C];
   const int wave = threadIdx.x >> 6, lane = threadIdx.x & 63;
   float4 gm[NV4], ag[NV4], ab[NV4], ad[NV4];
+  float4 ap[LVL ? NV4 : 1];
+  int cur = -1, s1 = 0x7fffffff, s2 = 0x7fffffff, s3 = 0x7fffffff;
+  if constexpr (LVL) {
+    for (int i = threadIdx.x; i < PD_LEVEL_SUMS_MAX * C; i += 64 * WAVES) (&lv[0][0])[i] = 0.f;
+    if (lm.levels > 1) s1 = (int)lm.start[1];
+    if (lm.levels > 2) s2 = (int)lm.start[2];
+    if (lm.levels > 3) s3 = (int)lm.start[3];
+#pragma unroll
+    for (int j = 0; j < NV4; ++j) ap[j] = make_float4(0.f, 0.f, 0.f, 0.f);
+    __syncthreads();
+  }
 #pragma unroll
   for (int j = 0; j < NV4; ++j) {
     gm[j] = ld4(gamma + j * 256 + lane * 4);
     ag[j] = ab[j] = ad[j] = make_float4(0.f, 0.f, 0.f, 0.f);
   }
   for (int r = blockIdx.x * WAVES + wave; r < rows; r += gridDim.x * WAVES) {
+    if constexpr (LVL) {
+      const int l = level_of(r, lm.tokens, s1, s2, s3);
+      if (l != cur) {
+        if (cur >= 0) level_flush<NV4>(lv[cur], lane, ap);
+        cur = l;
+      }
+    }
     const int64_t base = (int64_t)r * C + lane * 4;
     const float mu = mean[r], rs = rstd[r];
     float4 g[NV4], xh[NV4];
@@ -155,7 +197,8 @@
       if (dypos_c) {
         const float4 p = ld4(dypos_c + base + j * 256);
         t = add4(t, p);
-        if (dpos_acc) {
+        if constexpr (LVL) ap[j] = add4(ap[j], p);
+        else if (dpos_acc) {
           float *a = dpos_acc + (int64_t)(r / pos_div) * C + j * 256 + lane * 4;
           if (pos_div == 1) st4(a, add4(ld4(a), p));
           else { atomicAdd(a, p.x); atomicAdd(a + 1, p.y); atomicAdd(a + 2, p.z); atomicAdd(a + 3, p.w); }
@@ -185,6 +228,11 @@
       mz = fmaxf(mz, amax4(o));
     }
     if (dz_amax) { mz = wave_max(mz); if (lane == 0) dz_amax[r] = mz; }
+  }
+  if constexpr (LVL) {
+    if (cur >= 0) level_flush<NV4>(lv[cur], lane, ap);
+    __syncthreads();
+    for (int i = threadIdx.x; i < lm.levels * C; i += 64 * WAVES) atomicAdd(lvl_acc + i, (&lv[0][0])[i]);
   }
   if (!dgamma && !dbeta && !dbias) return;
 #pragma unroll
@@ -862,6 +910,60 @@
   }
 }
 
+template <int NV4, int WAVES>
+__global__ __launch_bounds__(64 * WAVES) void sum3_levels_f32(const float *__restrict__ a, const float *__restrict__ b, const float *__restrict__ c,
+                                                              float *__restrict__ out, float *__restrict__ lvl_acc, LevelMap lm, int rows)
+{
+  constexpr int C = NV4 * 256;
+  __shared__ float lv[PD_LEVEL_SUMS_MAX][C];
+  const int wave = threadIdx.x >> 6, lane = threadIdx.x & 63;
+  for (int i = threadIdx.x; i < PD_LEVEL_SUMS_MAX * C; i += 64 * WAVES) (&lv[0][0])[i] = 0.f;
+  int cur = -1, s1 = 0x7fffffff, s2 = 0x7fffffff, s3 = 0x7fffffff;
+  if (lm.levels > 1) s1 = (int)lm.start[1];
+  if (lm.levels > 2) s2 = (int)lm.start[2];
+  if (lm.levels > 3) s3 = (int)lm.start[3];
+  float4 ap[NV4];
+#pragma unroll
+  for (int j = 0; j < NV4; ++j) ap[j] = make_float4(0.f, 0.f, 0.f, 0.f);
+  __syncthreads();
+  const int stride = gridDim.x * WAVES;
+  auto row = [&](int r, const float4 (&x)[NV4], const float4 (&y)[NV4], const float4 (&w)[NV4]) {
+    const int l = level_of(r, lm.tokens, s1, s2, s3);
+    if (l != cur) {
+      if (cur >= 0) level_flush<NV4>(lv[cur], lane, ap);
+      cur = l;
+    }
+    const int64_t base = (int64_t)r * C + lane * 4;
+#pragma unroll
+    for (int j = 0; j < NV4; ++j) {
+      st4(out + base + j * 256, make_float4((x[j].x + y[j].x) + w[j].x, (x[j].y + y[j].y) + w[j].y, (x[j].z + y[j].z) + w[j].z, (x[j].w + y[j].w) + w[j].w));
+      ap[j] = add4(ap[j], w[j]);
+    }
+  };
+  int r = blockIdx.x * WAVES + wave;
+  for (; r + stride < rows; r += 2 * stride) {
+    const int64_t b0 = (int64_t)r * C + lane * 4, b1 = (int64_t)(r + stride) * C + lane * 4;
+    float4 x0[NV4], y0[NV4], w0[NV4], x1[NV4], y1[NV4], w1[NV4];
+#pragma unroll
+    for (int j = 0; j < NV4; ++j) {
+      x0[j] = ld4(a + b0 + j * 256); y0[j] = ld4(b + b0 + j * 256); w0[j] = ld4(c + b0 + j * 256);
+      x1[j] = ld4(a + b1 + j * 256); y1[j] = ld4(b + b1 + j * 256); w1[j] = ld4(c + b1 + j * 256);
+    }
+    row(r, x0, y0, w0);
+    row(r + stride, x1, y1, w1);
+  }
+  if (r < rows) {
+    const int64_t b0 = (int64_t)r * C + lane * 4;
+    float4 x0[NV4], y0[NV4], w0[NV4];
+#pragma unroll
+    for (int j = 0; j < NV4; ++j) { x0[j] = ld4(a + b0 + j * 256); y0[j] = ld4(b + b0 + j * 256); w0[j] = ld4(c + b0 + j * 256); }
+    row(r, x0, y0, w0);
+  }
+  if (cur >= 0) level_flush<NV4>(lv[cur], lane, ap);
+  __syncthreads();
+  for (int i = threadIdx.x; i < lm.levels * C; i += 64 * WAVES) atomicAdd(lvl_acc + i, (&lv[0][0])[i]);
+}
+
 bool dt_ok(int dt) { return dt == PD_F32 || dt == PD_BF16; }
 
 }
@@ -914,9 +1016,13 @@
 static int add_layernorm_bwd(const float *dy, const float *dy2, const void *dy_c, const void *dypos_c, int c_dtype,
                              const float *z, const float *mean, const float *rstd, const float *gamma, float *dz,
                              void *dz_c, int dzc_dtype, float *dgamma, float *dbeta, float *dbias, float *dpos_acc,
-                             int pos_div, int rows, int C, void *stream_, float *dz_amax)
+                             int pos_div, int rows, int C, void *stream_, float *dz_amax, float *lvl_acc = nullptr,
+                             LevelMap lm = LevelMap{nullptr, 0, 0})
 {
   if (rows < 0 || C <= 0 || (C % 256)) return pd_set_error(PD_ERR_INVALID_ARG, "pd_add_layernorm_bwd: rows=%d C=%d", rows, C);
+  if (lvl_acc && (!lm.start || lm.levels < 1 || lm.levels > PD_LEVEL_SUMS_MAX || lm.tokens <= 0 || !dypos_c || dpos_acc))
+    return pd_set_error(PD_ERR_INVALID_ARG, "pd_add_layernorm_bwd_levels_amax: levels=%d (1 .. %d) tokens_per_image=%d, needs level_start and dypos_c",
+                        lm.levels, PD_LEVEL_SUMS_MAX, lm.tokens);
   if (rows == 0) return PD_OK;
   if ((!dy && !dy2 && !dy_c && !dypos_c) || !z || !mean || !rstd || !gamma || !dz)
     return pd_set_error(PD_ERR_INVALID_ARG, "pd_add_layernorm_bwd: null pointer");
@@ -924,9 +1030,11 @@
   if (dpos_acc && pos_div <= 0) return pd_set_error(PD_ERR_INVALID_ARG, "pd_add_layernorm_bwd: pos_div");
   hipStream_t s = (hipStream_t)stream_;
   const bool cb = c_dtype == PD_BF16, db = dzc_dtype == PD_BF16;
-#define LAUNCH(CT, DT, WV) hipLaunchKernelGGL((add_ln_bwd<NV4, CT, DT, WV>), g, b, 0, s, dy, dy2, (const CT *)dy_c, (const CT *)dypos_c, z, mean, rstd, gamma, dz, (DT *)dz_c, dgamma, dbeta, dbias, dpos_acc, pos_div, rows, dz_amax)
+#define LAUNCH(CT, DT, WV) hipLaunchKernelGGL((add_ln_bwd<NV4, CT, DT, WV>), g, b, 0, s, dy, dy2, (const CT *)dy_c, (const CT *)dypos_c, z, mean, rstd, gamma, dz, (DT *)dz_c, dgamma, dbeta, dbias, dpos_acc, pos_div, rows, dz_amax, LevelMap{nullptr, 0, 0}, (float *)nullptr)
+#define LAUNCH_LVL(WV) hipLaunchKernelGGL((add_ln_bwd<NV4, float, float, WV, true>), g, b, 0, s, dy, dy2, (const float *)dy_c, (const float *)dypos_c, z, mean, rstd, gamma, dz, (float *)nullptr, dgamma, dbeta, dbias, (float *)nullptr, 1, rows, dz_amax, lm, lvl_acc)
 #define LAUNCH_W(WV)                                                                    \
-  if (cb) { if (db) LAUNCH(bf16_t, bf16_t, WV); else LAUNCH(bf16_t, float, WV); }      \
+  if (lvl_acc) LAUNCH_LVL(WV);                                                          \
+  else if (cb) { if (db) LAUNCH(bf16_t, bf16_t, WV); else LAUNCH(bf16_t, float, WV); } \
   else { if (db) LAUNCH(float, bf16_t, WV); else LAUNCH(float, float, WV); }
   NV4_SWITCH(C, {
     constexpr int FAT = NV4 == 1 ? 16 : NV4 == 2 ? 8 : 4;
@@ -962,6 +1070,36 @@
 {
   return add_layernorm_bwd(dy, dy2, dy_c, dypos_c, c_dtype, z, mean, rstd, gamma, dz, dz_c, dzc_dtype, dgamma, dbeta, dbias, dpos_acc, pos_div, rows, C,
                            stream_, dz_amax);
+}
+
+extern "C" int pd_add_layernorm_bwd_levels_amax(const float *dy, const float *dy2, const void *dy_c, const void *dypos_c, int c_dtype,
+                                                const float *z, const float *mean, const float *rstd, const float *gamma, float *dz,
+                                                void *dz_c, int dzc_dtype, float *dgamma, float *dbeta, float *dbias, float *level_acc,
+                                                const int64_t *level_start, int levels, int tokens_per_image, float *dz_amax, int rows, int C,
+                                                void *stream_)
+{
+  if (!level_acc) return pd_set_error(PD_ERR_INVALID_ARG, "pd_add_layernorm_bwd_levels_amax: level_acc is null");
+  if (c_dtype != PD_F32 || dz_c) return pd_set_error(PD_ERR_INVALID_ARG, "pd_add_layernorm_bwd_levels_amax: fp32 terms, no dz_c");
+  return add_layernorm_bwd(dy, dy2, dy_c, dypos_c, c_dtype, z, mean, rstd, gamma, dz, nullptr, dzc_dtype, dgamma, dbeta, dbias, nullptr, 1, rows, C,
+                           stream_, dz_amax, level_acc, LevelMap{level_start, levels, tokens_per_image});
+}
+
+extern "C" int pd_sum3_levels_f32(const float *a, const float *b, const float *c, float *out, float *level_acc, const int64_t *level_start,
+                                  int levels, int tokens_per_image, int rows, int C, void *stream_)
+{
+  if (rows < 0 || rows > 0x7fff0000 || C <= 0 || (C % 256) || C > 1024) return pd_set_error(PD_ERR_INVALID_ARG, "pd_sum3_levels_f32: rows=%d C=%d", rows, C);
+  if (levels < 1 || levels > PD_LEVEL_SUMS_MAX || tokens_per_image <= 0)
+    return pd_set_error(PD_ERR_INVALID_ARG, "pd_sum3_levels_f32: levels=%d (1 .. %d) tokens_per_image=%d", levels, PD_LEVEL_SUMS_MAX, tokens_per_image);
+  if (rows == 0) return PD_OK;
+  if (!a || !b || !c || !out || !level_acc || !level_start || (((uintptr_t)a | (uintptr_t)b | (uintptr_t)c | (uintptr_t)out) & 15))
+    return pd_set_error(PD_ERR_INVALID_ARG, "pd_sum3_levels_f32: null / misaligned pointer");
+  const LevelMap lm{level_start, levels, tokens_per_image};
+  NV4_SWITCH(C, {
+    constexpr int WV = NV4 == 1 ? 16 : NV4 == 2 ? 8 : 4;
+    const dim3 g(max(1, min(256, (rows + 4 * WV - 1) / (4 * WV))));
+    hipLaunchKernelGGL((sum3_levels_f32<NV4, WV>), g, dim3(64 * WV), 0, (hipStream_t)stream_, a, b, c, out, level_acc, lm, rows);
+  })
+  return pd_check_launch("pd_sum3_levels_f32");
 }
 
 static int colsum_launch(void *x, const void *h, int dtype, int rows, int N, float *acc, bool relu, hipStream_t s, const char *who)
diff --git a/partdistillation_amd/functions/encoder_core.py b/partdistillation_amd/functions/encoder_core.py
--- a/partdistillation_amd/functions/encoder_core.py
+++ b/partdistillation_amd/functions/encoder_core.py
@@ -106,9 +106,10 @@
 
 
 class EncoderSpec:
-    def __init__(self, n_heads, n_levels, n_points, eps, im2col_step, reference_points, spatial_shapes, level_start_index):
+    def __init__(self, n_heads, n_levels, n_points, eps, im2col_step, reference_points, spatial_shapes, level_start_index, level_sizes=None):
         self.M, self.L, self.P, self.eps, self.im2col_step = n_heads, n_levels, n_points, eps, im2col_step
         self.ref, self.shapes, self.lsi = reference_points, spatial_shapes, level_start_index
+        self.level_sizes = None if level_sizes is None else [int(n) for n in level_sizes]
 
 
 USE_X3 = True
@@ -116,6 +117,7 @@
 X3_PROJ = os.environ.get("PD_X3_PROJ", "1") != "0"
 H2_WGRAD = os.environ.get("PD_H2_WGRAD", "1") != "0"
 H2 = os.environ.get("PD_H2", "1") != "0"
+ENC_BOUNDARY = os.environ.get("PD_ENC_BOUNDARY", "1") != "0"
 PRESPLIT = False
 
 
@@ -151,12 +153,30 @@
         return self.t[self.t.shape[0] - 1 - i if self.rev else i]
 
 
+def _level_sums(d_pos, sizes):
+    d_pos = d_pos if d_pos.is_contiguous() else d_pos.contiguous()
+    B, S, C = d_pos.shape
+    if not (d_pos.is_cuda and d_pos.dtype == torch.float32 and C % 128 == 0):
+        return torch.stack([t.sum((0, 1)) for t in torch.split(d_pos, sizes, dim=1)])
+    d_le = torch.zeros((len(sizes), C), dtype=torch.float32, device=d_pos.device)
+    start = 0
+    for l, n in enumerate(sizes):
+        for b in range(B):
+            rw.colsum_acc(d_pos[b, start:start + n], d_le[l])
+        start += n
+    return d_le
+
+
 class EncoderCore(Function):
     @staticmethod
     def forward(ctx, spec: EncoderSpec, src, pos, *params):
         ctx.set_materialize_grads(False)
         B, S, C = src.shape
         M, L, P = spec.M, spec.L, spec.P
+        ctx.level_embed = None
+        if spec.level_sizes is not None:
+            assert len(params) % N_LAYER == 1 and sum(spec.level_sizes) == S and tuple(params[-1].shape) == (len(spec.level_sizes), C)
+            ctx.level_embed, params = params[-1], params[:-1]
         nl = len(params) // N_LAYER
         T = B * S
         src2 = src.reshape(T, C)
@@ -349,7 +369,8 @@
         spec, params = ctx.spec, ctx.params
         B, S, C, nl = ctx.dims
         T = B * S
-        need_w = any(ctx.needs_input_grad[3:])
+        need_w = any(ctx.needs_input_grad[3:3 + nl * N_LAYER])
+        lvl = ctx.level_embed is not None and ENC_BOUNDARY and rw.level_sums_supported(C, len(spec.level_sizes))
         n_off, n_aw, n_l1 = params[0].shape[0], params[2].shape[0], params[10].shape[0]
         per = n_off + n_aw + 2 * C + n_l1
         wk = ctx.wk
@@ -367,24 +388,31 @@
         ref = ref if ref.is_contiguous() else ref.contiguous()
         rec_f = getattr(ctx, "rec", None)
         if rec_f is None:
-            dy, dy2, dyq, d_pos, grads = EncoderCore._bwd_layers_h2(spec, params, ctx.dims, ctx.saved, ctx.saved_am, dy, stacks, need_w, ref)
+            dy, dy2, dyq, d_pos, grads = EncoderCore._bwd_layers_h2(spec, params, ctx.dims, ctx.saved, ctx.saved_am, dy, stacks, need_w, ref, lvl)
         else:
             if rec_f.generation != ctx.rec_gen:
                 raise RuntimeError("the fused encoder ran another forward before this backward: the recorded region's activation arena was "
                                    "overwritten (set PD_CMDBUF=0 for graphs that keep several forward passes alive)")
             slots = [dy] + [k.t for k in stacks] + [spec.shapes, spec.lsi, ref] + list(params)
-            key = ("bwd", id(rec_f), need_w, tuple(k.rev for k in stacks))
+            key = ("bwd", id(rec_f), need_w, tuple(k.rev for k in stacks), lvl)
             rec = _RECS.get(key)
             if rec is None or not rec.matches(slots):
                 rec = cmdbuf.Recording(slots, "encoder backward", stable=[rec_f])
                 with rec:
-                    outs = EncoderCore._bwd_layers_h2(spec, params, ctx.dims, ctx.saved, ctx.saved_am, dy, stacks, need_w, ref)
-                    outs = outs[:4] + (cmdbuf.Fresh(outs[4]),)
+                    outs = EncoderCore._bwd_layers_h2(spec, params, ctx.dims, ctx.saved, ctx.saved_am, dy, stacks, need_w, ref, lvl)
+                    outs = outs[:3] + (cmdbuf.Fresh([outs[3]]) if lvl else outs[3], cmdbuf.Fresh(outs[4]))
                 dy, dy2, dyq, d_pos, grads = rec.finish(outs)
                 _RECS.put(key, rec)
             else:
-                cmdbuf.unalias_grads(params, rec.owns)
+                cmdbuf.unalias_grads(list(params) + ([ctx.level_embed] if lvl else []), rec.owns)
                 dy, dy2, dyq, d_pos, grads = rec.replay(slots)
+            if lvl:
+                d_pos = d_pos[0]
+        if not need_w:
+            grads = [None] * len(grads)
+        if lvl:
+            d_src = rw.sum3_levels(dy, dy2, dyq, d_pos, spec.lsi, S)
+            return (None, d_src.view(B, S, C), None, *grads, d_pos)
         if all(t_.is_cuda and t_.dtype == torch.float32 and t_.is_contiguous() and t_.numel() == dy.numel() for t_ in (dy, dy2, dyq, d_pos)) \
                 and dy.numel() % 4 == 0:
             d_src, d_pos_out = torch.empty_like(dy), torch.empty_like(d_pos)
@@ -395,12 +423,12 @@
             d_pos = d_pos + dyq if rec_f is not None else d_pos.add_(dyq)
             d_src = dy + dy2
             d_src += dyq
-        if not need_w:
-            grads = [None] * len(grads)
+        if ctx.level_embed is not None:
+            return (None, d_src.view(B, S, C), None, *grads, _level_sums(d_pos.view(B, S, C), spec.level_sizes))
         return (None, d_src.view(B, S, C), d_pos.view(B, S, C), *grads)
 
     @staticmethod
-    def _bwd_layers_h2(spec, params, dims, saved, saved_am, dy, stacks, need_w, ref):
+    def _bwd_layers_h2(spec, params, dims, saved, saved_am, dy, stacks, need_w, ref, lvl=False):
         B, S, C, nl = dims
         M, L, P = spec.M, spec.L, spec.P
         T = B * S
@@ -433,7 +461,7 @@
             p = params[i * N_LAYER + j]
             o = offs[i * N_LAYER + j]
             return buf[o:o + p.numel()].view(p.shape)
-        d_pos = torch.zeros((T, C), dtype=torch.float32, device=dev)
+        d_pos = torch.zeros((len(spec.level_sizes), C) if lvl else (T, C), dtype=torch.float32, device=dev)
         grads = [None] * (nl * N_LAYER)
         t_am = lambda w: _Stack(row_amax(w.t.view(-1, w.t.shape[2])).view(nl, w.t.shape[1]), w.rev)
         l1_tam, l2_tam, op_tam, vp_tam, oa_tam = t_am(l1_t), t_am(l2_t), t_am(op_t), t_am(vp_t), t_am(oa_t)
@@ -444,8 +472,12 @@
             x, q, v4, loc6, attn5, a, z1, m1, r1, y1, h, z2, m2, r2, fused_ref, hbits = saved[i]
             (g_sow, g_sob, g_aww, g_awb, g_vpw, g_vpb, g_opw, g_opb, g_n1w, g_n1b, g_l1w, g_l1b, g_l2w, g_l2b, g_n2w,
              g_n2b) = [G(i, j) for j in range(N_LAYER)]
-            dz2, _, dz2_am = rw.add_ln_bwd(z2, m2, r2, n2_w, dy=dy, dy2=dy2, dypos_c=dyq, dgamma=g_n2w, dbeta=g_n2b, dbias=g_l2b,
-                                           dpos_acc=d_pos if dyq is not None else None, pos_div=1, amax=True)
+            if lvl and dyq is not None:
+                dz2, _, dz2_am = rw.add_ln_bwd(z2, m2, r2, n2_w, dy=dy, dy2=dy2, dypos_c=dyq, dgamma=g_n2w, dbeta=g_n2b, dbias=g_l2b,
+                                               level_acc=d_pos, level_start=spec.lsi, tokens=S)
+            else:
+                dz2, _, dz2_am = rw.add_ln_bwd(z2, m2, r2, n2_w, dy=dy, dy2=dy2, dypos_c=dyq, dgamma=g_n2w, dbeta=g_n2b, dbias=g_l2b,
+                                               dpos_acc=d_pos if dyq is not None else None, pos_div=1, amax=True)
             x_am, q_am, a_am, y1_am, h_am = saved_am[i]
             wgrad(dz2, h, g_l2w, None, dz2_am, h_am)
             if hbits is not None:
@@ -497,7 +529,7 @@
         M, L, P = spec.M, spec.L, spec.P
         T = B * S
         dev = d_out.device
-        need_w = any(ctx.needs_input_grad[3:])
+        need_w = any(ctx.needs_input_grad[3:3 + nl * N_LAYER])
         from . import gemm as _gemm
         h2 = getattr(ctx, "h2", False)
         wh2 = h2 and H2_WGRAD
@@ -628,4 +660,6 @@
         d_src += dyq
         if not need_w:
             grads = [None] * len(grads)
+        if ctx.level_embed is not None:
+            return (None, d_src.view(B, S, C), None, *grads, _level_sums(d_pos.view(B, S, C), spec.level_sizes))
         return (None, d_src.view(B, S, C), d_pos.view(B, S, C), *grads)
diff --git a/partdistillation_amd/functions/rowwise.py b/partdistillation_amd/functions/rowwise.py
--- a/partdistillation_amd/functions/rowwise.py
+++ b/partdistillation_amd/functions/rowwise.py
@@ -51,8 +51,21 @@
 
 
 def add_ln_bwd(z, mean, rstd, gamma, *, dy=None, dy2=None, dy_c=None, dypos_c=None, dz_c_dtype=None, dgamma=None, dbeta=None,
-               dbias=None, dpos_acc=None, pos_div=1, out=None, amax=False):
+               dbias=None, dpos_acc=None, pos_div=1, out=None, amax=False, level_acc=None, level_start=None, tokens=0):
     rows, C = z.shape
+    if level_acc is not None:
+        assert dpos_acc is None and dz_c_dtype is None and dy_c is None and dypos_c is not None and dypos_c.dtype == torch.float32
+        assert dypos_c.is_contiguous() and all(t is None or (t.is_contiguous() and t.dtype == torch.float32) for t in (dy, dy2))
+        assert level_start.dtype == torch.int64 and level_start.is_cuda and level_start.is_contiguous()
+        levels = level_start.numel()
+        assert level_acc.dtype == torch.float32 and level_acc.is_contiguous() and tuple(level_acc.shape) == (levels, C) and tokens > 0
+        dz = out if out is not None else torch.empty((rows, C), dtype=torch.float32, device=z.device)
+        am = torch.empty(rows, dtype=torch.float32, device=z.device)
+        _lib.check(_lib.load().pd_add_layernorm_bwd_levels_amax(
+            _p(dy), _p(dy2), None, dypos_c.data_ptr(), _lib.PD_F32, z.data_ptr(), mean.data_ptr(), rstd.data_ptr(), gamma.data_ptr(),
+            dz.data_ptr(), None, 0, _p(dgamma), _p(dbeta), _p(dbias), level_acc.data_ptr(), level_start.data_ptr(), levels, int(tokens),
+            am.data_ptr(), rows, C, _stream()))
+        return dz, None, am
     assert z.dtype == torch.float32 and gamma.dtype == torch.float32 and mean.dtype == torch.float32
     cd = None
     for t in (dy_c, dypos_c):
@@ -113,6 +126,20 @@
     _lib.check(_lib.load().pd_add_rows_amax_f32(a.data_ptr(), b.data_ptr(), q.data_ptr(), ac.data_ptr() if ac is not None else None, am.data_ptr(),
                                                 qm.data_ptr(), a.shape[0], a.shape[1], _stream()))
     return q, ac, am, qm
+
+
+def sum3_levels(a, b, c, level_acc, level_start, tokens):
+    assert all(t.is_contiguous() and t.dtype == torch.float32 and t.shape == a.shape for t in (a, b, c)) and a.dim() == 2
+    assert level_start.dtype == torch.int64 and level_start.is_cuda and level_start.is_contiguous()
+    assert level_acc.dtype == torch.float32 and level_acc.is_contiguous() and tuple(level_acc.shape) == (level_start.numel(), a.shape[1])
+    out = torch.empty_like(a)
+    _lib.check(_lib.load().pd_sum3_levels_f32(a.data_ptr(), b.data_ptr(), c.data_ptr(), out.data_ptr(), level_acc.data_ptr(), level_start.data_ptr(),
+                                              level_start.numel(), int(tokens), a.shape[0], a.shape[1], _stream()))
+    return out
+
+
+def level_sums_supported(C, levels):
+    return C % 256 == 0 and C <= 1024 and 1 <= levels <= 4
 
 
 def colsum_acc(x, acc):
diff --git a/partdistillation_amd/lib.py b/partdistillation_amd/lib.py
--- a/partdistillation_amd/lib.py
+++ b/partdistillation_amd/lib.py
@@ -7,7 +7,7 @@
 CSRC = os.path.join(_HERE, "csrc")
 
 PD_F32, PD_F64, PD_BF16 = 0, 1, 2
-ABI_VERSION = 49
+ABI_VERSION = 50
 
 _c_int, _c_vp = ctypes.c_int, ctypes.c_void_p
 
@@ -86,6 +86,9 @@
     "pd_add_layernorm_fwd_amax": (_c_int, [_c_vp, _c_int, _c_vp, _c_vp, _c_vp, ctypes.c_float, _c_vp, _c_vp, _c_vp, _c_vp, _c_int, _c_vp,
                                            _c_int, _c_vp, _c_vp, _c_vp, _c_vp, _c_int, _c_int, _c_vp]),
     "pd_add_layernorm_bwd_amax": (_c_int, [_c_vp] * 4 + [_c_int] + [_c_vp] * 6 + [_c_int] + [_c_vp] * 4 + [_c_int] + [_c_vp] + [_c_int] * 2 + [_c_vp]),
+    "pd_add_layernorm_bwd_levels_amax": (_c_int, [_c_vp] * 4 + [_c_int] + [_c_vp] * 6 + [_c_int] + [_c_vp] * 5 + [_c_int] * 2 + [_c_vp] + [_c_int] * 2
+                                         + [_c_vp]),
+    "pd_sum3_levels_f32": (_c_int, [_c_vp] * 6 + [_c_int] * 4 + [_c_vp]),
     "pd_colsum_acc": (_c_int, [_c_vp, _c_int, _c_int, _c_int, _c_vp, _c_vp]),
     "pd_relu_bwd_colsum": (_c_int, [_c_vp, _c_vp, _c_int, _c_int, _c_int, _c_vp, _c_vp]),
     "pd_mem_prep_fwd": (_c_int, [_c_vp, ctypes.c_int64, _c_vp, _c_vp, _c_vp, _c_vp, _c_int, _c_int, _c_int, _c_int, _c_vp]),
diff --git a/partdistillation_amd/modeling/pixel_decoder/msdeformattn.py b/partdistillation_amd/modeling/pixel_decoder/msdeformattn.py
--- a/partdistillation_amd/modeling/pixel_decoder/msdeformattn.py
+++ b/partdistillation_amd/modeling/pixel_decoder/msdeformattn.py
@@ -13,7 +13,7 @@
 from ...functions.fused import group_norm_nhwc, group_norm_nhwc_supported
 from ...functions.gemm import linear_f32
 from .ops.modules import MSDeformAttn
-from ...functions.encoder_core import EncoderCore, EncoderSpec
+from ...functions.encoder_core import ENC_BOUNDARY, EncoderCore, EncoderSpec
 from ...functions.rowwise import supports_width, upsample_add, upsample_add_supported
 
 
@@ -64,7 +64,7 @@
         return ref[:, :, None] * valid_ratios[:, None]
 
     def forward(self, src, spatial_shapes, level_start_index, valid_ratios, pos=None, padding_mask=None,
-                shapes_host=None):
+                shapes_host=None, level_embed=None):
         key = (tuple(map(tuple, shapes_host)), src.shape[0], str(src.device)) if shapes_host is not None else None
         if key is not None and key in self._ref_cache:
             reference_points = self._ref_cache[key]
@@ -74,9 +74,11 @@
                 self._ref_cache[key] = reference_points
         if self._fused_ok(src, pos, reference_points, padding_mask):
             l0 = self.layers[0]
+            sizes = [h * w for h, w in shapes_host] if level_embed is not None else None
             spec = EncoderSpec(l0.self_attn.n_heads, l0.self_attn.n_levels, l0.self_attn.n_points, l0.norm1.eps,
-                               l0.self_attn.im2col_step, reference_points, spatial_shapes, level_start_index)
-            return EncoderCore.apply(spec, src, pos, *self._core_params())
+                               l0.self_attn.im2col_step, reference_points, spatial_shapes, level_start_index, sizes)
+            return EncoderCore.apply(spec, src, pos, *self._core_params(), *(() if level_embed is None else (level_embed,)))
+        assert level_embed is None, "a positional table without an autograd edge needs the fused encoder node"
         out = src
         for layer in self.layers:
             out = layer(out, pos, reference_points, spatial_shapes, level_start_index, padding_mask)
@@ -84,9 +86,13 @@
 
     fused_core = True
 
+    def takes_level_embed(self, src, shapes_host):
+        return ENC_BOUNDARY and shapes_host is not None and self._fused_ok(src, True, None, None)
+
     def _fused_ok(self, src, pos, reference_points, padding_mask):
         if not (self.fused_core and self.num_layers and src.is_cuda and src.dtype == torch.float32 and pos is not None
-                and padding_mask is None and reference_points.shape[-1] == 2 and not torch.is_autocast_enabled("cuda")):
+                and padding_mask is None and (reference_points is None or reference_points.shape[-1] == 2)
+                and not torch.is_autocast_enabled("cuda")):
             return False
         l0 = self.layers[0]
         if self.training and any(d.p > 0 for l in self.layers for d in (l.dropout1, l.dropout2, l.dropout3)):
@@ -198,13 +204,20 @@
             src = CatLevels.apply(*srcs)
         else:
             src = torch.cat([s.flatten(2).transpose(1, 2) for s in srcs], 1)
+        level_embed = None
         if src.is_cuda and src.dtype == torch.float32 and self.level_embed.dtype == torch.float32 and self.d_model % 128 == 0:
-            pos = LevelPos.apply(self.level_embed, *pos_embeds)
+            if self.encoder.takes_level_embed(src, shapes_host):
+                level_embed = self.level_embed
+                with torch.no_grad():
+                    pos = LevelPos.apply(level_embed, *pos_embeds)
+            else:
+                pos = LevelPos.apply(self.level_embed, *pos_embeds)
         else:
             pos = torch.cat([p.flatten(2).transpose(1, 2) + self.level_embed[i].view(1, 1, -1)
                              for i, p in enumerate(pos_embeds)], 1)
         valid_ratios = src.new_ones((src.shape[0], len(srcs), 2))
-        memory = self.encoder(src, spatial_shapes, level_start_index, valid_ratios, pos, None, shapes_host=shapes_host)
+        memory = self.encoder(src, spatial_shapes, level_start_index, valid_ratios, pos, None, shapes_host=shapes_host,
+                              level_embed=level_embed)
         return memory, spatial_shapes, level_start_index, shapes_host
 
 
```

New measurement: 110.6 (median of 6 runs). No clear change (+0.5%).
